# PearCoding/PearRay

Hardware: AMD Instinct MI355X
Metric: Msamples/s (higher is better)
Workload: dtype f32; 1 GPU; C4: Cornell box + 999968-triangle soup (1000000 triangles), 1920x1080, `direct` integrator (NEE+MIS+RR, depth 64), sobol 1024-spp schedule, hero wavelengths (spd CMIS), 307 iterations timed; parallelism=tiles1, collective=none (one rank)

## Files before the change

pearray_amd/csrc/device/pr_device.h:

```cpp
#pragma once

#include <hip/hip_runtime.h>
#include <stdint.h>

#include "../../../include/prgpu.h"

#ifndef PR_INLINE_CLOSURES
#define PR_INLINE_CLOSURES 0
#endif

#if PR_INLINE_CLOSURES
#define PR_CLOSURE __forceinline__
#else
#define PR_CLOSURE __noinline__
#endif

namespace prd {

constexpr float PR_EPS		= 1.1920928955078125e-7f;
constexpr float PR_INV_PI_F = 0.31830988618379067154f;
constexpr float PR_PI_F	  = 3.14159265358979323846f;
constexpr uint32_t INVALID	= PRGPU_INVALID_ID;
constexpr float SHADOW_RAY_MIN = 0.0001f;
constexpr float BOUNCE_RAY_MIN = 0.0001f;
// ... 5 lines not shown
constexpr float CIE_END		   = 830.0f;
constexpr float CIE_Y_NORM_SUM = 113.042314572337f;
constexpr float CIE_RANGE	   = CIE_END - CIE_START;
constexpr float CIE_DELTA	   = CIE_RANGE / (CIE_SAMPLES - 1);
constexpr float CIE_Y_NORM	   = CIE_Y_NORM_SUM * CIE_DELTA;

struct __attribute__((aligned(64))) Rec64 {
	float4 q[4];
};
static_assert(sizeof(Rec64) == 64, "Rec64 must be 64 bytes");
constexpr uint32_t REC_LEAF_BIT = 1u;
constexpr uint32_t REC_SINGLE_BIT = 2u;
constexpr uint32_t REC_EMPTY	= 0xFFFFFFFFu;
constexpr uint32_t REC_UNIT_SHIFT = 2u;
constexpr uint32_t LEAF_UNIT_SINGLE = 0x80000000u;
__host__ __device__ __forceinline__ const float4* rec_ptr(const Rec64* recs, uint32_t ref)
{
	return reinterpret_cast<const float4*>(reinterpret_cast<const char*>(recs) + (size_t(ref & ~3u) << 4));
}
constexpr float SLAB_REL		= 1.0000028610229492f;
constexpr float INV_D_MAX		= 1.2089258196146292e24f;
constexpr float SCENE_COORD_MAX = 268435456.0f;

struct DevEntity {
	float m[12];
	float nm[9];
	uint32_t first_tri, n_tris, emission, has_normals;
	float vol_scale, world_area;
	uint32_t light_id, kind;
	float sphere_r;
	uint32_t has_uvs;
};

constexpr uint32_t FEAT_DELTA_MATERIALS = 1u, FEAT_INFINITE_LIGHTS = 2u, FEAT_PLANES = 4u, FEAT_SPHERES = 8u, FEAT_AOVS = 16u, FEAT_SHAPE_LIGHTS = 32u, FEAT_TEXTURES = 64u,
				   FEAT_ROUGH_MATERIALS = 128u, FEAT_LPE = 256u, FEAT_QUADRICS = 512u, FEAT_DISKS = 1024u, FEAT_IMAGES = 2048u,
				   FEAT_MIX_MATERIALS = 4096u ,
				   FEAT_EXPR = 8192u , FEAT_ALL = 16383u;

struct DevQuadric {
	float p[10];
	float lo[3], hi[3];
	float wlo[3], whi[3];
	float inv[12];
	uint32_t tri;
	uint32_t entity;
};

struct DevShapeLight {
	float S[3], Ex[3], Ey[3], Ez[3], nrm[3];
	float width, height;
	float inv[12];
	float pdf_cache;
	float radius;
	float pad[2];
};
struct __attribute__((aligned(128))) DevLight {
	float m[12];
	float nm[9];
	uint32_t entity, kind, n_tris, tri_offset;
	uint32_t has_normals, radiance;
	float vol_scale;
	prgpu_spectrum node, lhs, rhs;
	uint32_t pad[3];
};
static_assert(sizeof(DevLight) == 256, "DevLight must be two 128-byte lines");
struct __attribute__((aligned(128))) DevMaterial {
	prgpu_material m;
	prgpu_spectrum albedo;
};
static_assert(sizeof(DevMaterial) == 128, "DevMaterial must be one 128-byte line");
constexpr uint32_t LIGHT_TRI_FLOATS = 20;
constexpr uint32_t PRIM_SPHERE_BIT = 0x40000000u;
constexpr uint32_t PRIM_DISK_BIT   = 0x20000000u;
constexpr uint32_t PRIM_INDEX_MASK = ~(PRIM_SPHERE_BIT | PRIM_DISK_BIT);

struct DevInfLight {
	uint32_t kind, radiance, background, flags;
	float nm[9], inv_nm[9];
	float outgoing[3];
	float dx[3], dy[3];
	float cos_theta, cone_pdf;
	uint32_t table_offset, az_count, el_count;
	uint32_t dist_offset, dist_w, dist_h;
	float ground_brightness;
};
constexpr int SKY_BANDS			 = PRGPU_SKY_BANDS;
constexpr float SKY_BAND_START	 = 320.0f;
constexpr float SKY_BAND_DELTA	 = 40.0f;
constexpr float ELEVATION_RANGE = PR_PI_F * 0.5f;
constexpr float AZIMUTH_RANGE	 = PR_PI_F * 2;

struct DevCamera {
	float o[3], right[3], up[3], focal[3], xap[3], yap[3];
	float near_t, far_t;
	uint32_t dof, ortho;
	uint32_t kind;
	float angles[4];
	float fov, xaspect, yaspect;
	uint32_t clip;
};

struct DevScene {
	const Rec64* recs;
	uint32_t n_tris, n_inner, n_leaf;
	uint32_t bvh_wide;
	const float* positions;
	const float* normals;
	const float* uvs;
	const uint32_t* indices;
	const uint32_t* tri_material;
	const uint32_t* tri_entity;
	const uint32_t* tri_slot;
	const uint8_t* tri_class;
	const DevEntity* entities;
	const DevMaterial* materials;
	const prgpu_emission* emissions;
	const prgpu_spectrum* spectra;
	const float* tables;
	const uint32_t* light_entity;
	const DevLight* lights;
	const float* light_tris;
	const float* light_cdf;
	uint32_t n_lights;
	const DevInfLight* inf_lights;
	const DevShapeLight* shape_lights;
	uint32_t n_inf_lights;
	const float* sky_cdf;
	float scene_radius;
	uint32_t features;
	const float* wl_cdf;
	uint32_t wl_cdf_size;
	float wl_u_offset, wl_u_scale;
	float agh_c, agh_n;
	const float* sobol2d;
	const float* rr_prob;
	uint32_t rr_size;
	const float* filter;
	const float* cie;
	DevCamera cam;
	prgpu_settings cfg;
	uint32_t spp, mj_x, mj_y, mj_seed;
	uint32_t halton_bx, halton_by, halton_burnin;
	uint32_t single_tap;
	float centre_weight;
	float eps_t;
	const DevQuadric* quadrics;
	uint32_t n_quadrics;
	const float4* shade_rec;
};

struct __attribute__((aligned(128))) SlotState {
	float4 ray_o, ray_d;
	float4 hit;
	uint32_t flags, pad[3];
	float4 sh_o, sh_d;
	float4 wl, wl_pdf;
	float4 cie_x, cie_y, cie_z;
	float4 throughput, path_pdf, prev_pdf;
	float4 last_pos;
	float4 sh_xyz;
};
static_assert(sizeof(SlotState) == 256, "SlotState must be two 128-byte lines");
struct PathState {
	uint64_t* rng;
	uint32_t* pixel;
	struct SlotState* st;
	uint32_t* iter;
	float4* sh_o;
	float4* sh_d;
	float4* sh_xyz;
	uint32_t* sh_slot;
	float* iter_xyz;
	uint32_t plane_stride;
	uint32_t iter_base;
	float* out_xyz;
	uint32_t* samples;
	uint32_t* feedback;
	uint32_t* prim_entity;
	uint32_t* prim_prim;
	float* online_mean;
	float* online_variance;
	const struct DevLpe* lpe;
	uint32_t* cost;
	float* aov[PRGPU_AOV_COUNT];
	uint32_t aov_mask;
};

constexpr uint32_t FLAG_MONO		  = 1u << 8;
constexpr uint32_t FLAG_LAST_DELTA	  = 1u << 9;
constexpr uint32_t FLAG_LAST_EMISSIVE = 1u << 10;
constexpr uint32_t FLAG_NO_RAY		  = 1u << 12;
constexpr uint32_t FLAG_GROUP_MONO	  = 1u << 11;

struct V3 {
	float x, y, z;
};
__device__ __forceinline__ V3 v3(float x, float y, float z) { return V3{ x, y, z }; }
__device__ __forceinline__ V3 operator+(V3 a, V3 b) { return v3(a.x + b.x, a.y + b.y, a.z + b.z); }
__device__ __forceinline__ V3 operator-(V3 a, V3 b) { return v3(a.x - b.x, a.y - b.y, a.z - b.z); }
__device__ __forceinline__ V3 operator-(V3 a) { return v3(-a.x, -a.y, -a.z); }
__device__ __forceinline__ V3 operator*(V3 a, float s) { return v3(a.x * s, a.y * s, a.z * s); }
__device__ __forceinline__ float dot(V3 a, V3 b) { return (a.x * b.x + a.y * b.y) + a.z * b.z; }
__device__ __forceinline__ V3 cross(V3 a, V3 b) { return v3(a.y * b.z - a.z * b.y, a.z * b.x - a.x * b.z, a.x * b.y - a.y * b.x); }
__device__ __forceinline__ V3 normalized(V3 a)
{
	const float n = sqrtf(dot(a, a));
	return v3(a.x / n, a.y / n, a.z / n);
}
__device__ __forceinline__ float comp(V3 a, int i) { return i == 0 ? a.x : (i == 1 ? a.y : a.z); }

struct Blob {
	float v[4];
};
__device__ __forceinline__ Blob blob(float a) { return Blob{ { a, a, a, a } }; }
__device__ __forceinline__ Blob blob4(float a, float b, float c, float d) { return Blob{ { a, b, c, d } }; }
__device__ __forceinline__ Blob from4(float4 a) { return blob4(a.x, a.y, a.z, a.w); }
__device__ __forceinline__ float4 to4(Blob a) { return make_float4(a.v[0], a.v[1], a.v[2], a.v[3]); }
__device__ __forceinline__ Blob operator*(Blob a, Blob b) { return blob4(a.v[0] * b.v[0], a.v[1] * b.v[1], a.v[2] * b.v[2], a.v[3] * b.v[3]); }
__device__ __forceinline__ Blob operator*(Blob a, float s) { return blob4(a.v[0] * s, a.v[1] * s, a.v[2] * s, a.v[3] * s); }
__device__ __forceinline__ Blob operator/(Blob a, Blob b) { return blob4(a.v[0] / b.v[0], a.v[1] / b.v[1], a.v[2] / b.v[2], a.v[3] / b.v[3]); }
__device__ __forceinline__ Blob operator/(Blob a, float s) { return blob4(a.v[0] / s, a.v[1] / s, a.v[2] / s, a.v[3] / s); }
__device__ __forceinline__ Blob operator-(Blob a, Blob b) { return blob4(a.v[0] - b.v[0], a.v[1] - b.v[1], a.v[2] - b.v[2], a.v[3] - b.v[3]); }
__device__ __forceinline__ float bsum(Blob a) { return ((a.v[0] + a.v[1]) + a.v[2]) + a.v[3]; }
__device__ __forceinline__ bool all_le(Blob a, float e) { return a.v[0] <= e && a.v[1] <= e && a.v[2] <= e && a.v[3] <= e; }
__device__ __forceinline__ bool is_zero(Blob a, float e)
{
	return fabsf(a.v[0]) <= e && fabsf(a.v[1]) <= e && fabsf(a.v[2]) <= e && fabsf(a.v[3]) <= e;
}
__device__ __forceinline__ Blob hero_only() { return blob4(1, 0, 0, 0); }

constexpr uint64_t PCG_MULT = 6364136223846793005ULL;
__device__ __forceinline__ uint32_t rng_u32(uint64_t& s)
{
	const uint64_t old	  = s;
	s					  = old * PCG_MULT;
	const uint32_t rshift = uint32_t(old >> 61) & 7u;
	const uint64_t x	  = old ^ (old >> 22);
	return uint32_t(x >> (22u + rshift));
}
__device__ __forceinline__ float rng_float(uint64_t& s)
{
	return __uint_as_float((rng_u32(s) >> 9) | 0x3F800000u) - 1.0f;
}

__device__ __forceinline__ void pr_sincos_2pi(float u, float& s, float& c)
{
	const float k  = floorf(u * 4.0f + 0.5f);
	const float r  = u - 0.25f * k;
	const float x  = 6.28318530717958647692f * r;
	const float x2 = x * x;
	float ps	   = -1.9515295891e-4f;
	ps			   = ps * x2 + 8.3321608736e-3f;
	ps			   = ps * x2 + -1.6666654611e-1f;
	const float sn = (ps * x2) * x + x;
	float pc	   = 2.443315711809948e-5f;
	pc			   = pc * x2 + -1.388731625493765e-3f;
	pc			   = pc * x2 + 4.166664568298827e-2f;
	const float cs = (pc * x2) * x2 + (1.0f - 0.5f * x2);
	switch (int(k) & 3) {
	case 0: s = sn; c = cs; break;
	case 1: s = cs; c = -sn; break;
	case 2: s = -sn; c = -cs; break;
	default: s = -cs; c = sn; break;
	}
}
__device__ __forceinline__ void pr_sincos_rad(float x, float& s, float& c) { pr_sincos_2pi(x * 0.15915494309189533577f, s, c); }
__device__ __forceinline__ float asin_poly(float x)
{
	const float z = x * x;
	float p		  = 4.2163199048e-2f;
	p			  = p * z + 2.4181311049e-2f;
	p			  = p * z + 4.5470025998e-2f;
	p			  = p * z + 7.4953002686e-2f;
	p			  = p * z + 1.6666752422e-1f;
	return (p * z) * x + x;
}
__device__ __forceinline__ float safe_acos(float a)
{
	const float x = fmaxf(-1.0f, fminf(1.0f, a));
	if (x < -0.5f)
		return 3.14159265358979323846f - 2.0f * asin_poly(sqrtf((1.0f + x) * 0.5f));
	if (x > 0.5f)
		return 2.0f * asin_poly(sqrtf((1.0f - x) * 0.5f));
	return 1.57079632679489661923f - asin_poly(x);
}
__device__ __forceinline__ float diff_prod(float a, float b, float c, float d)
{
	const float cd	= c * d;
	const float err = __fmaf_rn(-c, d, cd);
	const float dop = __fmaf_rn(a, b, -cd);
	return dop + err;
}
__device__ __forceinline__ float sum_prod(float a, float b, float c, float d) { return __fmaf_rn(a, b, c * d); }
__device__ __forceinline__ float atan_poly(float xx)
{
	float x = fabsf(xx), y = 0.0f;
	if (x > 2.414213562373095f) {
		y = 1.57079632679489661923f;
		x = -(1.0f / x);
	} else if (x > 0.4142135623730950f) {
		y = 0.78539816339744830962f;
		x = (x - 1.0f) / (x + 1.0f);
	}
	const float z = x * x;
	float p		  = 8.05374449538e-2f;
	p			  = p * z - 1.38776856032e-1f;
	p			  = p * z + 1.99777106478e-1f;
	p			  = p * z - 3.33329491539e-1f;
	y			  = y + ((p * z) * x + x);
	return xx < 0.0f ? -y : y;
}
__device__ __forceinline__ float pr_atan2(float y, float x)
{
	if (x == 0.0f) {
		if (y == 0.0f)
			return 0.0f;
		return y > 0.0f ? 1.57079632679489661923f : -1.57079632679489661923f;
	}
	const float a = atan_poly(y / x);
	if (x > 0.0f)
// ... 997 lines not shown
```

pearray_amd/csrc/device/render.h:

```cpp
#pragma once
#include "pr_device.h"

namespace prd {
constexpr int N_DEVICE_COUNTERS = PRGPU_STAT_COUNT + 32;

struct TraceWorkspace {
	uint32_t* queue_head = nullptr;
	uint2* spill		 = nullptr;
	uint32_t max_blocks	 = 0;
	int refill_below	 = 44;
	uint32_t* bl_list	 = nullptr;
	uint32_t* bl_word	 = nullptr;
	uint32_t* slot_unit	 = nullptr;
	size_t bl_entries	 = 0;
};
size_t trace_workspace_spill_entries(uint32_t max_blocks);
uint32_t trace_stack_capacity();

void launch_raygen(const DevScene& sc, const PathState& ps, uint32_t slot_base, uint32_t n_slots, uint32_t iter, unsigned long long* gstats, hipStream_t st);
void launch_trace_closest(const DevScene& sc, const PathState& ps, const uint32_t* active, uint32_t slot_base, uint32_t n_active, bool count,
						  const TraceWorkspace& ws, uint32_t* shade_counters, unsigned long long* gstats, hipStream_t st);
void launch_shade(const DevScene& sc, const PathState& ps, const uint32_t* active, uint32_t slot_base, uint32_t n_active, uint32_t* next_active,
				  uint32_t* counters, uint32_t* dead_list, uint32_t* queue_head_closest, uint32_t* queue_head_shadow, unsigned long long* gstats,
				  hipStream_t st);
void launch_regen(const DevScene& sc, const PathState& ps, const uint32_t* dead, uint32_t n_dead, uint32_t iter_end, uint32_t* next_active,
				  uint32_t* counters, unsigned long long* gstats, hipStream_t st);
void launch_trace_shadow(const DevScene& sc, const PathState& ps, uint32_t n_items, bool count, const TraceWorkspace& ws, unsigned long long* gstats,
						 hipStream_t st);
struct PersistentGeometry {
	uint32_t n_blocks, slots_per_block;
};
PersistentGeometry persistent_geometry(uint32_t n_owned, uint32_t max_blocks, uint32_t max_slots_per_block);
uint32_t persistent_slot_padding();
uint32_t slot_array_padding();
uint32_t persistent_block_threads();
int shade_ticks_counter();
struct PersistentTuning {
	uint32_t slots	  = 384;
	int shade_min	  = 64;
	int shade_partial = 16;
	int fin_batch	  = 16;
	int occupancy	  = 3;
	int shader_wave	  = -1;
	bool resident	  = true;
};
void launch_path_persistent(const DevScene& sc, const PathState& ps, const uint32_t* owned, uint32_t n_owned, uint32_t iter_begin, uint32_t iter_end,
							bool count, const TraceWorkspace& ws, const PersistentTuning& tune, int shader_waves , uint32_t* next_pixel, uint32_t* error,
							unsigned long long* gstats, hipStream_t st);
struct PathVariant {
	int id;
	uint32_t features;
};
constexpr uint32_t FEAT_NO_LPE = FEAT_ALL & ~(FEAT_LPE | FEAT_QUADRICS | FEAT_DISKS | FEAT_IMAGES | FEAT_MIX_MATERIALS | FEAT_EXPR), FEAT_NO_ROUGH = FEAT_NO_LPE & ~FEAT_ROUGH_MATERIALS;
constexpr PathVariant PATH_VARIANTS[] = { { 1, 0u }, { 2, FEAT_DELTA_MATERIALS }, { 3, FEAT_NO_ROUGH }, { 4, FEAT_NO_LPE }, { 5, FEAT_ALL } };
constexpr int N_PATH_VARIANTS		  = int(sizeof(PATH_VARIANTS) / sizeof(PATH_VARIANTS[0]));
constexpr int path_variant(uint32_t features)
{
	for (int i = 0; i < N_PATH_VARIANTS - 1; ++i)
		if ((features & ~PATH_VARIANTS[i].features) == 0u)
			return i;
	return N_PATH_VARIANTS - 1;
}
constexpr int path_variant_row(int id)
{
	int i = 0;
	while (i < N_PATH_VARIANTS && PATH_VARIANTS[i].id != id)
		++i;
	return i;
}
constexpr bool path_variants_nested()
{
	for (int i = 0; i + 1 < N_PATH_VARIANTS; ++i)
		if ((PATH_VARIANTS[i].features & ~PATH_VARIANTS[i + 1].features) != 0u)
			return false;
	return true;
}
static_assert(PATH_VARIANTS[N_PATH_VARIANTS - 1].features == FEAT_ALL, "the last variant must cover every scene");
constexpr bool expr_rides_with_images()
{
	for (int i = 0; i < N_PATH_VARIANTS; ++i)
		if (((PATH_VARIANTS[i].features & FEAT_IMAGES) != 0u) != ((PATH_VARIANTS[i].features & FEAT_EXPR) != 0u))
			return false;
	return true;
}
static_assert(expr_rides_with_images(), "FEAT_EXPR and FEAT_IMAGES must sit in the same rows: the closures' _uv forms serve both");
static_assert(path_variants_nested(), "each variant's mask must be contained in the next one's: then the first covering row is the smallest covering one");
struct PathSub {
	int occupancy;
	bool wide, count;
};
constexpr PathSub PATH_SUBS[] = { { 3, false, false }, { 3, false, true }, { 2, false, false }, { 2, false, true }, { 3, true, false }, { 3, true, true } };
constexpr int N_PATH_SUBS	  = int(sizeof(PATH_SUBS) / sizeof(PATH_SUBS[0]));
constexpr int path_sub(int occupancy, bool wide, bool count)
{
	const int occ = occupancy >= 3 ? 3 : 2;
	int i		  = 0;
	while (i < N_PATH_SUBS && !(PATH_SUBS[i].occupancy == occ && PATH_SUBS[i].count == count && (occ == 2 || PATH_SUBS[i].wide == wide)))
		++i;
	return i;
}
constexpr bool path_subs_complete()
{
	for (int k = 0; k < 8; ++k)
		if (path_sub(2 + (k >> 2), (k & 2) != 0, (k & 1) != 0) >= N_PATH_SUBS)
			return false;
	for (int i = 0; i < N_PATH_SUBS; ++i)
		if (path_sub(PATH_SUBS[i].occupancy, PATH_SUBS[i].wide, PATH_SUBS[i].count) != i)
			return false;
	return true;
}
static_assert(path_subs_complete(), "PATH_SUBS and path_sub disagree");
struct LatencyGeometry {
	uint32_t n_blocks, slots_per_wave, total_slots;
};
struct LatencyTuning {
	uint32_t slots_per_wave = 256;
	int shade_min			= 48;
	int refill_below		= 40;
};
LatencyGeometry latency_geometry(uint32_t n_owned, uint32_t max_blocks_throughput, uint32_t max_slots_per_wave);
bool latency_variant_built(uint32_t features);
void launch_path_latency(const DevScene& sc, const PathState& ps, const uint32_t* owned, uint32_t n_owned, uint32_t iter_begin, uint32_t iter_end, bool count,
						 const TraceWorkspace& ws, const LatencyTuning& tune, uint32_t* error, unsigned long long* gstats, hipStream_t st);
void launch_resolve(const DevScene& sc, const PathState& ps, uint32_t iter, hipStream_t st);
size_t sort_active_temp_bytes(uint32_t n_max);
void launch_sort_active(const DevScene& sc, const PathState& ps, const uint32_t* active, uint32_t n, uint32_t* keys_in, uint32_t* keys_out, uint32_t* active_out,
						void* temp, size_t temp_bytes, hipStream_t st);
void launch_service_closest(const DevScene& sc, uint32_t n, const float* org, const float* dir, const float* tmin, const float* tmax,
							uint32_t* entity, uint32_t* prim, float* u, float* v, float* t, const TraceWorkspace& ws, unsigned long long* gstats,
							hipStream_t st);
void launch_tri_slot(const DevScene& sc, const uint32_t* leaf_units , uint32_t* tri_slot, hipStream_t st);
void launch_service_closest_split(const DevScene& sc, uint32_t n, const float* org, const float* dir, const float* tmin, const float* tmax,
								  uint32_t* entity, uint32_t* prim, float* u, float* v, float* t, const TraceWorkspace& ws, uint32_t* tri_slot,
								  unsigned long long* gstats, bool leaf_single , hipStream_t st);
void launch_service_any(const DevScene& sc, uint32_t n, const float* org, const float* dir, const float* tmin, const float* distance,
						uint8_t* occluded, const TraceWorkspace& ws, unsigned long long* gstats, hipStream_t st);
struct AoState {
	float4* rec;
	uint32_t* occluded;
	const uint64_t* jump;
	uint32_t* counts;
	uint64_t jump_all;
	uint32_t sample_count;
	uint64_t* dbg_state;
	float* dbg_org;
	float* dbg_dir;
	uint8_t* dbg_occluded;
};

void launch_ao_hits(const DevScene& sc, const PathState& ps, const AoState& ao, uint32_t n_slots, bool instrumented, uint32_t* n_hits, uint32_t* queue_head_closest,
					uint32_t* queue_head_ao, unsigned long long* gstats, hipStream_t st);
void launch_ao_occlusion(const DevScene& sc, const PathState& ps, const AoState& ao, uint32_t n_slots, bool instrumented, const uint32_t* n_hits, const TraceWorkspace& ws,
						 unsigned long long* gstats, hipStream_t st);
void launch_ao_splat(const DevScene& sc, const PathState& ps, const AoState& ao, uint32_t n_slots, const uint32_t* n_hits, hipStream_t st);
bool ao_counts_folded();

constexpr uint32_t VF_RANDOM_COLOURS = 23, VF_GREEN = 23, VF_RED = 24, VF_BLUE = 25, VF_COLOURS = 26;
struct VfState {
	const float4* colours;
	uint32_t mode;
	uint32_t weighting;
};
void launch_vf_shade(const DevScene& sc, const PathState& ps, const VfState& vf, uint32_t n_slots, uint32_t* queue_head_closest, unsigned long long* gstats, hipStream_t st);
}
```

pearray_amd/csrc/device/render.hip:

```cpp
#define PR_WAVEFRONT 1
#define PR_THROUGHPUT 2
#define PR_LATENCY 3
#if !defined(PR_UNIT) || (PR_UNIT != PR_WAVEFRONT && PR_UNIT != PR_THROUGHPUT && PR_UNIT != PR_LATENCY)
#error "compile with -DPR_UNIT=PR_WAVEFRONT, PR_THROUGHPUT or PR_LATENCY (see the Makefile)"
#endif
#include "render.h"

#include <algorithm>
#include <array>
#include <utility>
#if PR_UNIT == PR_WAVEFRONT
#include <hipcub/hipcub.hpp>
#endif

namespace prd {

__device__ __forceinline__ unsigned long long lane_ballot(bool p) { return __builtin_amdgcn_ballot_w64(p); }
__device__ __forceinline__ bool lane_in(unsigned long long m) { return __builtin_amdgcn_inverse_ballot_w64(m); }
__device__ __forceinline__ int wave_popc(unsigned long long m)
{
	int n = __builtin_popcountll(m);
	asm volatile("" : "+s"(n));
	return n;
}
// ... 641 lines not shown
	if ((FEATS & FEAT_QUADRICS) && E.kind == PRGPU_ENTITY_QUADRIC) {
		const DevQuadric& Q = sc.quadrics[E.has_uvs];
		const V3 L = v3(((Q.inv[0] * P.x + Q.inv[1] * P.y) + Q.inv[2] * P.z) + Q.inv[3], ((Q.inv[4] * P.x + Q.inv[5] * P.y) + Q.inv[6] * P.z) + Q.inv[7],
						((Q.inv[8] * P.x + Q.inv[9] * P.y) + Q.inv[10] * P.z) + Q.inv[11]);
		g.N = mat3_mul(E.nm, normalized(quadric_gradient(Q.p, L)));
		frame_duff(g.N, g.Nx, g.Ny);
		g.Nx	   = normalized(g.Nx);
		g.Ny	   = normalized(g.Ny);
		g.entity   = e;
		g.prim	   = 0;
		g.material = sc.tri_material[tri];
		g.emission = E.emission;
		g.uv[0] = g.uv[1] = 0.0f;
		return;
	}
	if ((FEATS & FEAT_PLANES) && E.kind == PRGPU_ENTITY_PLANE) {
		const uint32_t t0 = E.first_tri;
		const V3 v0 = load3(sc.positions, sc.indices[3 * t0]), v1 = load3(sc.positions, sc.indices[3 * t0 + 1]), v3p = load3(sc.positions, sc.indices[3 * t0 + 2]);
		const V3 x = v3p - v0, y = v1 - v0;
		g.N		   = normalized(mat3_mul(E.nm, normalized(cross(x, y))));
		g.Nx	   = normalized(linear_mul(E.m, x));
		g.Ny	   = normalized(linear_mul(E.m, y));
		g.entity   = e;
		g.prim	   = 0;
		g.material = sc.tri_material[tri];
		g.emission = E.emission;
		g.uv[0] = tri == E.first_tri ? u : 1 - u;
		g.uv[1] = tri == E.first_tri ? v : 1 - v;
		return;
	}
	const bool has_uv = (FEATS & FEAT_TEXTURES) && E.has_uvs != 0u;
	const V3 n0 = v3(r0.x, r0.y, r0.z), n1 = v3(r0.w, r1.x, r1.y), n2 = v3(r1.z, r1.w, r2.x);
	const V3 p0 = v3(r2.y, r2.z, r2.w), p1 = v3(r3.x, r3.y, r3.z), p2 = v3(r3.w, r4.x, r4.y);
	const float uv0[2] = { r4.z, r4.w }, uv1[2] = { r5.x, r5.y }, uv2[2] = { r5.z, r5.w };
	if (FEATS & (FEAT_TEXTURES | FEAT_AOVS)) {
		if (has_uv) {
			for (int c = 0; c < 2; ++c)
				g.uv[c] = (uv1[c] * u + uv2[c] * v) + uv0[c] * (1 - u - v);
		} else {
			g.uv[0] = u;
			g.uv[1] = v;
		}
	}
	if (E.has_normals) {
		N = tri_interp(n0, n1, n2, u, v);
		if (has_uv) {
			const V3 dp1 = p1 - p0, dp2 = p2 - p0;
			const float du1 = uv1[0] - uv0[0], dv1 = uv1[1] - uv0[1];
			const float du2 = uv2[0] - uv0[0], dv2 = uv2[1] - uv0[1];
			const float det = diff_prod(dv2, du1, dv1, du2);
			if (det <= PR_EPS) {
				frame_duff(N, Nx, Ny);
				Nx = normalized_or_zero(Nx);
				Ny = normalized_or_zero(Ny);
			} else {
				const V3 t = dp1 * dv2 - dp2 * dv1;
				Nx		   = v3(t.x / det, t.y / det, t.z / det);
				Nx		   = Nx - N * dot(N, Nx);
				Nx		   = normalized_or_zero(Nx);
				Ny		   = cross(N, Nx);
			}
		} else {
			frame_duff(N, Nx, Ny);
		}
	} else {
		Nx = p1 - p0;
		Ny = p2 - p0;
		N  = cross(Nx, Ny);
	}
	g.N		   = normalized(mat3_mul(E.nm, N));
	g.Nx	   = normalized(mat3_mul(E.nm, Nx));
	g.Ny	   = normalized(mat3_mul(E.nm, Ny));
	g.entity   = e;
	g.prim	   = tri - E.first_tri;
	g.material = __float_as_uint(r6.y);
	g.emission = E.emission;
}

struct PathCie {
	float x[4], y[4], z[4];
};
__device__ __forceinline__ uint32_t fragment_value(const DevScene& sc, const Blob& mis, const Blob& importance, const Blob& grp_importance,
												  const Blob& radiance, bool mono, const PathCie& cie, float blend, float xyz[3])
{
	const Blob imp		  = grp_importance * importance;
	const Blob heroFactor = mono ? hero_only() : blob(1);
	const Blob contrib	  = heroFactor * ((mis * imp) * radiance);
	uint32_t fb = 0;
	for (int k = 0; k < 4; ++k) {
		if (isnan(contrib.v[k]))
			fb |= 0x1;
		if (isinf(contrib.v[k]))
			fb |= 0x2;
		if (contrib.v[k] < -PR_EPS)
			fb |= 0x4;
	}
	xyz[0] = xyz[1] = xyz[2] = 0.0f;
	if (fb)
		return fb;
	float triplet[3] = { 0, 0, 0 };
	if (sc.cfg.spectral_mono) {
		triplet[0] = triplet[1] = triplet[2] = contrib.v[0];
	} else {
		for (int k = 0; k < 4; ++k) {
			triplet[0] += contrib.v[k] * cie.x[k];
			triplet[1] += contrib.v[k] * cie.y[k];
			triplet[2] += contrib.v[k] * cie.z[k];
		}
	}
	const float w = sc.single_tap ? sc.centre_weight * blend : blend;
	xyz[0] = w * triplet[0];
	xyz[1] = w * triplet[1];
	xyz[2] = w * triplet[2];
	return 0;
}
__device__ __forceinline__ uint32_t fragment_feedback_zero(const Blob& mis, const Blob& importance, const Blob& grp_importance, bool mono)
{
	const Blob imp		  = grp_importance * importance;
	const Blob heroFactor = mono ? hero_only() : blob(1);
	const Blob contrib	  = heroFactor * ((mis * imp) * blob(0));
	uint32_t fb = 0;
	for (int k = 0; k < 4; ++k) {
		if (isnan(contrib.v[k]))
			fb |= 0x1;
		if (isinf(contrib.v[k]))
			fb |= 0x2;
		if (contrib.v[k] < -PR_EPS)
			fb |= 0x4;
	}
	return fb;
}
__device__ __forceinline__ size_t iter_entry(const PathState& ps, uint32_t slot, uint32_t pixel)
{
	return (ps.plane_stride ? size_t(ps.iter[slot] - ps.iter_base) * ps.plane_stride : size_t(0)) + size_t(3) * pixel;
}
__device__ __forceinline__ void apply_fragment(const PathState& ps, uint32_t pixel, size_t entry, uint32_t fb, const float xyz[3], uint32_t lpe_mask = 0u)
{
	if (fb) {
		ps.feedback[pixel] |= fb;
	} else {
		ps.iter_xyz[entry + 0] += xyz[0];
		ps.iter_xyz[entry + 1] += xyz[1];
		ps.iter_xyz[entry + 2] += xyz[2];
		for (uint32_t k = 0; lpe_mask != 0u && k < PRGPU_LPE_MAX; ++k)
			if (lpe_mask & (1u << k)) {
				float* plane = ps.lpe->iter[k];
				plane[entry + 0] += xyz[0];
				plane[entry + 1] += xyz[1];
				plane[entry + 2] += xyz[2];
			}
	}
}

__device__ __forceinline__ void fold_iteration(const PathState& ps, uint32_t pixel, uint32_t iter, const float value[3], bool with_lpe = false)
{
	const float it = (float)(iter + 1), itm1 = (float)iter;
	for (int c = 0; c < 3; ++c) {
		if (ps.online_mean) {
			float mean		  = ps.online_mean[3 * pixel + c];
			const float var	  = ps.online_variance[3 * pixel + c];
			const float delta = value[c] - mean;
			mean += delta / it;
			const float delta2				  = value[c] - mean;
			ps.online_mean[3 * pixel + c]	  = mean;
			ps.online_variance[3 * pixel + c] = (var * itm1 + delta * delta2) / it;
		}
		ps.out_xyz[3 * pixel + c] = (ps.out_xyz[3 * pixel + c] * itm1 + value[c]) / it;
	}
	if (with_lpe && ps.lpe)
		for (uint32_t k = 0; k < ps.lpe->n; ++k) {
			float* out		  = ps.lpe->out[k];
			const float* iter_ = ps.lpe->iter[k];
			for (int c = 0; c < 3; ++c)
				out[3 * pixel + c] = (out[3 * pixel + c] * itm1 + iter_[3 * pixel + c]) / it;
		}
}
__device__ __forceinline__ float rr_probability(const DevScene& sc, uint32_t L)
{
	return sc.rr_prob[L < sc.rr_size ? L : sc.rr_size - 1];
}
__device__ __forceinline__ bool is_normal(float f)
{
	const uint32_t e = (__float_as_uint(f) >> 23) & 0xFFu;
	return e != 0 && e != 0xFF;
}

struct BlockStats {
	unsigned int v[PRGPU_STAT_COUNT + 4];
};
__device__ __forceinline__ void stats_init(BlockStats& s)
{
	if (threadIdx.x < PRGPU_STAT_COUNT + 4)
		s.v[threadIdx.x] = 0;
	__syncthreads();
}
__device__ __forceinline__ void stats_flush(BlockStats& s, unsigned long long* g)
{
	__syncthreads();
	if (threadIdx.x < PRGPU_STAT_COUNT + 4 && s.v[threadIdx.x])
		atomicAdd(&g[threadIdx.x], (unsigned long long)s.v[threadIdx.x]);
}

__device__ __forceinline__ uint32_t wave_append(bool pred, uint32_t* counter)
{
	const unsigned long long mask = __ballot(pred);
	const uint32_t lane			  = threadIdx.x & 63u;
	const uint32_t prefix		  = __popcll(mask & ((1ull << lane) - 1ull));
	uint32_t base				  = 0;
	if (mask != 0ull) {
		const int leader = __ffsll((long long)mask) - 1;
		if ((int)lane == leader)
			base = atomicAdd(counter, (uint32_t)__popcll(mask));
		base = __shfl(base, leader, 64);
	}
	return base + prefix;
}

__device__ __forceinline__ float halton(uint32_t index, uint32_t base)
{
	float result = 0;
	float f		 = 1;
	for (uint32_t i = index; i > 0;) {
		f = f / base;
		result += f * (i % base);
		i = (uint32_t)floorf(i / (float)base);
	}
	return result;
}
struct WlTable {
	const float* cdf	  = nullptr;
	const uint16_t* guide = nullptr;
};
__device__ __forceinline__ bool camera_path(const DevScene& sc, const PathState& ps, uint32_t slot, uint32_t iter, BlockStats& bs, bool with_lpe = false, WlTable wlt = WlTable())
{
	const prgpu_settings& cfg = sc.cfg;
	const uint32_t pixel	  = ps.pixel[slot];
	const uint32_t gx = pixel % cfg.width, gy = pixel / cfg.width;
	uint64_t rnd = ps.rng[pixel];
	float ax, ay;
	if (cfg.aa_sampler == PRGPU_SAMPLER_MJITT) {
		const uint32_t n  = max(1u, sc.spp);
		const uint32_t id = mjitt_permute(iter, n, sc.mj_seed * 0x51633e2d);
		const uint32_t sx = mjitt_permute(id % sc.mj_x, sc.mj_x, sc.mj_seed * 0x68bc21eb);
		const uint32_t sy = mjitt_permute(id / sc.mj_x, sc.mj_y, sc.mj_seed * 0x02e5be93);
		const float jx	  = rng_float(rnd);
		const float jy	  = rng_float(rnd);
		ax				  = (sx + (sy + jx) / sc.mj_y) / sc.mj_x;
		ay				  = (id + jy) / n;
	} else if (cfg.aa_sampler == PRGPU_SAMPLER_UNIFORM) {
		ax = ay = 0.5f;
	} else if (cfg.aa_sampler == PRGPU_SAMPLER_STRATIFIED) {
		const float range = (1.0f - 0.0f) / (int)sc.mj_x;
		const float ux = rng_float(rnd), uy = rng_float(rnd);
		ax = 0.0f + ux * range + (int)(iter % sc.mj_x) * range;
		ay = 0.0f + uy * range + (int)(iter / sc.mj_x) * range;
	} else if (cfg.aa_sampler >= PRGPU_SAMPLER_SOBOL && cfg.aa_sampler <= PRGPU_SAMPLER_HAMMERSLEY && iter < sc.spp) {
		ax = sc.sobol2d[2 * iter];
		ay = sc.sobol2d[2 * iter + 1];
	} else if (cfg.aa_sampler == PRGPU_SAMPLER_HALTON || cfg.aa_sampler == PRGPU_SAMPLER_HAMMERSLEY) {
		ax = halton(iter + sc.halton_burnin, sc.halton_bx);
		ay = halton(iter + sc.halton_burnin, sc.halton_by);
	} else {
		ax = rng_float(rnd);
		ay = rng_float(rnd);
	}
	const float px = (float)gx + ax - 0.5f, py = (float)gy + ay - 0.5f;
	const float l1 = rng_float(rnd), l2 = rng_float(rnd);
	(void)rng_float(rnd);
	Blob wl, wl_pdf;
	if (cfg.spectral_mono) {
		wl	   = blob(cfg.spectral_start);
		wl_pdf = blob(1.0f);
	} else if (cfg.mapper == PRGPU_MAPPER_SPD_CMIS) {
		const float span = cfg.spectral_end - cfg.spectral_start;
		for (int k = 0; k < 4; ++k) {
			float pdf;
			const float u = rng_float(rnd);
			const float v = wlt.guide ? distribution_sample_continuous_guided(wlt.cdf, sc.wl_cdf_size, wlt.guide, u, pdf) : distribution_sample_continuous(sc.wl_cdf, sc.wl_cdf_size, u, pdf);
			wl.v[k]		  = v * span + cfg.spectral_start;
			wl_pdf.v[k]	  = pdf;
		}
	} else if (cfg.mapper == PRGPU_MAPPER_SPD_HERO) {
		const float span = cfg.spectral_end - cfg.spectral_start;
		float pdf;
		const float v	  = distribution_sample_continuous(sc.wl_cdf, sc.wl_cdf_size, rng_float(rnd), pdf);
		const float hero  = v * span + cfg.spectral_start;
		const float delta = span / 4;
		wl.v[0]			  = hero;
		for (int k = 1; k < 4; ++k)
			wl.v[k] = cfg.spectral_start + fmodf(hero - cfg.spectral_start + k * delta, span);
		wl_pdf = blob(pdf);
	} else if (cfg.mapper == PRGPU_MAPPER_AGH_CMIS) {
		for (int k = 0; k < 4; ++k) {
			wl.v[k]		= agh_sample(rng_float(rnd), sc.agh_n, sc.agh_c);
			wl_pdf.v[k] = agh_pdf(wl.v[k], sc.agh_n);
		}
	} else if (cfg.mapper == PRGPU_MAPPER_AGH_HERO) {
		const float span  = cfg.spectral_end - cfg.spectral_start;
		const float hero  = agh_sample(rng_float(rnd), sc.agh_n, sc.agh_c);
		const float delta = span / 4;
		wl.v[0]			  = hero;
		for (int k = 1; k < 4; ++k)
			wl.v[k] = cfg.spectral_start + fmodf(hero - cfg.spectral_start + k * delta, span);
		wl_pdf = blob(agh_pdf(hero, sc.agh_n));
	} else if (cfg.mapper == PRGPU_MAPPER_CIE || cfg.mapper == PRGPU_MAPPER_CIE_Y) {
		const float span = cfg.spectral_end - cfg.spectral_start;
		for (int k = 0; k < 4; ++k) {
			float pdf;
			const float v = distribution_sample_continuous(sc.wl_cdf, sc.wl_cdf_size, sc.wl_u_offset + rng_float(rnd) * sc.wl_u_scale, pdf);
			wl.v[k]		  = v * span + cfg.spectral_start;
			wl_pdf.v[k]	  = pdf / sc.wl_u_scale;
		}
	} else {
		const float u	  = rng_float(rnd);
		const float span  = cfg.spectral_end - cfg.spectral_start;
		const float delta = span / 4;
		const float start = u * span;
		wl.v[0]			  = start + cfg.spectral_start;
		for (int k = 1; k < 4; ++k)
			wl.v[k] = cfg.spectral_start + fmodf(start + k * delta, span);
		wl_pdf = blob(1.0f);
	}
	const float nx = 2 * (px / (float)cfg.width - 0.5f);
	const float ny = -(2 * (py / (float)cfg.height - 0.5f));
	const DevCamera& cam = sc.cam;
	V3 o = v3(cam.o[0], cam.o[1], cam.o[2]);
	V3 d = (v3(cam.right[0], cam.right[1], cam.right[2]) * nx + v3(cam.up[0], cam.up[1], cam.up[2]) * ny) + v3(cam.focal[0], cam.focal[1], cam.focal[2]);
	bool has_ray = true;
	if (cam.kind == PRGPU_CAMERA_SPHERICAL) {
		const float sx = px / (float)cfg.width, sy = 1 - py / (float)cfg.height;
		const float theta = cam.angles[0] + sy * (cam.angles[1] - cam.angles[0]);
		const float phi	  = cam.angles[2] + sx * (cam.angles[3] - cam.angles[2]);
		float sT, cT, sP, cP;
		pr_sincos_rad(theta, sT, cT);
		pr_sincos_rad(phi, sP, cP);
		d = normalized(from_tangent_space(v3(cam.up[0], cam.up[1], cam.up[2]), v3(cam.right[0], cam.right[1], cam.right[2]), v3(cam.focal[0], cam.focal[1], cam.focal[2]),
										  v3(sP * cT, cP * cT, sT)));
	} else if (cam.kind == PRGPU_CAMERA_FISHEYE) {
		const float fx = 2 * (px / (float)cfg.width - 0.5f) / cam.xaspect;
		const float fy = -(2 * (py / (float)cfg.height - 0.5f) / cam.yaspect);
		has_ray		   = !(cam.clip && fx * fx + fy * fy > 1);
		const float r	  = sqrtf(fx * fx + fy * fy);
		const float theta = r * cam.fov / 2;
		float sT, cT;
		pr_sincos_rad(theta, sT, cT);
		const float sP = r < PR_EPS ? 0 : fy / r;
		const float cP = r < PR_EPS ? 0 : fx / r;
		d = normalized(from_tangent_space(v3(cam.focal[0], cam.focal[1], cam.focal[2]), v3(cam.right[0], cam.right[1], cam.right[2]), v3(cam.up[0], cam.up[1], cam.up[2]),
										  v3(cP * sT, sP * sT, cT)));
	} else if (cam.ortho) {
		o = (o + v3(cam.right[0], cam.right[1], cam.right[2]) * nx) + v3(cam.up[0], cam.up[1], cam.up[2]) * ny;
		d = v3(cam.focal[0], cam.focal[1], cam.focal[2]);
	} else {
		if (cam.dof) {
			float sn, cs;
			pr_sincos_2pi(l1, sn, cs);
			const V3 e = v3(cam.xap[0], cam.xap[1], cam.xap[2]) * (l2 * sn) + v3(cam.yap[0], cam.yap[1], cam.yap[2]) * (l2 * cs);
			o		   = o + e;
			d		   = d - e;
		}
		d = normalized(d);
	}
	const bool mono	   = cfg.spectral_mono || !cfg.spectral_hero;
	ps.rng[pixel]	   = rnd;
	if (has_ray) {
		ps.st[slot].ray_o = make_float4(o.x, o.y, o.z, cam.near_t);
		ps.st[slot].ray_d = make_float4(d.x, d.y, d.z, cam.far_t);
	} else {
		ps.st[slot].ray_o = make_float4(o.x, o.y, o.z, 1.0f);
		ps.st[slot].ray_d = make_float4(0.0f, 0.0f, 1.0f, 0.0f);
	}
	ps.st[slot].wl		   = to4(wl);
	ps.st[slot].wl_pdf	   = to4(wl_pdf);
	{
		float c0[3], c1[3], c2[3], c3[3];
		cie_eval(sc.cie, wl.v[0], c0);
		cie_eval(sc.cie, wl.v[1], c1);
		cie_eval(sc.cie, wl.v[2], c2);
		cie_eval(sc.cie, wl.v[3], c3);
		ps.st[slot].cie_x = make_float4(c0[0], c1[0], c2[0], c3[0]);
		ps.st[slot].cie_y = make_float4(c0[1], c1[1], c2[1], c3[1]);
		ps.st[slot].cie_z = make_float4(c0[2], c1[2], c2[2], c3[2]);
	}
	ps.st[slot].throughput = make_float4(1, 1, 1, 1);
	ps.st[slot].path_pdf  = make_float4(1, 1, 1, 1);
	ps.st[slot].prev_pdf  = make_float4(1, 1, 1, 1);
	if (sc.features & FEAT_SHAPE_LIGHTS)
		ps.st[slot].last_pos = make_float4(0, 0, 0, 0);
	ps.st[slot].flags	   = 0u | (mono ? (FLAG_MONO | FLAG_GROUP_MONO) : 0u) | FLAG_LAST_DELTA | (has_ray ? 0u : FLAG_NO_RAY);
	if (with_lpe && ps.lpe) {
		const DevLpe& L	   = *ps.lpe;
		L.state[slot]	   = lpe_step(ps.lpe, 0u, LPE_SYM_CAMERA);
		const size_t lentry = (ps.plane_stride ? size_t(iter - ps.iter_base) * ps.plane_stride : size_t(0)) + size_t(3) * pixel;
		for (uint32_t k = 0; k < L.n; ++k) {
			float* plane	  = L.iter[k];
			plane[lentry + 0] = 0.0f;
			plane[lentry + 1] = 0.0f;
			plane[lentry + 2] = 0.0f;
		}
	}
	{
		const size_t entry = (ps.plane_stride ? size_t(iter - ps.iter_base) * ps.plane_stride : size_t(0)) + size_t(3) * pixel;
		ps.iter_xyz[entry + 0] = 0.0f;
		ps.iter_xyz[entry + 1] = 0.0f;
		ps.iter_xyz[entry + 2] = 0.0f;
	}
	atomicAdd(&bs.v[PRGPU_STAT_PIXEL_SAMPLES], 1u);
	if (has_ray) {
		atomicAdd(&bs.v[PRGPU_STAT_CAMERA_RAYS], 1u);
		atomicAdd(&bs.v[PRGPU_STAT_PRIMARY_RAYS], 1u);
	}
	return has_ray;
}

#if PR_UNIT == PR_WAVEFRONT
__global__ void __launch_bounds__(256) k_raygen(DevScene sc, PathState ps, uint32_t slot_base, uint32_t n_slots, uint32_t iter, unsigned long long* gstats)
{
	__shared__ BlockStats bs;
	stats_init(bs);
	const uint32_t local = blockIdx.x * blockDim.x + threadIdx.x;
	if (local < n_slots) {
		ps.iter[slot_base + local] = iter;
		camera_path(sc, ps, slot_base + local, iter, bs, ps.lpe != nullptr);
	}
	stats_flush(bs, gstats);
}

__global__ void __launch_bounds__(256) k_regen(DevScene sc, PathState ps, const uint32_t* __restrict__ dead, uint32_t n_dead, uint32_t iter_end,
											  uint32_t* __restrict__ next_active, uint32_t* __restrict__ counters, unsigned long long* gstats)
{
	__shared__ BlockStats bs;
	stats_init(bs);
	const uint32_t i = blockIdx.x * blockDim.x + threadIdx.x;
	bool alive	  = false;
	uint32_t slot = 0;
	if (i < n_dead) {
		slot				 = dead[i];
		const uint32_t pixel = ps.pixel[slot];
		const uint32_t iter	 = ps.iter[slot];
		const float v[3] = { ps.iter_xyz[3 * pixel], ps.iter_xyz[3 * pixel + 1], ps.iter_xyz[3 * pixel + 2] };
		fold_iteration(ps, pixel, iter, v, ps.lpe != nullptr);
		if (iter + 1 < iter_end) {
			ps.iter[slot] = iter + 1;
			camera_path(sc, ps, slot, iter + 1, bs, ps.lpe != nullptr);
			alive = true;
		}
	}
	const uint32_t pos = wave_append(alive, &counters[0]);
	if (alive)
		next_active[pos] = slot;
	stats_flush(bs, gstats);
}

template <bool COUNT>
__global__ void __launch_bounds__(TRAV_BLOCK) k_trace_closest(DevScene sc, PathState ps, const uint32_t* __restrict__ active, uint32_t slot_base,
															 uint32_t n_active, uint32_t* queue_head, uint2* spill, int refill_below, uint32_t* shade_counters,
															 unsigned long long* gstats)
{
	if (blockIdx.x == 0 && threadIdx.x == 0) {
		shade_counters[0] = 0;
		shade_counters[1] = 0;
		shade_counters[2] = 0;
	}
	auto load = [&](uint32_t i, V3& o, V3& d, float& tmin, float& tmax) {
		const uint32_t slot = active ? active[i] : slot_base + i;
		const float4 ro = ps.st[slot].ray_o, rd = ps.st[slot].ray_d;
		o	 = v3(ro.x, ro.y, ro.z);
		d	 = v3(rd.x, rd.y, rd.z);
		tmin = ro.w;
		tmax = rd.w;
	};
	auto store = [&](uint32_t i, const Hit& h) {
		const uint32_t slot = active ? active[i] : slot_base + i;
		ps.st[slot].hit		= make_float4(h.t, h.u, h.v, __uint_as_float(h.tri));
	};
	trace_persistent<false, COUNT>(sc, n_active, queue_head, spill, refill_below, load, store, gstats);
}

#endif
__device__ __forceinline__ RoughDistribution rough_distribution(const prgpu_material& m)
{
	const bool aniso = (m.flags & PRGPU_MATF_ANISOTROPIC) != 0;
	return RoughDistribution{ m.roughness_x, aniso ? m.roughness_y : m.roughness_x, aniso, (m.flags & PRGPU_MATF_NO_VNDF) == 0 };
}
__device__ __forceinline__ Blob rough_dielectric_eval(const RoughDistribution& d, V3 V, V3 L, const Blob& spec, const Blob& trans, const Blob& ior)
{
	Blob w;
	if (sv_same_hemisphere(V, L)) {
		for (int i = 0; i < 4; ++i)
			w.v[i] = mf_reflection_eval(d, V, L, false, DIELECTRIC_AIR, ior.v[i]);
		return w * spec;
	}
	for (int i = 0; i < 4; ++i)
		w.v[i] = mf_transmission_eval(d, V, L, DIELECTRIC_AIR, ior.v[i]);
	return w * trans;
}
__device__ __forceinline__ Blob rough_dielectric_pdf(const RoughDistribution& d, V3 V, V3 L, const Blob& ior)
{
	Blob F, p;
	for (int i = 0; i < 4; ++i)
		F.v[i] = fresnel_dielectric(V.z, DIELECTRIC_AIR, ior.v[i]);
	if (sv_same_hemisphere(V, L)) {
		for (int i = 0; i < 4; ++i)
			p.v[i] = mf_reflection_pdf(d, L, V);
		return F * p;
	}
	for (int i = 0; i < 4; ++i)
		p.v[i] = mf_transmission_pdf(d, V, L, DIELECTRIC_AIR, ior.v[i]);
	return (blob(1) - F) * p;
}
struct Principled {
	Blob base, ior, cie_y;
	float diff_trans, roughness, anisotropic, spec_trans, spec_tint, flatness, metallic, sheen, sheen_tint, clearcoat, clearcoat_gloss;
	bool thin, has_trans, vndf;

	__device__ __forceinline__ static float mix(float v0, float v1, float t) { return (1 - t) * v0 + t * v1; }
	__device__ __forceinline__ static float schlick_r0(float eta)
	{
		const float factor = (eta - 1.0f) / (eta + 1.0f);
		return factor * factor;
	}
	__device__ __forceinline__ float thin_transmission_roughness() const { return fmaxf(0.0f, fminf(1.0f, (0.65f * (bsum(ior) / 4) - 0.35f) * roughness)); }
	__device__ __forceinline__ RoughDistribution roughness_closure(float r) const
	{
		const float aspect = sqrtf(1 - anisotropic * 0.9f);
		const float ax	   = fmaxf(0.001f, r * r / aspect);
		const float ay	   = fmaxf(0.001f, r * r * aspect);
		return RoughDistribution{ ax, ay, true, vndf };
	}
	__device__ __forceinline__ bool is_delta() const { return roughness_closure(roughness).is_delta(); }
	struct Lobes {
		float diff_refl, diff_trans, spec_refl, spec_trans;
	};
	__device__ __forceinline__ Lobes lobe_distribution(V3 V) const
	{
		Lobes d;
		d.diff_refl = roughness * roughness * (1.0f - metallic) * (1.0f - spec_trans);
		d.spec_refl = 1;
		if (has_trans) {
			const float F = fresnel_dielectric(V.z, DIELECTRIC_AIR, ior.v[0]);
			d.diff_trans  = diff_trans * d.diff_refl;
			d.spec_trans  = (1.0f - F) * (1.0f - metallic) * spec_trans;
			d.spec_refl *= F;
		} else {
			d.diff_trans = 0;
			d.spec_trans = 0;
		}
		const float norm = d.diff_refl + d.spec_refl + d.diff_trans + d.spec_trans;
		if (norm <= PR_EPS)
			return Lobes{ 1.0f, 0.0f, 0.0f, 0.0f };
		d.diff_refl /= norm;
		d.spec_refl /= norm;
		d.diff_trans /= norm;
		d.spec_trans /= norm;
// ... 334 lines not shown
	v = theta * PR_INV_PI_F;
}
__device__ __forceinline__ float env_jacobian(float v)
{
	float s, c;
	pr_sincos_rad(v * PR_PI_F, s, c);
	const float denom = 2 * PR_PI_F * PR_PI_F * s;
	return denom <= PR_EPS ? 0.0f : 1.0f / denom;
}
template <bool EXPR = false>
__device__ __forceinline__ void inf_light_eval(const DevScene& sc, const DevInfLight& il, V3 dir, const Blob& wl, bool camera_ray, Blob& radiance, float& dir_pdf)
{
	if (il.kind == PRGPU_LIGHT_ENVIRONMENT && (il.flags & PRGPU_ENVF_TEXTURED)) {
		const V3 ld = mat3_mul(il.inv_nm, dir);
		float u, v;
		uv_from_direction(ld, u, v);
		radiance = (camera_ray && il.background != INVALID) ? spectrum_eval<false, EXPR>(sc, il.background, wl) : env_image_eval<EXPR>(sc, il, wl, u, v);
		if (il.dist_w)
			dir_pdf = distribution2d_pdf(sc.sky_cdf + il.dist_offset, il.dist_w, il.dist_h, u, v) * env_jacobian(v);
		else
			dir_pdf = fabsf(ld.z) * PR_INV_PI_F;
		return;
	}
	if (il.kind == PRGPU_LIGHT_SKY) {
		const ElAz ea	  = ea_from_direction(mat3_mul(il.inv_nm, dir));
		const bool extend = (il.flags & PRGPU_SKYF_EXTEND) != 0;
		if (!extend && ea.el < 0.0f) {
			radiance = blob(0);
			dir_pdf	 = 0.0f;
			return;
		}
		radiance = sky_radiance(sc.tables + il.table_offset, il.az_count, il.el_count, wl, ea);
		dir_pdf	 = distribution2d_pdf(sc.sky_cdf + il.dist_offset, il.dist_w, il.dist_h, ea.az / AZIMUTH_RANGE,
									  extend ? ea.el / (2 * ELEVATION_RANGE) + 0.5f : ea.el / ELEVATION_RANGE);
		dir_pdf *= sky_jacobian(ea.el);
		return;
	}
	if (il.kind == PRGPU_LIGHT_SUN) {
		const float cosine = fmaxf(0.0f, dot(dir, v3(il.outgoing[0], il.outgoing[1], il.outgoing[2])));
		if (cosine < il.cos_theta) {
			radiance = blob(0);
			dir_pdf	 = 0.0f;
		} else {
			radiance = spectrum_eval<false, EXPR>(sc, il.radiance, wl);
			dir_pdf	 = il.cone_pdf;
		}
		return;
	}
	if (il.kind == PRGPU_LIGHT_CIE_SKY) {
		radiance = cie_sky_radiance<EXPR>(sc, il, wl, dir);
		dir_pdf	 = fabsf(mat3_mul(il.inv_nm, dir).z) * PR_INV_PI_F;
		return;
	}
	radiance	= spectrum_eval<false, EXPR>(sc, (camera_ray && il.background != INVALID) ? il.background : il.radiance, wl);
	const V3 ld = mat3_mul(il.inv_nm, dir);
	dir_pdf		= fabsf(ld.z) * PR_INV_PI_F;
}
template <bool EXPR = false>
__device__ __forceinline__ void inf_light_sample(const DevScene& sc, const DevInfLight& il, float d0, float d1, const Blob& wl, V3& L, float& dir_pdf, Blob& radiance)
{
	if (il.kind == PRGPU_LIGHT_DISTANT) {
		L		 = v3(il.outgoing[0], il.outgoing[1], il.outgoing[2]);
		dir_pdf	 = 1.0f;
		radiance = spectrum_eval<false, EXPR>(sc, il.radiance, wl);
	} else if (il.kind == PRGPU_LIGHT_ENVIRONMENT && (il.flags & PRGPU_ENVF_TEXTURED)) {
		float u, v;
		V3 lo;
		if (il.dist_w) {
			distribution2d_sample(sc.sky_cdf + il.dist_offset, il.dist_w, il.dist_h, d0, d1, u, v, dir_pdf);
			float st, ct, sp, cp;
			pr_sincos_rad(v * PR_PI_F, st, ct);
			pr_sincos_rad(u * 2 * PR_PI_F, sp, cp);
			lo = v3(st * cp, st * sp, ct);
			dir_pdf *= env_jacobian(v);
		} else {
			u		= d0;
			v		= d1;
			lo		= cos_hemi(d0, d1);
			dir_pdf = lo.z * PR_INV_PI_F;
		}
		L		 = mat3_mul(il.nm, lo);
		radiance = env_image_eval<EXPR>(sc, il, wl, u, v);
	} else if (il.kind == PRGPU_LIGHT_SKY) {
		float u, v;
		distribution2d_sample(sc.sky_cdf + il.dist_offset, il.dist_w, il.dist_h, d0, d1, u, v, dir_pdf);
		const ElAz ea = (il.flags & PRGPU_SKYF_EXTEND) ? ElAz{ 2 * ELEVATION_RANGE * (v - 0.5f), AZIMUTH_RANGE * u } : ElAz{ ELEVATION_RANGE * v, AZIMUTH_RANGE * u };
		L			  = mat3_mul(il.nm, ea_to_direction(ea));
		dir_pdf *= sky_jacobian(ea.el);
		radiance = sky_radiance(sc.tables + il.table_offset, il.az_count, il.el_count, wl, ea);
	} else if (il.kind == PRGPU_LIGHT_SUN) {
		const V3 dir = uniform_cone(d0, d1, il.cos_theta);
		L			 = from_tangent_space(v3(il.outgoing[0], il.outgoing[1], il.outgoing[2]), v3(il.dx[0], il.dx[1], il.dx[2]), v3(il.dy[0], il.dy[1], il.dy[2]), dir);
		dir_pdf		 = il.cone_pdf;
		radiance	 = spectrum_eval<false, EXPR>(sc, il.radiance, wl);
	} else {
		const V3 lo = cos_hemi(d0, d1);
		dir_pdf		= lo.z * PR_INV_PI_F;
		L			= mat3_mul(il.nm, lo);
		radiance	= il.kind == PRGPU_LIGHT_CIE_SKY ? cie_sky_radiance<EXPR>(sc, il, wl, L) : spectrum_eval<false, EXPR>(sc, il.radiance, wl);
	}
}

__device__ __forceinline__ uint32_t scatter_symbol(uint32_t kind, float roughness_x, V3 Vt, V3 Lt)
{
	const bool same = sv_same_hemisphere(Vt, Lt);
	switch (kind) {
	case PRGPU_MAT_LAMBERT:
	case PRGPU_MAT_OREN_NAYAR: return LPE_SYM_DIFFUSE_REFLECTION;
	case PRGPU_MAT_NULL: return LPE_SYM_SPECULAR_TRANSMISSION;
	case PRGPU_MAT_DIELECTRIC:
	case PRGPU_MAT_ROUGH_DIELECTRIC: return same ? LPE_SYM_SPECULAR_REFLECTION : LPE_SYM_SPECULAR_TRANSMISSION;
	case PRGPU_MAT_PRINCIPLED:
		return roughness_x < 0.5f ? (same ? LPE_SYM_SPECULAR_REFLECTION : LPE_SYM_SPECULAR_TRANSMISSION) : (same ? LPE_SYM_DIFFUSE_REFLECTION : LPE_SYM_DIFFUSE_TRANSMISSION);
	default: return LPE_SYM_SPECULAR_REFLECTION;
	}
}
__device__ __forceinline__ uint32_t scatter_symbol(const prgpu_material& m, V3 Vt, V3 Lt) { return scatter_symbol(m.kind, m.roughness_x, Vt, Lt); }

template <bool AOVS>
__device__ __forceinline__ void commit_shading_point(const PathState& ps, uint32_t pixel, V3 P, const GeomPoint& gp, V3 ray_d, float depth2)
{
	ps.samples[pixel] += 1;
	if (AOVS && ps.aov_mask) {
		auto add3 = [&](int k, V3 v) {
			if (ps.aov[k]) {
				ps.aov[k][3 * pixel] += v.x;
				ps.aov[k][3 * pixel + 1] += v.y;
				ps.aov[k][3 * pixel + 2] += v.z;
			}
		};
		auto add1 = [&](int k, float v) {
			if (ps.aov[k])
				ps.aov[k][pixel] += v;
		};
		add3(PRGPU_AOV_POSITION, P);
		add3(PRGPU_AOV_NORMAL, gp.N);
		add3(PRGPU_AOV_NORMAL_G, gp.N);
		add3(PRGPU_AOV_TANGENT, gp.Nx);
		add3(PRGPU_AOV_BITANGENT, gp.Ny);
		add3(PRGPU_AOV_VIEW, ray_d);
		add1(PRGPU_AOV_ENTITY_ID, (float)gp.entity);
		add1(PRGPU_AOV_MATERIAL_ID, (float)gp.material);
		add1(PRGPU_AOV_EMISSION_ID, (float)gp.emission);
		add1(PRGPU_AOV_DEPTH, sqrtf(depth2));
	}
}

template <uint32_t FEATS>
__device__ __forceinline__ void shade_vertex(const DevScene& sc, const PathState& ps, uint32_t slot, BlockStats& bs, bool& alive, bool& want_shadow,
											 float4& sh_o, float4& sh_d, float4& sh_xyz, const float4* hit_src = nullptr )
{
	constexpr bool EXPR		  = (FEATS & FEAT_EXPR) != 0u;
	const prgpu_settings& cfg = sc.cfg;
	const uint32_t pixel = ps.pixel[slot];
	const size_t entry	 = iter_entry(ps, slot, pixel);
	const float4 ro = ps.st[slot].ray_o, rd = ps.st[slot].ray_d;
	const V3 ray_o = v3(ro.x, ro.y, ro.z), ray_d = v3(rd.x, rd.y, rd.z);
	const float4 hit4  = hit_src ? *hit_src : ps.st[slot].hit;
	const uint32_t tri = __float_as_uint(hit4.w);
	uint32_t flags	   = ps.st[slot].flags;
	if (flags & FLAG_NO_RAY)
		return;
	const uint32_t depth = flags & 0xFFu;
	const bool mono		 = (flags & FLAG_MONO) != 0;
	const Blob wl		 = from4(ps.st[slot].wl);
	const Blob wvl_pdf	 = from4(ps.st[slot].wl_pdf);
	PathCie cie;
	{
		const float4 cx = ps.st[slot].cie_x, cy = ps.st[slot].cie_y, cz = ps.st[slot].cie_z;
		cie.x[0] = cx.x; cie.x[1] = cx.y; cie.x[2] = cx.z; cie.x[3] = cx.w;
		cie.y[0] = cy.x; cie.y[1] = cy.y; cie.y[2] = cy.z; cie.y[3] = cy.w;
		cie.z[0] = cz.x; cie.z[1] = cz.y; cie.z[2] = cz.z; cie.z[3] = cz.w;
	}
	Blob throughput		 = from4(ps.st[slot].throughput);
	Blob path_pdf		 = from4(ps.st[slot].path_pdf);
	Blob prev_pdf		 = from4(ps.st[slot].prev_pdf);
	const Blob grp_imp	 = (flags & FLAG_GROUP_MONO) ? hero_only() : blob(1.0f);
	const float blend	 = 1.0f;
	const bool power_mis = cfg.mis == PRGPU_MIS_POWER;
	const Blob hf		 = mono ? hero_only() : blob(1.0f);
	const bool with_lpe	 = (FEATS & FEAT_LPE) && ps.lpe != nullptr;
	uint32_t lpe		 = with_lpe ? ps.lpe->state[slot] : 0u;

	if (depth == 0 && tri == INVALID) {
		ps.prim_entity[pixel] = INVALID;
		ps.prim_prim[pixel]	  = INVALID;
	}
	if (tri == INVALID) {
		atomicAdd(&bs.v[PRGPU_STAT_BACKGROUND_HITS], 1u);
		float xyz[3];
		uint32_t fb;
		const uint32_t m_bg = with_lpe ? lpe_accepting(ps.lpe, lpe_step(ps.lpe, lpe, LPE_SYM_BACKGROUND)) : 0u;
		if (depth == 0) {
			atomicAdd(&bs.v[PRGPU_STAT_CAMERA_DEPTH], 1u);
			bool illuminated = false;
			for (uint32_t k = 0; (FEATS & FEAT_INFINITE_LIGHTS) && k < sc.n_inf_lights; ++k) {
				const DevInfLight& il = sc.inf_lights[k];
				if (il.kind == PRGPU_LIGHT_DISTANT)
					continue;
				illuminated = true;
				Blob radiance;
				float dir_pdf;
				inf_light_eval<EXPR>(sc, il, ray_d, wl, true, radiance, dir_pdf);
				fb = fragment_value(sc, blob(1), blob(1), grp_imp, radiance, mono, cie, blend, xyz);
				apply_fragment(ps, pixel, entry, fb, xyz, m_bg);
			}
			if (!illuminated) {
				fb = fragment_value(sc, blob(1), blob(1), grp_imp, blob(0), mono, cie, blend, xyz);
				apply_fragment(ps, pixel, entry, fb, xyz, m_bg);
			}
		} else if ((FEATS & FEAT_INFINITE_LIGHTS) && sc.n_inf_lights && cfg.direct) {
			float denom_mis = 0;
			Blob radiance	= blob(0);
			for (uint32_t k = 0; k < sc.n_inf_lights; ++k) {
				const DevInfLight& il = sc.inf_lights[k];
				if (il.kind == PRGPU_LIGHT_DISTANT)
					continue;
				Blob er;
				float dir_pdf;
				inf_light_eval<EXPR>(sc, il, ray_d, wl, false, er, dir_pdf);
				const float selProb = sc.light_cdf[sc.n_lights + k + 1] - sc.light_cdf[sc.n_lights + k];
				const float pdf_S	= dir_pdf * selProb;
				for (int c = 0; c < 4; ++c)
					radiance.v[c] += er.v[c];
				const Blob a = prev_pdf * pdf_S;
				denom_mis += bsum(power_mis ? a * a : a);
			}
			if (!cfg.nee || (flags & FLAG_LAST_DELTA)) {
				fb = fragment_value(sc, hf / (wvl_pdf * bsum(hf)), throughput, grp_imp, radiance, mono, cie, blend, xyz);
			} else {
				const float denom = bsum(power_mis ? path_pdf * path_pdf : path_pdf) + denom_mis;
				const float p0	  = power_mis ? path_pdf.v[0] * path_pdf.v[0] : path_pdf.v[0];
				const Blob mis	  = (hf * p0) / ((power_mis ? wvl_pdf * wvl_pdf : wvl_pdf) * denom);
				fb				  = fragment_value(sc, mis, throughput, grp_imp, radiance, mono, cie, blend, xyz);
			}
			apply_fragment(ps, pixel, entry, fb, xyz, m_bg);
		} else {
			fb = fragment_value(sc, hf / (wvl_pdf * bsum(hf)), throughput, grp_imp, blob(0), mono, cie, blend, xyz);
			apply_fragment(ps, pixel, entry, fb, xyz, m_bg);
		}
	} else {
		const V3 P = ray_o + ray_d * hit4.x;
		GeomPoint gp;
		geometry_point<FEATS>(sc, tri, hit4.y, hit4.z, P, gp);
		if (depth == 0) {
			ps.prim_entity[pixel] = gp.entity;
			ps.prim_prim[pixel]	  = gp.prim;
		}
		const V3 N		   = gp.N;
		const float NdotV  = dot(ray_d, N);
		const V3 dP		   = ray_o - P;
		const float depth2 = dot(dP, dP);
		const uint32_t pathLength = depth + 1;
		atomicAdd(&bs.v[PRGPU_STAT_ENTITY_HITS], 1u);
		atomicAdd(&bs.v[PRGPU_STAT_CAMERA_DEPTH], 1u);
		if (pathLength == 1)
			commit_shading_point<(FEATS & FEAT_AOVS) != 0>(ps, pixel, P, gp, ray_d, depth2);
		const bool hasEmission = gp.emission != INVALID;
		bool go_on			   = true;
		if (cfg.direct && hasEmission) {
			const float cosC = -NdotV;
			if (!(fabsf(cosC) <= PR_EPS)) {
				const bool behind	= cosC < 0.0f;
				const Blob radiance = behind ? blob(0) : spectrum_eval<false, EXPR>(sc, sc.emissions[gp.emission].radiance, wl);
				float xyz[3];
				uint32_t fb;
				if (!cfg.nee || behind || (flags & FLAG_LAST_DELTA)) {
					fb = fragment_value(sc, hf / (wvl_pdf * bsum(hf)), throughput, grp_imp, radiance, mono, cie, blend, xyz);
				} else {
					const uint32_t lid	 = sc.entities[gp.entity].light_id;
					const float selProb	 = sc.light_cdf[lid + 1] - sc.light_cdf[lid];
					float posPDF		 = 1.0f / sc.entities[gp.entity].world_area;
					if ((FEATS & FEAT_SHAPE_LIGHTS) && sc.entities[gp.entity].kind == PRGPU_ENTITY_PLANE) {
						const float4 lpos = ps.st[slot].last_pos;
						posPDF			  = plane_light_pdf(sc.shape_lights[gp.entity], P, v3(lpos.x, lpos.y, lpos.z));
					} else if ((FEATS & FEAT_SHAPE_LIGHTS) && sc.entities[gp.entity].kind == PRGPU_ENTITY_SPHERE) {
						posPDF = 2 * sc.shape_lights[gp.entity].pdf_cache;
					}
					posPDF				 = posPDF * depth2 / fabsf(cosC);
					const float posPDF_S = posPDF * selProb;
					const Blob a		 = prev_pdf * posPDF_S;
					const float denom	 = bsum(power_mis ? a * a : a) + bsum(power_mis ? path_pdf * path_pdf : path_pdf);
					const float p0		 = power_mis ? path_pdf.v[0] * path_pdf.v[0] : path_pdf.v[0];
					const Blob mis		 = (hf * p0) / ((power_mis ? wvl_pdf * wvl_pdf : wvl_pdf) * denom);
					fb					 = fragment_value(sc, mis, throughput, grp_imp, radiance, mono, cie, blend, xyz);
				}
				apply_fragment(ps, pixel, entry, fb, xyz, with_lpe ? lpe_accepting(ps.lpe, lpe_step(ps.lpe, lpe, LPE_SYM_EMISSIVE)) : 0u);
			}
			if (!cfg.emissive_scatter)
				go_on = false;
		}
		if (gp.material == INVALID)
			go_on = false;
		if (go_on) {
			const DevMaterial& dmat = sc.materials[gp.material];
			prgpu_material mat		= dmat.m;
			constexpr bool MIX		= (FEATS & FEAT_MIX_MATERIALS) != 0u;
			const bool comb			= MIX && (mat.kind == PRGPU_MAT_BLEND || mat.kind == PRGPU_MAT_ADD);
			if ((FEATS & FEAT_TEXTURES) && (sc.features & FEAT_TEXTURES) && !comb) {
				mat.albedo		 = resolve_texture(sc, mat.albedo, gp.uv);
				mat.ior			 = resolve_texture(sc, mat.ior, gp.uv);
				mat.k			 = resolve_texture(sc, mat.k, gp.uv);
				mat.transmission = resolve_texture(sc, mat.transmission, gp.uv);
			}
			const V3 Vt				 = to_tangent_space(N, gp.Nx, gp.Ny, -ray_d);
			uint64_t rnd			 = ps.rng[pixel];
			const bool deltaMat		 = (FEATS & FEAT_DELTA_MATERIALS) && (mat.kind == PRGPU_MAT_DIELECTRIC || mat.kind == PRGPU_MAT_CONDUCTOR || mat.kind == PRGPU_MAT_MIRROR);
			const bool roughMat		 = (FEATS & FEAT_ROUGH_MATERIALS) && (mat.kind == PRGPU_MAT_ROUGH_CONDUCTOR || mat.kind == PRGPU_MAT_ROUGH_DIELECTRIC || mat.kind == PRGPU_MAT_PRINCIPLED);
			const bool delta1 = comb && mix_delta_only(sc.materials[mat.two_sided].m.kind), delta2 = comb && mix_delta_only(sc.materials[mat.thin].m.kind);
			const bool deltaOnly = comb ? (delta1 && delta2) : (deltaMat || (MIX && mat.kind == PRGPU_MAT_NULL));
			const Blob cie_y_blob	 = blob4(cie.y[0], cie.y[1], cie.y[2], cie.y[3]);
			constexpr bool IMG	= (FEATS & FEAT_IMAGES) != 0u;
			Blob albedo_v		= roughMat ? blob(0) : albedo_eval<IMG, EXPR>(sc, mat, dmat.albedo, dmat.m.albedo, wl, gp.uv);
			if (cfg.nee && !deltaOnly && !hasEmission && (sc.n_lights + ((FEATS & FEAT_INFINITE_LIGHTS) ? sc.n_inf_lights : 0u))) {
				do {
					float selPdf;
					const uint32_t n_sel = sc.n_lights + ((FEATS & FEAT_INFINITE_LIGHTS) ? sc.n_inf_lights : 0u);
					const float u_sel	 = rng_float(rnd);
					uint32_t lid		 = 0;
					if (n_sel == 1)
						selPdf = 1.0f;
					else
						lid = distribution_sample_discrete(sc.light_cdf, n_sel + 1, u_sel, selPdf, nullptr);
					if ((FEATS & FEAT_INFINITE_LIGHTS) && lid >= sc.n_lights) {
						const DevInfLight& il = sc.inf_lights[lid - sc.n_lights];
						const float d0 = rng_float(rnd), d1 = rng_float(rnd);
						(void)rng_float(rnd);
						(void)rng_float(rnd);
						V3 L;
						float dirPdf;
						const bool delta = il.kind == PRGPU_LIGHT_DISTANT;
						Blob radiance;
						inf_light_sample<EXPR>(sc, il, d0, d1, wl, L, dirPdf, radiance);
						const V3 lpos	 = P + L * sc.scene_radius;
						const V3 dLP	 = lpos - P;
						const float sqrD = dot(dLP, dLP);
						const float cosC = fabsf(dot(L, N));
						const float cosL = 1.0f;
						if (!(cosC * cosL > GEOMETRY_EPS && sqrD > DISTANCE_EPS))
							break;
						const V3 Lt = to_tangent_space(N, gp.Nx, gp.Ny, L);
						Blob weight, bsdf_pdf;
						bool evalDelta;
						uint32_t sym_kind	= 0u;
						float sym_roughness = 0.0f;
						if constexpr (MIX)
							vertex_eval<FEATS>(sc, mat, albedo_v, comb, delta1, delta2, wl, cie_y_blob, Vt, Lt, weight, bsdf_pdf, evalDelta, sym_kind, sym_roughness, gp.uv);
						else
							material_eval<FEATS>(sc, mat, albedo_v, wl, cie_y_blob, Vt, Lt, weight, bsdf_pdf, evalDelta, gp.uv);
						if (evalDelta)
							break;
						const Blob bsdfWvlPdfS = bsdf_pdf * hf;
						if (all_le(bsdfWvlPdfS, PDF_EPS))
							break;
						const Blob connectionW = radiance * weight;
						const bool worth	   = !is_zero(connectionW, PR_EPS);
						float lightPdfS;
						if (delta) {
							lightPdfS = 1;
						} else {
							lightPdfS = dirPdf;
							lightPdfS *= selPdf;
							if (!is_normal(lightPdfS) || lightPdfS <= PDF_EPS)
								break;
						}
						const Blob lightPdfS2 = (blob(1) * lightPdfS) * hf;
						if (all_le(lightPdfS2, PDF_EPS))
							break;
						Blob mis;
						if (cfg.direct && !(flags & FLAG_LAST_EMISSIVE)) {
							const float rr		= rr_probability(sc, pathLength);
							const Blob bsdfPdfS = bsdfWvlPdfS * rr;
							const Blob a = path_pdf * lightPdfS2, b = path_pdf * bsdfPdfS;
							const float denom = bsum(power_mis ? a * a : a) + bsum(power_mis ? b * b : b);
							const float num	  = path_pdf.v[0] * lightPdfS2.v[0];
							mis = delta ? hf / bsum(hf) : blob(power_mis ? num * num : num) / ((hf * denom) * (power_mis ? wvl_pdf * wvl_pdf : wvl_pdf));
						} else {
							mis = hf / (wvl_pdf * bsum(hf));
						}
						const V3 oN = dot(L, N) < 0 ? -N : N;
						float sh_far = INFINITY;
						const V3 so	 = sane_ray(safe_position(P, L, oN), sh_far);
						float xyz_vis[3];
						const float xyz_occ[3] = { 0.0f, 0.0f, 0.0f };
						const uint32_t fb_vis = fragment_value(sc, mis, throughput, grp_imp, connectionW / lightPdfS2.v[0], mono, cie, blend, xyz_vis);
						const uint32_t fb_occ = fragment_feedback_zero(mis, throughput, grp_imp, mono);
						atomicAdd(&bs.v[PRGPU_STAT_BACKGROUND_HITS], 1u);
						if (worth) {
							atomicAdd(&bs.v[PRGPU_STAT_SHADOW_RAYS], 1u);
							want_shadow = true;
							sh_o		= make_float4(so.x, so.y, so.z, SHADOW_RAY_MIN);
							sh_d		= make_float4(L.x, L.y, L.z, sh_far);
							const uint32_t m_nee = with_lpe ? lpe_accepting(ps.lpe, lpe_step(ps.lpe, lpe_step(ps.lpe, lpe, scatter_symbol(MIX ? sym_kind : mat.kind, MIX ? sym_roughness : mat.roughness_x, Vt, Lt)), LPE_SYM_BACKGROUND)) : 0u;
							sh_xyz		= make_float4(xyz_vis[0], xyz_vis[1], xyz_vis[2], __uint_as_float(fb_vis | (fb_occ << 8) | (m_nee << 16)));
						} else {
							apply_fragment(ps, pixel, entry, fb_occ, xyz_occ);
						}
						break;
					}
					const DevLight& LE = sc.lights[lid];
					const uint32_t le  = LE.entity;
					const float u0 = rng_float(rnd), u1 = rng_float(rnd);
					V3 lp;
					float pdf_a;
					GeomPoint lgp;
					if ((FEATS & FEAT_SHAPE_LIGHTS) && LE.kind == PRGPU_ENTITY_PLANE) {
						const DevShapeLight& SL = sc.shape_lights[le];
						plane_light_sample(SL, P, u0, u1, lp, pdf_a);
						lgp.N = v3(SL.Ez[0], SL.Ez[1], SL.Ez[2]);
					} else if ((FEATS & FEAT_SHAPE_LIGHTS) && LE.kind == PRGPU_ENTITY_SPHERE) {
						sphere_light_sample(sc.shape_lights[le], LE.m, P, u0, u1, lp, pdf_a);
						lgp.N = normalized_or_zero(lp - v3(LE.m[3], LE.m[7], LE.m[11]));
					} else if ((FEATS & FEAT_DISKS) && LE.kind == PRGPU_ENTITY_DISK) {
						disk_light_sample(sc.shape_lights[le], LE.m, u0, u1, lp, pdf_a);
						lgp.N = normalized(mat3_mul(LE.nm, v3(0.0f, 0.0f, 1.0f)));
					} else {
						float k0, k1;
						const float f0		= modff(u0 * LE.n_tris, &k0);
						const float f1		= modff(u1 * LE.n_tris, &k1);
						const uint32_t face = min((uint32_t)k0, LE.n_tris - 1);
						const float* lt = sc.light_tris + size_t(LE.tri_offset + face) * LIGHT_TRI_FLOATS;
						const V3 p0 = v3(lt[0], lt[1], lt[2]), p1 = v3(lt[3], lt[4], lt[5]), p2 = v3(lt[6], lt[7], lt[8]);
						const V3 ee		 = cross(p1 - p0, p2 - p0);
						const float area = 0.5f * sqrtf(dot(ee, ee));
						pdf_a			 = 1.0f / (LE.n_tris * area * LE.vol_scale);
						float bu, bv;
						if (f1 > f0) {
							const float x = f0 / 2;
							bu = x;
							bv = f1 - x;
						} else {
							const float y = f1 / 2;
							bu = f0 - y;
							bv = y;
						}
						lp = affine_mul(LE.m, tri_interp(p0, p1, p2, bu, bv));
						V3 Nl;
						if (LE.has_normals)
							Nl = tri_interp(v3(lt[9], lt[10], lt[11]), v3(lt[12], lt[13], lt[14]), v3(lt[15], lt[16], lt[17]), bu, bv);
						else
							Nl = cross(p1 - p0, p2 - p0);
						lgp.N = normalized(mat3_mul(LE.nm, Nl));
					}
					const V3 L			 = normalized(lp - P);
					const float cosLight = fminf(1.0f, fmaxf(-1.0f, -dot(L, lgp.N)));
					const Blob radiance	 = spectrum_eval_copy<EXPR>(sc, LE.node, LE.lhs, LE.rhs, wl);
					const V3 dLP		 = lp - P;
					const float sqrD	 = dot(dLP, dLP);
					const float cosC	 = fabsf(dot(L, N));
					const float cosL	 = fabsf(cosLight);
					if (!(cosC * cosL > GEOMETRY_EPS && sqrD > DISTANCE_EPS))
						break;
					const V3 Lt = to_tangent_space(N, gp.Nx, gp.Ny, L);
					Blob weight, bsdf_pdf;
					bool evalDelta;
					uint32_t sym_kind	= 0u;
					float sym_roughness = 0.0f;
					if constexpr (MIX)
						vertex_eval<FEATS>(sc, mat, albedo_v, comb, delta1, delta2, wl, cie_y_blob, Vt, Lt, weight, bsdf_pdf, evalDelta, sym_kind, sym_roughness, gp.uv);
					else
						material_eval<FEATS>(sc, mat, albedo_v, wl, cie_y_blob, Vt, Lt, weight, bsdf_pdf, evalDelta, gp.uv);
					if (evalDelta)
						break;
					const Blob bsdfWvlPdfS = bsdf_pdf * hf;
					if (all_le(bsdfWvlPdfS, PDF_EPS))
						break;
					const Blob connectionW = radiance * weight;
					const bool worth	   = !is_zero(connectionW, PR_EPS);
					float lightPdfS		   = pdf_a * sqrD / cosL;
					lightPdfS *= selPdf;
					if (!is_normal(lightPdfS) || lightPdfS <= PDF_EPS)
						break;
					const Blob lightPdfS2 = (blob(1) * lightPdfS) * hf;
					if (all_le(lightPdfS2, PDF_EPS))
						break;
					Blob mis;
					if (cfg.direct && !(flags & FLAG_LAST_EMISSIVE)) {
						const float rr		= rr_probability(sc, pathLength);
						const Blob bsdfPdfS = bsdfWvlPdfS * rr;
						const Blob a = path_pdf * lightPdfS2, b = path_pdf * bsdfPdfS;
						const float denom = bsum(power_mis ? a * a : a) + bsum(power_mis ? b * b : b);
						const float num	  = path_pdf.v[0] * lightPdfS2.v[0];
						mis				  = blob(power_mis ? num * num : num) / ((hf * denom) * (power_mis ? wvl_pdf * wvl_pdf : wvl_pdf));
					} else {
						mis = hf / (wvl_pdf * bsum(hf));
					}
					float distance = sqrtf(sqrD);
					const V3 oN	   = dot(L, N) < 0 ? -N : N;
					const V3 so	   = sane_ray(safe_position(P, L, oN), distance);
					float xyz_vis[3];
					const float xyz_occ[3] = { 0.0f, 0.0f, 0.0f };
					const uint32_t fb_vis = fragment_value(sc, mis, throughput, grp_imp, connectionW / lightPdfS2.v[0], mono, cie, blend, xyz_vis);
					const uint32_t fb_occ = fragment_feedback_zero(mis, throughput, grp_imp, mono);
					atomicAdd(&bs.v[PRGPU_STAT_ENTITY_HITS], 1u);
					if (worth) {
						atomicAdd(&bs.v[PRGPU_STAT_SHADOW_RAYS], 1u);
						want_shadow = true;
						sh_o		= make_float4(so.x, so.y, so.z, SHADOW_RAY_MIN);
						sh_d		= make_float4(L.x, L.y, L.z, distance);
						const uint32_t m_nee = with_lpe ? lpe_accepting(ps.lpe, lpe_step(ps.lpe, lpe_step(ps.lpe, lpe, scatter_symbol(MIX ? sym_kind : mat.kind, MIX ? sym_roughness : mat.roughness_x, Vt, Lt)), LPE_SYM_EMISSIVE)) : 0u;
						sh_xyz		= make_float4(xyz_vis[0], xyz_vis[1], xyz_vis[2], __uint_as_float(fb_vis | (fb_occ << 8) | (m_nee << 16)));
					} else {
						apply_fragment(ps, pixel, entry, fb_occ, xyz_occ);
					}
				} while (false);
			}
			flags = hasEmission ? (flags | FLAG_LAST_EMISSIVE) : (flags & ~FLAG_LAST_EMISSIVE);

			const float scatProb = deltaOnly ? 1.0f : rr_probability(sc, pathLength);
			bool cont			 = !(scatProb <= PR_EPS);
			if (cont && scatProb < 1.0f) {
				const float rp = rng_float(rnd);
				if (rp > scatProb)
					cont = false;
			}
			if (cont) {
				V3 Lt;
				Blob integral_weight, pdf_s;
				bool heroCollapsing = false;
				float mix_weight = 1.0f, mix_pdf = 1.0f;
				bool child_rough = false;
				if (comb) {
					const bool add	  = mat.kind == PRGPU_MAT_ADD;
					const float f	  = fminf(1.0f, fmaxf(0.0f, mat.roughness_x));
					const bool second = !(rng_float(rnd) < (add ? 0.5f : 1 - f));
					mix_pdf			  = add ? 0.5f : (second ? f : 1 - f);
					mix_weight		  = add ? 1.0f : mix_pdf;
					const uint32_t id = second ? mat.thin : mat.two_sided;
					mix_child<FEATS>(sc, id, wl, gp.uv, mat, albedo_v, child_rough);
				}
				const bool sampleDeltaMat = comb ? mix_delta_only(mat.kind) : deltaOnly, sampleRoughMat = comb ? child_rough : roughMat;
				bool sampleDelta	= sampleDeltaMat;
				if (sampleRoughMat && IMG) {
					rough_sample_uv(sc, mat, wl, cie_y_blob, Vt, rnd, Lt, integral_weight, pdf_s, sampleDelta, heroCollapsing, gp.uv);
				} else if (sampleRoughMat) {
					rough_sample(sc, mat, wl, cie_y_blob, Vt, rnd, Lt, integral_weight, pdf_s, sampleDelta, heroCollapsing);
				} else if ((FEATS & FEAT_DELTA_MATERIALS) && mat.kind == PRGPU_MAT_MIRROR) {
					pdf_s			= blob(1);
					integral_weight = albedo_v;
					Lt				= v3(-Vt.x, -Vt.y, Vt.z);
				} else if (MIX && mat.kind == PRGPU_MAT_NULL) {
					pdf_s			= blob(1);
					integral_weight = blob(1);
					Lt				= -Vt;
				} else if ((FEATS & FEAT_DELTA_MATERIALS) && mat.kind == PRGPU_MAT_CONDUCTOR) {
					pdf_s		   = blob(1);
					const Blob eta = spectrum_eval<IMG, EXPR>(sc, mat.ior, wl, gp.uv), kk = spectrum_eval<IMG, EXPR>(sc, mat.k, wl, gp.uv);
					Blob fresnel;
					for (int i = 0; i < 4; ++i)
						fresnel.v[i] = fresnel_conductor(fabsf(Vt.z), 1.0f, eta.v[i], kk.v[i]);
					integral_weight = fresnel * albedo_v;
					Lt				= v3(-Vt.x, -Vt.y, Vt.z);
					heroCollapsing	= spectrum_varying<EXPR>(sc.spectra[mat.ior]) || spectrum_varying<EXPR>(sc.spectra[mat.k]);
				} else if (sampleDeltaMat) {
					pdf_s		  = blob(1);
					const Blob n2 = spectrum_eval<IMG, EXPR>(sc, mat.ior, wl, gp.uv);
					float F		  = fresnel_dielectric(Vt.z, DIELECTRIC_AIR, n2.v[0]);
					if (mat.thin && F < 1.0f)
						F += (1 - F) * F / (F + 1);
					const Blob rWeight = albedo_v;
					if (rng_float(rnd) <= F) {
						Lt				= v3(-Vt.x, -Vt.y, Vt.z);
						integral_weight = rWeight;
					} else {
						const Blob tWeight = mat.transmission != INVALID ? spectrum_eval<IMG, EXPR>(sc, mat.transmission, wl, gp.uv) : rWeight;
						if (mat.thin) {
							Lt				= -Vt;
							integral_weight = tWeight;
						} else {
							Lt				= refract_shading(DIELECTRIC_AIR / n2.v[0], Vt);
							integral_weight = (signbit(Lt.z) == signbit(Vt.z)) ? rWeight : tWeight;
						}
					}
					heroCollapsing = spectrum_varying<EXPR>(sc.spectra[mat.ior]);
				} else if (MIX && mat.kind == PRGPU_MAT_OREN_NAYAR) {
					const float s1 = rng_float(rnd), s2 = rng_float(rnd);
					Lt				= cos_hemi(s1, s2);
					integral_weight = oren_nayar_calc(albedo_v, mat.roughness_x, Vt, Lt, fmaxf(0.0f, Lt.z));
					pdf_s			= blob(Lt.z * PR_INV_PI_F);
				} else if (!mat.two_sided && Vt.z < 0.0f) {
					Lt				= v3(0, 0, 0);
					integral_weight = blob(0);
					pdf_s			= blob(0);
				} else {
					const float s1 = rng_float(rnd), s2 = rng_float(rnd);
					Lt				= cos_hemi(s1, s2);
					integral_weight = albedo_v;
					pdf_s			= blob(Lt.z * PR_INV_PI_F);
					if (signbit(Vt.z) != signbit(Lt.z))
						Lt = -Lt;
				}
				if (comb) {
					integral_weight = integral_weight * mix_weight;
					pdf_s			= pdf_s * mix_pdf;
				}
				const V3 L = normalized(from_tangent_space(N, gp.Nx, gp.Ny, Lt));
				if (with_lpe)
					lpe = lpe_step(ps.lpe, lpe, scatter_symbol(mat, Vt, Lt));
				flags	 = sampleDelta ? (flags | FLAG_LAST_DELTA) : (flags & ~FLAG_LAST_DELTA);
				prev_pdf = path_pdf;
				path_pdf = path_pdf * (pdf_s * scatProb);
				if (all_le(path_pdf, PDF_EPS))
					cont = false;
				if (cont) {
					throughput = throughput * integral_weight;
					if (heroCollapsing) {
						throughput = throughput * hero_only();
						path_pdf   = path_pdf * hero_only();
					}
					if (is_zero(throughput, PR_EPS))
						cont = false;
					if (heroCollapsing)
						flags |= FLAG_MONO;
				}
				if (cont) {
					const V3 oN		 = dot(L, N) < 0 ? -N : N;
					float far_t		 = INFINITY;
					const V3 no		 = sane_ray(safe_position(P, L, oN), far_t);
					const uint32_t nd = depth + 1;
					if (nd < cfg.max_ray_depth) {
						alive				= true;
						ps.st[slot].ray_o		= make_float4(no.x, no.y, no.z, BOUNCE_RAY_MIN);
						ps.st[slot].ray_d		= make_float4(L.x, L.y, L.z, far_t);
						ps.st[slot].throughput = to4(throughput);
						ps.st[slot].path_pdf	= to4(path_pdf);
						ps.st[slot].prev_pdf	= to4(prev_pdf);
						if ((FEATS & FEAT_SHAPE_LIGHTS) && (sc.features & FEAT_SHAPE_LIGHTS))
							ps.st[slot].last_pos = make_float4(P.x, P.y, P.z, 0.0f);
						ps.st[slot].flags		= (flags & ~0xFFu) | nd;
						if (with_lpe)
							ps.lpe->state[slot] = lpe;
						atomicAdd(&bs.v[PRGPU_STAT_CAMERA_RAYS], 1u);
						atomicAdd(&bs.v[PRGPU_STAT_BOUNCE_RAYS], 1u);
						if (flags & FLAG_MONO)
							atomicAdd(&bs.v[PRGPU_STAT_MONOCHROME_RAYS], 1u);
					}
				}
			}
			ps.rng[pixel] = rnd;
		}
	}
}

#if PR_UNIT == PR_WAVEFRONT
__global__ void __launch_bounds__(256) k_shade(DevScene sc, PathState ps, const uint32_t* __restrict__ active, uint32_t slot_base, uint32_t n_active,
											  uint32_t* __restrict__ next_active, uint32_t* __restrict__ counters ,
											  uint32_t* __restrict__ dead_list, uint32_t* queue_head_closest, uint32_t* queue_head_shadow,
											  unsigned long long* gstats)
{
	__shared__ BlockStats bs;
	stats_init(bs);
	if (blockIdx.x == 0 && threadIdx.x == 0) {
		*queue_head_closest = 0;
		*queue_head_shadow	= 0;
	}
	const uint32_t i = blockIdx.x * blockDim.x + threadIdx.x;
	bool alive = false, want_shadow = false;
	uint32_t slot = 0;
	float4 sh_o = make_float4(0, 0, 0, 0), sh_d = sh_o, sh_xyz = sh_o;
	if (i < n_active) {
		slot = active ? active[i] : slot_base + i;
		if (ps.lpe)
			shade_vertex<FEAT_ALL>(sc, ps, slot, bs, alive, want_shadow, sh_o, sh_d, sh_xyz);
		else if (sc.features)
			shade_vertex<(FEAT_ALL & ~FEAT_LPE)>(sc, ps, slot, bs, alive, want_shadow, sh_o, sh_d, sh_xyz);
		else
			shade_vertex<0u>(sc, ps, slot, bs, alive, want_shadow, sh_o, sh_d, sh_xyz);
	}
	const uint32_t pos_next = wave_append(alive, &counters[0]);
	if (alive)
		next_active[pos_next] = slot;
	if (dead_list) {
		const bool died			= i < n_active && !alive;
		const uint32_t pos_dead = wave_append(died, &counters[2]);
		if (died)
			dead_list[pos_dead] = slot;
	}
	const uint32_t pos_sh = wave_append(want_shadow, &counters[1]);
	if (want_shadow) {
		ps.sh_o[pos_sh]	   = sh_o;
		ps.sh_d[pos_sh]	   = sh_d;
		ps.sh_xyz[pos_sh]  = sh_xyz;
		ps.sh_slot[pos_sh] = slot;
	}
	stats_flush(bs, gstats);
}

template <bool COUNT>
__global__ void __launch_bounds__(TRAV_BLOCK) k_trace_shadow(DevScene sc, PathState ps, uint32_t n, uint32_t* queue_head, uint2* spill,
															int refill_below, unsigned long long* gstats)
{
	auto load = [&](uint32_t i, V3& o, V3& d, float& tmin, float& tmax) {
		const float4 so = ps.sh_o[i], sd = ps.sh_d[i];
		o	 = v3(so.x, so.y, so.z);
		d	 = v3(sd.x, sd.y, sd.z);
		tmin = so.w;
		tmax = sd.w - 0.001f;
	};
	auto store = [&](uint32_t i, const Hit& h) {
		const float4 x		 = ps.sh_xyz[i];
		const uint32_t fbs	 = __float_as_uint(x.w);
		const uint32_t pixel = ps.pixel[ps.sh_slot[i]];
		const size_t entry	 = iter_entry(ps, ps.sh_slot[i], pixel);
		if (h.tri != INVALID) {
			const uint32_t fb = (fbs >> 8) & 0xFFu;
			if (fb)
				ps.feedback[pixel] |= fb;
		} else {
			const float xyz[3] = { x.x, x.y, x.z };
			apply_fragment(ps, pixel, entry, fbs & 0xFFu, xyz, (fbs >> 16) & 0xFu);
		}
	};
	trace_persistent<true, COUNT>(sc, n, queue_head, spill, refill_below, load, store, gstats);
}

__global__ void __launch_bounds__(256) k_resolve(DevScene sc, PathState ps, uint32_t iter)
{
	const uint32_t W = sc.cfg.width, H = sc.cfg.height;
	const uint32_t p = blockIdx.x * blockDim.x + threadIdx.x;
	if (p >= W * H)
		return;
	float acc[3];
	if (sc.single_tap) {
		acc[0] = ps.iter_xyz[3 * p];
		acc[1] = ps.iter_xyz[3 * p + 1];
		acc[2] = ps.iter_xyz[3 * p + 2];
	} else {
		const int r = (int)sc.cfg.filter_radius, dd = 2 * r + 1;
		const int x = (int)(p % W), y = (int)(p / W);
		acc[0] = acc[1] = acc[2] = 0.0f;
		for (int sy = y - r; sy <= y + r; ++sy) {
			if (sy < 0 || sy >= (int)H)
				continue;
			for (int sx = x - r; sx <= x + r; ++sx) {
				if (sx < 0 || sx >= (int)W)
					continue;
				const float fw = sc.filter[(y - sy + r) * dd + (x - sx + r)];
				if (fw > PR_EPS) {
					const uint32_t q = (uint32_t)sy * W + (uint32_t)sx;
					acc[0] += fw * ps.iter_xyz[3 * q];
					acc[1] += fw * ps.iter_xyz[3 * q + 1];
					acc[2] += fw * ps.iter_xyz[3 * q + 2];
				}
			}
		}
	}
	fold_iteration(ps, p, iter, acc);
}


#endif
#ifndef PR_PP_SLOTS_MAX
#define PR_PP_SLOTS_MAX (PP_BLOCK == 768 ? 1536 : 512)
#endif
#ifndef PR_FIN_PRIO
#define PR_FIN_PRIO 2
#endif
#ifndef PR_REFILL_PRIO
#define PR_REFILL_PRIO 2
#endif
#ifndef PR_SHADE_PRIO
#define PR_SHADE_PRIO 3
#endif
constexpr int PP_SLOTS_MAX		= PR_PP_SLOTS_MAX;
constexpr uint32_t WL_LDS		= 448;
constexpr uint32_t PP_EMPTY		= 0xFFFFFFFFu;
constexpr uint32_t PP_ANY		= 0x80000000u;
constexpr uint32_t PP_DEAD		= 0x100u;
constexpr uint32_t PP_VISIBLE	= 0x200u;
constexpr uint32_t PP_CLS_SHIFT	= 12u;
constexpr uint32_t PP_SHADOW	= 0x400u;
constexpr unsigned long long PP_IDLE_LIMIT_TICKS = 30ull * 100000000ull;

template <int NQ>
struct PPShared {
	uint2 stack[STACK_LDS * TRAV_BLOCK];
	uint32_t q_ray[2 * PP_SLOTS_MAX];
	uint32_t q_shade[NQ + 1][PP_SLOTS_MAX];
	uint32_t pending[PP_SLOTS_MAX];
	uint32_t ray_head, ray_tail, shade_head[NQ + 1], shade_tail[NQ + 1];
	float wl_cdf[WL_LDS];
	uint16_t wl_guide[CDF_GUIDE_BUCKETS + 2];
	uint32_t n_list, unit_next, exhausted, n_frozen;
	uint32_t live;
	uint32_t error;
	BlockStats bs;
};

__device__ __forceinline__ uint32_t lds_load(const uint32_t* p) { return __hip_atomic_load(p, __ATOMIC_RELAXED, __HIP_MEMORY_SCOPE_WORKGROUP); }
__device__ __forceinline__ uint32_t wave_bcast0(uint32_t v) { return (uint32_t)__builtin_amdgcn_readfirstlane((int)v); }

__device__ __forceinline__ void ring_push(uint32_t* q, uint32_t cap_mask, uint32_t* tail, bool pred, uint32_t value)
{
	const unsigned long long mask = __ballot(pred);
	if (mask == 0ull)
		return;
	const uint32_t lane = threadIdx.x & 63u;
	uint32_t base		= 0;
	const int leader	= __ffsll((long long)mask) - 1;
	if ((int)lane == leader)
		base = __hip_atomic_fetch_add(tail, (uint32_t)__popcll(mask), __ATOMIC_RELAXED, __HIP_MEMORY_SCOPE_WORKGROUP);
	base = __shfl(base, leader, 64);
	if (pred)
		__hip_atomic_store(&q[(base + __popcll(mask & ((1ull << lane) - 1ull))) & cap_mask], value, __ATOMIC_RELEASE, __HIP_MEMORY_SCOPE_WORKGROUP);
}
__device__ __forceinline__ uint32_t ring_claim(uint32_t* head, const uint32_t* tail, uint32_t want, uint32_t& first)
{
	uint32_t n = 0, h = 0;
	if ((threadIdx.x & 63u) == 0) {
		h				 = lds_load(head);
		const uint32_t t = lds_load(tail);
		n				 = min(want, t - h);
		if (n) {
			uint32_t expect = h;
			if (!__hip_atomic_compare_exchange_strong(head, &expect, h + n, __ATOMIC_RELAXED, __ATOMIC_RELAXED, __HIP_MEMORY_SCOPE_WORKGROUP))
				n = 0;
		}
	}
	first = wave_bcast0(h);
	return wave_bcast0(n);
}
__device__ __forceinline__ uint32_t ring_take(uint32_t* q, uint32_t cap_mask, uint32_t pos)
{
	uint32_t* e = &q[pos & cap_mask];
	uint32_t v;
	while ((v = __hip_atomic_load(e, __ATOMIC_ACQUIRE, __HIP_MEMORY_SCOPE_WORKGROUP)) == PP_EMPTY)
		__builtin_amdgcn_s_sleep(1);
	__hip_atomic_store(e, PP_EMPTY, __ATOMIC_RELAXED, __HIP_MEMORY_SCOPE_WORKGROUP);
	return v;
}


template <uint32_t FEATS>
__device__ __forceinline__ void apply_deferred_nee(const PathState& ps, uint32_t slot, uint32_t pw)
{
	if (pw & PP_SHADOW) {
		const float4 x		 = ps.st[slot].sh_xyz;
		const uint32_t fbs	 = __float_as_uint(x.w);
		const uint32_t pixel = ps.pixel[slot];
		if (pw & PP_VISIBLE) {
			const float xyz[3] = { x.x, x.y, x.z };
			apply_fragment(ps, pixel, iter_entry(ps, slot, pixel), fbs & 0xFFu, xyz, (FEATS & FEAT_LPE) ? (fbs >> 16) & 0xFu : 0u);
		} else if ((fbs >> 8) & 0xFFu) {
			ps.feedback[pixel] |= (fbs >> 8) & 0xFFu;
		}
	}
}

template <uint32_t FEATS>
__device__ __forceinline__ void fold_ended_sample(const PathState& ps, uint32_t slot, uint32_t pixel, uint32_t iter)
{
	if (ps.cost)
		ps.cost[pixel] += (ps.st[slot].flags & 0xFFu) + 1u;
	if (!ps.plane_stride) {
		const float v[3] = { ps.iter_xyz[3 * pixel], ps.iter_xyz[3 * pixel + 1], ps.iter_xyz[3 * pixel + 2] };
		fold_iteration(ps, pixel, iter, v, (FEATS & FEAT_LPE) != 0u);
	}
}


struct PersistentArgs {
	const uint32_t* owned;
	uint32_t n_owned;
	uint32_t* next_pixel;
	uint32_t* error;
	uint32_t slots_per_block;
	uint32_t iter_begin, iter_end;
	uint2* spill;
	int refill_below;
	uint32_t shade_min;
	uint32_t shade_partial;
	uint32_t shader_wave;
	int fin_batch;
	uint32_t direct_map;
	uint32_t resident;
	uint32_t bl_cap;
	uint32_t* bl_list;
	uint32_t* bl_word;
	uint32_t* slot_unit;
	unsigned long long* gstats;
};
constexpr uint32_t PP_SHADE_HELP = 128u;
constexpr uint32_t BL_UNWRITTEN = 0xFFFFFFFEu, BL_HOLE = 0xFFFFFFFFu;

template <bool COUNT, uint32_t FEATS, int WIDE>
__device__ __forceinline__ void path_persistent(const DevScene& sc, const PathState& ps, const PersistentArgs& a)
{
	constexpr int NQ = (FEATS & FEAT_ROUGH_MATERIALS) ? 2 : 1;
	constexpr int QR = NQ;
	constexpr uint32_t FEATS_PLAIN = FEATS & ~FEAT_ROUGH_MATERIALS;
	__shared__ PPShared<NQ> sh;
	constexpr uint32_t RAY_MASK = 2 * PP_SLOTS_MAX - 1, SHADE_MASK = PP_SLOTS_MAX - 1;
	const uint32_t lane	 = threadIdx.x & 63u;
	const uint32_t block_slots = a.slots_per_block;
	const uint32_t slot0	   = blockIdx.x * block_slots;
	for (uint32_t i = threadIdx.x; i < 2 * PP_SLOTS_MAX; i += TRAV_BLOCK)
		sh.q_ray[i] = PP_EMPTY;
	for (uint32_t i = threadIdx.x; i < PP_SLOTS_MAX; i += TRAV_BLOCK) {
		sh.q_shade[QR][i] = i < block_slots ? i : PP_EMPTY;
		for (int q = 0; q < NQ; ++q)
			sh.q_shade[q][i] = PP_EMPTY;
		sh.pending[i] = 0;
		if (i < block_slots)
			ps.pixel[slot0 + i] = INVALID;
	}
	if (threadIdx.x == 0) {
		sh.ray_head = sh.ray_tail = 0;
		for (int q = 0; q < NQ; ++q)
			sh.shade_head[q] = sh.shade_tail[q] = 0;
		sh.shade_head[QR] = 0;
		sh.shade_tail[QR] = block_slots;
		sh.live					  = block_slots;
		sh.error				  = 0;
		sh.n_list = sh.unit_next = sh.exhausted = sh.n_frozen = 0;
	}
	uint32_t* const bl_list = a.bl_list + size_t(blockIdx.x) * a.bl_cap;
	uint32_t* const bl_word = a.bl_word + size_t(blockIdx.x) * a.bl_cap;
	if (a.resident)
		for (uint32_t i = threadIdx.x; i < a.bl_cap; i += TRAV_BLOCK) {
			bl_list[i] = BL_UNWRITTEN;
			bl_word[i] = 0u;
		}
	const bool wl_in_lds = sc.wl_cdf_size >= 2u && sc.wl_cdf_size <= WL_LDS && sc.cfg.mapper == PRGPU_MAPPER_SPD_CMIS;
	if (wl_in_lds)
		for (uint32_t i = threadIdx.x; i < sc.wl_cdf_size; i += TRAV_BLOCK)
			sh.wl_cdf[i] = sc.wl_cdf[i];
	stats_init(sh.bs);
	__syncthreads();
	if (wl_in_lds) {
		for (uint32_t b = threadIdx.x; b <= CDF_GUIDE_BUCKETS; b += TRAV_BLOCK) {
			const float x = (float)b / (float)CDF_GUIDE_BUCKETS;
			int first = 0, len = (int)sc.wl_cdf_size;
			while (len > 0) {
				const int half = len / 2, middle = first + half;
				if (sh.wl_cdf[middle] <= x) {
					first = middle + 1;
					len -= half + 1;
				} else {
					len = half;
				}
			}
			sh.wl_guide[b] = (uint16_t)first;
		}
		__syncthreads();
	}
	WlTable wlt;
	if (wl_in_lds) {
		wlt.cdf	  = sh.wl_cdf;
		wlt.guide = sh.wl_guide;
	}

	Stack st;
	Trav s;
	trav_attach(s, st, sh.stack, a.spill);
	s.any			  = false;
	bool has_ray	  = false;
	uint32_t my_entry = 0;

	uint32_t spins	  = 0;
	unsigned long long t_idle_since = 0;
	uint32_t cn_c = 0, cl_c = 0, cn_a = 0, cl_a = 0, cs_c = 0, cs_a = 0, witers = 0, wleaf = 0, sbatches = 0, slanes = 0;
	unsigned long long t_shade = 0, t_idle = 0, t_leaf = 0, t_inner = 0, t_refill = 0, t_fin = 0, t_cam = 0, t_vert = 0;
	unsigned long long t_cls[4] = { 0, 0, 0, 0 };
	uint32_t b_cls[4] = { 0, 0, 0, 0 }, l_cls[4] = { 0, 0, 0, 0 };
	const unsigned long long t_start = COUNT ? wall_clock64() : 0ull;
	const unsigned long long c_start = COUNT ? (unsigned long long)clock64() : 0ull;

	const uint32_t shader_idx = 3u;
	const bool shader		  = a.shader_wave != 0u && ((threadIdx.x >> 6) & 3u) + a.shader_wave > shader_idx;
	const uint32_t shade_full = a.shader_wave != 0u ? PP_SHADE_HELP : a.shade_min;
	for (;;) {
		const int n_act	  = __popcll(__ballot(has_ray));
		uint32_t n_shade = wave_bcast0(lds_load(&sh.shade_tail[0]) - lds_load(&sh.shade_head[0]));
		int cls			 = 0;
		for (int q = 1; q < NQ + 1; ++q) {
			const uint32_t nq = wave_bcast0(lds_load(&sh.shade_tail[q]) - lds_load(&sh.shade_head[q]));
			if (nq > n_shade) {
				n_shade = nq;
				cls		= q;
			}
		}
		uint32_t n_queued = wave_bcast0(lds_load(&sh.ray_tail) - lds_load(&sh.ray_head));

		bool shade_now;
		if (shader)
			shade_now = n_shade > 0u;
		else if (a.shader_wave != 0u)
			shade_now = n_shade >= shade_full || (n_queued == 0u && n_shade > 0u && n_act == 0);
		else
			shade_now = n_shade >= a.shade_min || (n_queued == 0u && ((n_shade >= a.shade_partial && n_act < a.refill_below) || (n_shade > 0u && n_act == 0)));
		if (shade_now) {
			uint32_t first;
			const uint32_t n = ring_claim(&sh.shade_head[cls], &sh.shade_tail[cls], 64u, first);
			if (n) {
				spins			  = 0;
#if PR_SHADE_PRIO
				__builtin_amdgcn_s_setprio(PR_SHADE_PRIO);
#endif
				const unsigned long long t0 = COUNT ? wall_clock64() : 0ull;
				if (COUNT && lane == 0) {
					++sbatches;
					slanes += n;
				}
				const bool mine	  = lane < n;
				uint32_t slot_l	  = 0;
				const bool regen_pass = cls == QR;
				const bool regen	  = regen_pass;
				if (mine)
					slot_l = ring_take(sh.q_shade[cls], SHADE_MASK, first + lane);
				const uint32_t slot = slot0 + slot_l;
				if (mine)
					apply_deferred_nee<FEATS>(ps, slot, lds_load(&sh.pending[slot_l]));
				bool alive = false, want_shadow = false;
				float4 sh_o = make_float4(0, 0, 0, 0), sh_d = sh_o, sh_xyz = sh_o;
				const unsigned long long t0v = COUNT ? wall_clock64() : 0ull;
				if (regen_pass) {
				} else if (NQ > 1 && cls == 1) {
					if (mine)
						shade_vertex<FEATS>(sc, ps, slot, sh.bs, alive, want_shadow, sh_o, sh_d, sh_xyz);
				} else {
					if (mine)
						shade_vertex<FEATS_PLAIN>(sc, ps, slot, sh.bs, alive, want_shadow, sh_o, sh_d, sh_xyz);
				}
				if (COUNT)
					t_vert += wall_clock64() - t0v;
				const bool to_regen = !regen_pass && mine && !alive && !want_shadow;
				const bool ended	= mine && regen;
				bool need_pixel	 = false;
				uint32_t iter	 = 0;
				if (ended) {
					const uint32_t pixel = ps.pixel[slot];
					need_pixel			 = true;
					if (pixel != INVALID) {
						iter = ps.iter[slot];
						fold_ended_sample<FEATS>(ps, slot, pixel, iter);
						if (iter + 1 < a.iter_end) {
							if (!a.resident) {
								need_pixel = false;
								iter	   = iter + 1;
							} else {
								const uint32_t old = __hip_atomic_fetch_add(&bl_word[a.slot_unit[slot]], 1u, __ATOMIC_ACQ_REL, __HIP_MEMORY_SCOPE_WORKGROUP);
								if ((old >> 16) >= (old & 0xFFFFu) + 1u) {
									need_pixel = false;
									iter	   = iter + 1;
								}
							}
						}
					}
				}
				bool retired = false;
				if (a.resident) {
					if (wave_bcast0(lds_load(&sh.exhausted)) == 0u) {
						const unsigned long long m = __ballot(need_pixel);
						if (m != 0ull) {
							const uint32_t n	= (uint32_t)__popcll(m);
							const uint32_t rank = (uint32_t)__popcll(m & ((1ull << lane) - 1ull));
							const int leader	= __ffsll((long long)m) - 1;
							uint32_t pos		= 0;
							if ((int)lane == leader)
								pos = __hip_atomic_fetch_add(&sh.n_list, n, __ATOMIC_RELAXED, __HIP_MEMORY_SCOPE_WORKGROUP);
							pos = __shfl(pos, leader, 64);
							const uint32_t n_fit = pos >= a.bl_cap ? 0u : min(n, a.bl_cap - pos);
							uint32_t idx		 = a.n_owned;
							if (n_fit != 0u) {
								__builtin_amdgcn_fence(__ATOMIC_SEQ_CST, "workgroup");
								if ((int)lane == leader)
									idx = atomicAdd(a.next_pixel, n_fit);
								idx = __shfl(idx, leader, 64);
							}
							if ((n_fit < n || idx + n_fit >= a.n_owned) && (int)lane == leader)
								__hip_atomic_store(&sh.exhausted, 1u, __ATOMIC_RELEASE, __HIP_MEMORY_SCOPE_WORKGROUP);
							if (need_pixel && rank < n_fit) {
								const uint32_t i = idx + rank;
								uint32_t entry	 = BL_HOLE;
								if (i < a.n_owned) {
									entry				= a.owned[i];
									ps.pixel[slot]		= entry;
									a.slot_unit[slot]	= pos + rank;
									iter				= a.iter_begin;
									need_pixel			= false;
								}
								__hip_atomic_store(&bl_list[pos + rank], entry, __ATOMIC_RELEASE, __HIP_MEMORY_SCOPE_WORKGROUP);
							}
						}
					}
					const uint32_t rounds = a.iter_end - a.iter_begin - 1u;
					while (__any(need_pixel)) {
						uint32_t nf = lds_load(&sh.n_frozen);
						if (nf == 0u) {
							if (lane == 0) {
								uint32_t expect = 0u;
								(void)__hip_atomic_compare_exchange_strong(&sh.n_frozen, &expect, min(lds_load(&sh.n_list), a.bl_cap) + 1u, __ATOMIC_RELAXED, __ATOMIC_RELAXED,
																		   __HIP_MEMORY_SCOPE_WORKGROUP);
							}
							nf = lds_load(&sh.n_frozen);
						}
						const uint32_t N		   = wave_bcast0(nf) - 1u;
						const unsigned long long total = (unsigned long long)N * rounds;
						const unsigned long long m = __ballot(need_pixel);
						const uint32_t rank		   = (uint32_t)__popcll(m & ((1ull << lane) - 1ull));
						const int leader		   = __ffsll((long long)m) - 1;
						uint32_t u0				   = 0;
						if ((int)lane == leader)
							u0 = __hip_atomic_fetch_add(&sh.unit_next, (uint32_t)__popcll(m), __ATOMIC_RELAXED, __HIP_MEMORY_SCOPE_WORKGROUP);
						u0 = __shfl(u0, leader, 64);
						if (need_pixel) {
							const uint32_t u = u0 + rank;
							if (u >= total) {
								retired	   = true;
								need_pixel = false;
							} else {
								const uint32_t k = u % N;
								uint32_t p;
								while ((p = __hip_atomic_load(&bl_list[k], __ATOMIC_ACQUIRE, __HIP_MEMORY_SCOPE_WORKGROUP)) == BL_UNWRITTEN)
									__builtin_amdgcn_s_sleep(1);
								if (p != BL_HOLE) {
									const uint32_t old = __hip_atomic_fetch_add(&bl_word[k], 1u << 16, __ATOMIC_ACQ_REL, __HIP_MEMORY_SCOPE_WORKGROUP);
									const uint32_t r   = (old >> 16) + 1u;
									if ((old & 0xFFFFu) >= r) {
										ps.pixel[slot]	  = p;
										a.slot_unit[slot] = k;
										iter			  = a.iter_begin + r;
										need_pixel		  = false;
									}
								}
							}
						}
					}
				} else {
					uint32_t idx;
					if (a.direct_map)
						idx = need_pixel && ps.pixel[slot] == INVALID ? slot : a.n_owned;
					else
						idx = wave_append(need_pixel, a.next_pixel);
					if (need_pixel) {
						if (idx < a.n_owned) {
							ps.pixel[slot] = a.owned[idx];
							iter		   = a.iter_begin;
						} else {
							retired = true;
						}
					}
				}
				const unsigned long long t0c = COUNT ? wall_clock64() : 0ull;
				if (ended && !retired) {
					ps.iter[slot] = iter;
					camera_path(sc, ps, slot, iter, sh.bs, (FEATS & FEAT_LPE) != 0u, wlt);
					alive = true;
				}
				if (COUNT)
					t_cam += wall_clock64() - t0c;
				const int n_retired = __popcll(__ballot(retired));
				if (n_retired && lane == 0)
					__hip_atomic_fetch_sub(&sh.live, (uint32_t)n_retired, __ATOMIC_RELAXED, __HIP_MEMORY_SCOPE_WORKGROUP);
				if (mine && !retired) {
					if (want_shadow) {
						ps.st[slot].sh_o	= sh_o;
						ps.st[slot].sh_d	= sh_d;
						ps.st[slot].sh_xyz = sh_xyz;
					}
					__hip_atomic_store(&sh.pending[slot_l], (alive ? 1u : 0u) + (want_shadow ? 1u + PP_SHADOW : 0u) + (alive ? 0u : PP_DEAD), __ATOMIC_RELAXED,
									   __HIP_MEMORY_SCOPE_WORKGROUP);
				}
				ring_push(sh.q_shade[QR], SHADE_MASK, &sh.shade_tail[QR], to_regen, slot_l);
				ring_push(sh.q_ray, RAY_MASK, &sh.ray_tail, want_shadow, slot_l | PP_ANY);
				ring_push(sh.q_ray, RAY_MASK, &sh.ray_tail, alive, slot_l);
				{
					const uint32_t pslot = slot0 + (has_ray ? (my_entry & ~PP_ANY) : 0u);
					const bool pany		 = has_ray && (my_entry & PP_ANY) != 0;
					const float4 ro = pany ? ps.st[pslot].sh_o : ps.st[pslot].ray_o, rd = pany ? ps.st[pslot].sh_d : ps.st[pslot].ray_d;
					s.r	   = ray_prepare(v3(ro.x, ro.y, ro.z), v3(rd.x, rd.y, rd.z), sc.eps_t);
					s.tmin = ro.w + 0.0f;
					s.any  = pany;
				}
#if PR_SHADE_PRIO
				__builtin_amdgcn_s_setprio(0);
#endif
				if (COUNT)
					t_shade += wall_clock64() - t0;
				if (COUNT && lane == 0)
					for (int q = 0; q < NQ + 1; ++q)
						if (q == cls) {
							t_cls[q] += wall_clock64() - t0;
							b_cls[q] += 1u;
							l_cls[q] += n;
						}
			}
			continue;
		}

		const unsigned long long idle = __ballot(!has_ray);
		if (!shader && idle != 0ull && n_queued > 0u) {
#if PR_REFILL_PRIO
			__builtin_amdgcn_s_setprio(PR_REFILL_PRIO);
#endif
			const unsigned long long t0r = COUNT ? wall_clock64() : 0ull;
			uint32_t first;
			const uint32_t n = ring_claim(&sh.ray_head, &sh.ray_tail, (uint32_t)__popcll(idle), first);
			const uint32_t r = __popcll(idle & ((1ull << lane) - 1ull));
			if (!has_ray && r < n) {
				my_entry			= ring_take(sh.q_ray, RAY_MASK, first + r);
				const uint32_t slot = slot0 + (my_entry & ~PP_ANY);
				const bool any		= (my_entry & PP_ANY) != 0;
				const float4 ro = any ? ps.st[slot].sh_o : ps.st[slot].ray_o, rd = any ? ps.st[slot].sh_d : ps.st[slot].ray_d;
				trav_begin(s, st, v3(ro.x, ro.y, ro.z), v3(rd.x, rd.y, rd.z), ro.w, any ? rd.w - 0.001f : rd.w, sc.eps_t);
				s.any	= any;
				has_ray = true;
				if (FEATS & FEAT_QUADRICS)
					trav_quadrics<(NQ > 1)>(sc, s, any);
			}
#if PR_REFILL_PRIO
			__builtin_amdgcn_s_setprio(0);
#endif
			if (COUNT)
				t_refill += wall_clock64() - t0r;
		}
		if (!__any(has_ray)) {
			if (lds_load(&sh.live) == 0u || lds_load(&sh.error) != 0u)
				break;
			const unsigned long long t0 = COUNT ? wall_clock64() : 0ull;
			__builtin_amdgcn_s_sleep(8);
			if (COUNT)
				t_idle += wall_clock64() - t0;
			if (n_shade == 0u && n_queued == 0u) {
				if (spins++ == 0u)
					t_idle_since = wall_clock64();
				else if ((spins & 1023u) == 0u && wall_clock64() - t_idle_since > PP_IDLE_LIMIT_TICKS) {
					if (lane == 0) {
						__hip_atomic_store(&sh.error, 1u, __ATOMIC_RELAXED, __HIP_MEMORY_SCOPE_WORKGROUP);
						atomicExch(a.error, 1u);
					}
					break;
				}
			}
			continue;
		}
		spins = 0;
		unsigned long long m_has  = lane_ballot(has_ray);
		unsigned long long m_wait = m_has & lane_ballot(s.cur == REC_EMPTY);
		for (;;) {
			const unsigned long long m_lb	 = lane_ballot((s.cur & REC_LEAF_BIT) != 0u);
			const unsigned long long m_leaf	 = m_has & m_lb & ~m_wait;
			const unsigned long long m_inner = m_has & ~m_lb;
			const int n_leaf = wave_popc(m_leaf), n_inner = wave_popc(m_inner);
			if (COUNT && lane == 0)
				++witers;
			const bool do_inner = n_inner >= n_leaf;
			const unsigned long long t0s = COUNT ? wall_clock64() : 0ull;
			if (lane_in(do_inner ? m_inner : m_leaf)) {
				const float4* __restrict__ rec = rec_ptr(sc.recs, s.cur);
				const float4 q0 = rec[0], q1 = rec[1], q2 = rec[2];
				const bool wide = WIDE == 2 ? sc.bvh_wide != 0u : WIDE == 1;
				float4 qw		= make_float4(0.0f, 0.0f, 0.0f, 0.0f);
				if (wide && do_inner)
					qw = rec[3];
				const uint2 top_e	   = PR_PEEK ? st.peek() : make_uint2(0u, 0u);
				const uint2* const top = PR_PEEK ? &top_e : nullptr;
				if (do_inner) {
					if (COUNT) {
						cn_c += s.any ? 0 : 1;
						cn_a += s.any ? 1 : 0;
					}
					trav_inner_rec<MODE_MIXED>(s, st, q0, q1, q2, qw, wide, top);
				} else {
					float4 q3 = make_float4(0.0f, 0.0f, 0.0f, 0.0f), q4 = q3, q5 = q3, q6 = q3, q7 = q3;
					if (!(s.cur & REC_SINGLE_BIT)) {
						q3 = rec[3];
						q4 = rec[4];
						q5 = rec[5];
						q6 = rec[6];
						q7 = rec[7];
					}
					if (COUNT) {
						cl_c += s.any ? 0 : 1;
						cl_a += s.any ? 1 : 0;
						if (s.cur & REC_SINGLE_BIT) {
							cs_c += s.any ? 0 : 1;
							cs_a += s.any ? 1 : 0;
						}
					}
					trav_leaf_rec<MODE_MIXED, (FEATS & ANA_ALL), (NQ > 1)>(s, st, q0, q1, q2, q3, q4, q5, q6, q7, top);
				}
			}
			if (COUNT) {
				if (do_inner)
					t_inner += wall_clock64() - t0s;
				else
					t_leaf += wall_clock64() - t0s;
			}
			const unsigned long long m_done = m_has & lane_ballot(s.cur == REC_EMPTY);
			unsigned long long m_fin		= m_done;
			if (a.fin_batch > 1) {
				const int n_done = wave_popc(m_done);
				const int n_run	 = wave_popc(m_has & ~m_done);
				if (n_done < a.fin_batch && n_run >= a.refill_below)
					m_fin = 0ull;
			}
			const unsigned long long t0f = COUNT ? wall_clock64() : 0ull;
			if (m_fin != 0ull) {
// ... 527 lines not shown
	hipLaunchKernelGGL(k_service_closest, trav_grid(ws, n), dim3(TRAV_BLOCK), 0, st, sc, n, org, dir, tmin, tmax, entity, prim, u, v, t, ws.queue_head,
					   ws.spill, ws.refill_below, gstats);
}
void launch_tri_slot(const DevScene& sc, const uint32_t* leaf_units, uint32_t* tri_slot, hipStream_t st)
{
	if (sc.n_leaf)
		hipLaunchKernelGGL(k_tri_slot, grid_for(sc.n_leaf), dim3(256), 0, st, sc, leaf_units, tri_slot);
}
void launch_service_closest_split(const DevScene& sc, uint32_t n, const float* org, const float* dir, const float* tmin, const float* tmax,
								  uint32_t* entity, uint32_t* prim, float* u, float* v, float* t, const TraceWorkspace& ws, uint32_t* tri_slot,
								  unsigned long long* gstats, bool leaf_single, hipStream_t st)
{
	(void)hipMemsetAsync(ws.queue_head, 0, sizeof(uint32_t), st);
	if (sc.bvh_wide)
		hipLaunchKernelGGL(k_service_closest_split<true>, trav_grid(ws, n), dim3(TRAV_BLOCK), 0, st, sc, n, org, dir, tmin, tmax, entity, prim, u, v, t, ws.queue_head,
						   ws.spill, tri_slot, ws.refill_below, gstats, leaf_single);
	else
		hipLaunchKernelGGL(k_service_closest_split<false>, trav_grid(ws, n), dim3(TRAV_BLOCK), 0, st, sc, n, org, dir, tmin, tmax, entity, prim, u, v, t, ws.queue_head,
						   ws.spill, tri_slot, ws.refill_below, gstats, leaf_single);
}
void launch_service_any(const DevScene& sc, uint32_t n, const float* org, const float* dir, const float* tmin, const float* distance,
						uint8_t* occluded, const TraceWorkspace& ws, unsigned long long* gstats, hipStream_t st)
{
	(void)hipMemsetAsync(ws.queue_head, 0, sizeof(uint32_t), st);
	hipLaunchKernelGGL(k_service_any, trav_grid(ws, n), dim3(TRAV_BLOCK), 0, st, sc, n, org, dir, tmin, distance, occluded, ws.queue_head, ws.spill,
					   ws.refill_below, gstats);
}
void launch_ao_hits(const DevScene& sc, const PathState& ps, const AoState& ao, uint32_t n_slots, bool instrumented, uint32_t* n_hits, uint32_t* queue_head_closest,
					uint32_t* queue_head_ao, unsigned long long* gstats, hipStream_t st)
{
	if (instrumented)
		hipLaunchKernelGGL(k_ao_hits<true>, grid_for(n_slots), dim3(256), 0, st, sc, ps, ao, n_slots, n_hits, queue_head_closest, queue_head_ao, gstats);
	else
		hipLaunchKernelGGL(k_ao_hits<false>, grid_for(n_slots), dim3(256), 0, st, sc, ps, ao, n_slots, n_hits, queue_head_closest, queue_head_ao, gstats);
}
void launch_ao_occlusion(const DevScene& sc, const PathState& ps, const AoState& ao, uint32_t n_slots, bool instrumented, const uint32_t* n_hits, const TraceWorkspace& ws,
						 unsigned long long* gstats, hipStream_t st)
{
	const dim3 g = trav_grid(ws, n_slots * ao.sample_count);
	if (instrumented)
		hipLaunchKernelGGL(k_ao_occlusion<true>, g, dim3(TRAV_BLOCK), 0, st, sc, ps, ao, n_hits, ws.queue_head, ws.spill, ws.refill_below, gstats);
	else
		hipLaunchKernelGGL(k_ao_occlusion<false>, g, dim3(TRAV_BLOCK), 0, st, sc, ps, ao, n_hits, ws.queue_head, ws.spill, ws.refill_below, gstats);
}
void launch_ao_splat(const DevScene& sc, const PathState& ps, const AoState& ao, uint32_t n_slots, const uint32_t* n_hits, hipStream_t st)
{
	hipLaunchKernelGGL(k_ao_splat, grid_for(n_slots), dim3(256), 0, st, sc, ps, ao, n_hits);
}
bool ao_counts_folded() { return PR_AO_FOLD != 0; }
void launch_vf_shade(const DevScene& sc, const PathState& ps, const VfState& vf, uint32_t n_slots, uint32_t* queue_head_closest, unsigned long long* gstats, hipStream_t st)
{
	hipLaunchKernelGGL(k_vf_shade, grid_for(n_slots), dim3(256), 0, st, sc, ps, vf, n_slots, queue_head_closest, gstats);
}

#endif

template <int VARIANT, int SUB>
void launch_pp(const DevScene& sc, const PathState& ps, const PersistentArgs& a, dim3 grid, hipStream_t st);
template <int VARIANT, int SUB>
void launch_pl(const DevScene& sc, const PathState& ps, const WaveArgs& a, dim3 grid, hipStream_t st);
#if PR_UNIT != PR_WAVEFRONT
#if !defined(PR_VARIANT) || !defined(PR_SUB)
#error "compile the persistent-kernel units with -DPR_VARIANT=<id of a row of PATH_VARIANTS> -DPR_SUB=<index>"
#endif
static_assert(path_variant_row(PR_VARIANT) < N_PATH_VARIANTS, "PR_VARIANT is not the id of a row of PATH_VARIANTS");
#if PR_UNIT == PR_LATENCY
template <int VARIANT, int SUB>
void launch_pl(const DevScene& sc, const PathState& ps, const WaveArgs& a, dim3 grid, hipStream_t st)
{
	static_assert(SUB == 0 || SUB == 1, "latency units: PR_SUB=0 (plain) or 1 (instrumented)");
	hipLaunchKernelGGL((k_path_latency<SUB != 0, PATH_VARIANTS[path_variant_row(VARIANT)].features>), grid, dim3(TRAV_BLOCK), 0, st, sc, ps, a);
}
template void launch_pl<PR_VARIANT, PR_SUB>(const DevScene&, const PathState&, const WaveArgs&, dim3, hipStream_t);
#else
template <int VARIANT, int SUB>
void launch_pp(const DevScene& sc, const PathState& ps, const PersistentArgs& a, dim3 grid, hipStream_t st)
{
	constexpr PathSub u		 = PATH_SUBS[SUB];
	constexpr uint32_t FEATS = PATH_VARIANTS[path_variant_row(VARIANT)].features;
	const dim3 block(TRAV_BLOCK);
	if constexpr (u.occupancy == 3)
		hipLaunchKernelGGL((k_path_persistent_occ3<u.count, FEATS, u.wide>), grid, block, 0, st, sc, ps, a);
	else
		hipLaunchKernelGGL((k_path_persistent<u.count, FEATS>), grid, block, 0, st, sc, ps, a);
}
template void launch_pp<PR_VARIANT, PR_SUB>(const DevScene&, const PathState&, const PersistentArgs&, dim3, hipStream_t);
#endif
#endif

#if PR_UNIT == PR_WAVEFRONT
PersistentGeometry persistent_geometry(uint32_t n_owned, uint32_t max_blocks, uint32_t max_slots_per_block)
{
	PersistentGeometry g;
	const uint32_t per_block = (n_owned + max_blocks - 1) / std::max(1u, max_blocks);
	const uint32_t cap		 = std::min((uint32_t)PP_SLOTS_MAX, std::max(256u, max_slots_per_block / 64u * 64u));
	g.slots_per_block		 = std::min(cap, std::max(64u, per_block));
	g.n_blocks				 = std::max(1u, std::min(max_blocks, (n_owned + g.slots_per_block - 1) / g.slots_per_block));
	return g;
}
uint32_t persistent_slot_padding() { return PP_SLOTS_MAX; }
uint32_t slot_array_padding() { return std::max<uint32_t>(PP_SLOTS_MAX, (TRAV_BLOCK / 64u) * PW_SLOTS_MAX); }
uint32_t persistent_block_threads() { return PP_BLOCK; }
int shade_ticks_counter() { return CNT_SHADE_TICKS; }

typedef void (*PpLaunchFn)(const DevScene&, const PathState&, const PersistentArgs&, dim3, hipStream_t);
typedef void (*PlLaunchFn)(const DevScene&, const PathState&, const WaveArgs&, dim3, hipStream_t);
template <int... I>
constexpr std::array<PpLaunchFn, sizeof...(I)> pp_launch_table(std::integer_sequence<int, I...>)
{
	return { { launch_pp<PATH_VARIANTS[I / N_PATH_SUBS].id, I % N_PATH_SUBS>... } };
}
constexpr bool pl_variant_built(int row) { return ((PR_PL_VARIANTS >> (PATH_VARIANTS[row].id - 1)) & 1u) != 0u; }
template <int ROW, int SUB>
constexpr PlLaunchFn pl_launcher()
{
	if constexpr (pl_variant_built(ROW))
		return launch_pl<PATH_VARIANTS[ROW].id, SUB>;
	else
		return nullptr;
}
template <int... I>
constexpr std::array<PlLaunchFn, sizeof...(I)> pl_launch_table(std::integer_sequence<int, I...>)
{
	return { { pl_launcher<I / 2, I % 2>()... } };
}

void launch_path_persistent(const DevScene& sc, const PathState& ps, const uint32_t* owned, uint32_t n_owned, uint32_t iter_begin, uint32_t iter_end,
							bool count, const TraceWorkspace& ws, const PersistentTuning& tune, int shader_waves, uint32_t* next_pixel, uint32_t* error,
							unsigned long long* gstats, hipStream_t st)
{
	const uint32_t max_slots_per_block = tune.slots;
	const PersistentGeometry g = persistent_geometry(n_owned, ws.max_blocks, max_slots_per_block);
	const bool all_in_flight   = uint64_t(g.n_blocks) * g.slots_per_block >= n_owned;
	PersistentArgs a;
	a.owned			  = owned;
	a.n_owned		  = n_owned;
	a.next_pixel	  = next_pixel;
	a.error			  = error;
	a.slots_per_block = g.slots_per_block;
	a.iter_begin	  = iter_begin;
	a.iter_end		  = iter_end;
	a.spill			  = ws.spill;
	a.refill_below	  = ws.refill_below;
	a.shade_min		  = (uint32_t)std::min(64, std::max(1, tune.shade_min));
	a.shade_partial	  = (uint32_t)std::min(64, std::max(1, tune.shade_partial));
	a.shader_wave	  = PP_BLOCK == 256 ? (uint32_t)std::min(2, std::max(0, shader_waves)) : (shader_waves ? 1u : 0u);
	a.gstats		  = gstats;
	a.direct_map	  = all_in_flight ? 1u : 0u;
	a.fin_batch		  = std::min(64, std::max(1, tune.fin_batch));
	const bool resident_ok = tune.resident;
	a.bl_cap		  = (uint32_t)std::min<uint64_t>(n_owned, 2ull * ((n_owned + g.n_blocks - 1) / g.n_blocks) + 1024ull);
	a.bl_list		  = ws.bl_list;
	a.bl_word		  = ws.bl_word;
	a.slot_unit		  = ws.slot_unit;
	a.resident		  = resident_ok && !all_in_flight && iter_end - iter_begin >= 2u && iter_end - iter_begin < 65536u && ws.bl_list != nullptr
						&& uint64_t(a.bl_cap) * g.n_blocks <= ws.bl_entries && uint64_t(a.bl_cap) * (iter_end - iter_begin) < (1ull << 31)
					  ? 1u
					  : 0u;
	if (!a.resident)
		a.bl_cap = 0;
	(void)hipMemsetAsync(next_pixel, 0, sizeof(uint32_t), st);
	const dim3 grid(g.n_blocks);
	static constexpr auto table = pp_launch_table(std::make_integer_sequence<int, N_PATH_VARIANTS * N_PATH_SUBS>{});
	table[path_variant(sc.features) * N_PATH_SUBS + path_sub(tune.occupancy, sc.bvh_wide != 0u, count)](sc, ps, a, grid, st);
}

LatencyGeometry latency_geometry(uint32_t n_owned, uint32_t max_blocks_throughput, uint32_t max_slots_per_wave)
{
	LatencyGeometry g;
	const uint32_t waves_per_block = TRAV_BLOCK / 64u;
	const uint32_t max_blocks	   = std::max(1u, max_blocks_throughput * 2u / 3u);
	const uint32_t max_waves	   = max_blocks * waves_per_block;
	const uint32_t cap			   = std::min((uint32_t)PW_SLOTS_MAX, std::max(64u, max_slots_per_wave / 64u * 64u));
	uint32_t spw = ((n_owned + max_waves - 1u) / max_waves + 63u) / 64u * 64u;
	spw			 = std::min(cap, std::max(64u, spw));
	g.slots_per_wave = spw;
	const uint32_t waves = std::max(1u, std::min(max_waves, (n_owned + spw - 1u) / spw));
	g.n_blocks			 = (waves + waves_per_block - 1u) / waves_per_block;
	g.total_slots		 = g.n_blocks * waves_per_block * spw;
	return g;
}
bool latency_variant_built(uint32_t features)
{
	return pl_variant_built(path_variant(features));
}
void launch_path_latency(const DevScene& sc, const PathState& ps, const uint32_t* owned, uint32_t n_owned, uint32_t iter_begin, uint32_t iter_end, bool count,
						 const TraceWorkspace& ws, const LatencyTuning& tune, uint32_t* error, unsigned long long* gstats, hipStream_t st)
{
	const LatencyGeometry g = latency_geometry(n_owned, ws.max_blocks, tune.slots_per_wave);
	WaveArgs a;
	a.owned			 = owned;
	a.n_owned		 = n_owned;
	a.error			 = error;
	a.slots_per_wave = g.slots_per_wave;
	a.total_slots	 = g.total_slots;
	a.iter_begin	 = iter_begin;
	a.iter_end		 = iter_end;
	a.spill			 = ws.spill;
	a.slot_index	 = ws.slot_unit;
	a.refill_below	 = std::min(64, std::max(1, tune.refill_below));
	a.shade_min		 = (uint32_t)std::min(64, std::max(1, tune.shade_min));
	a.gstats		 = gstats;
	static constexpr auto table = pl_launch_table(std::make_integer_sequence<int, N_PATH_VARIANTS * 2>{});
	if (PlLaunchFn fn = table[path_variant(sc.features) * 2 + (count ? 1 : 0)])
		fn(sc, ps, a, dim3(g.n_blocks), st);
}

uint32_t trace_stack_capacity() { return (uint32_t)(STACK_LDS + STACK_SPILL); }
size_t trace_workspace_spill_entries(uint32_t max_blocks) { return size_t(max_blocks) * std::max(TRAV_BLOCK, PP_BLOCK) * STACK_SPILL; }
#endif

}
```

pearray_amd/csrc/prgpu_api.hip:

```cpp
#include <hip/hip_runtime.h>
#include <dlfcn.h>

#include <algorithm>
#include <climits>
#include <cmath>
#include <cstdlib>
#include <cstring>
#include <map>
#include <string>
#include <vector>

#include "../../include/prgpu.h"
#include "device/bvh.h"
#include "device/render.h"
#include "host/setup.h"
#include "tables/pr_vf_colors.inl"
static_assert(sizeof(PR_VF_COLOR_RGB) / sizeof(PR_VF_COLOR_RGB[0]) == prd::VF_COLOURS, "one row per colour index of device/render.h");

namespace {

thread_local std::string g_error;

int fail(int code, const std::string& msg)
{
// ... 7 lines not shown
		if (_e != hipSuccess)                                                                               \
			return fail(PRGPU_EDEVICE, std::string(#expr) + " failed: " + hipGetErrorString(_e));           \
	} while (0)

}
namespace prgpu_host {
int set_last_error(int code, const std::string& msg) { return fail(code, msg); }
}
namespace {

constexpr int KNOB_INVALID = INT_MIN;
struct Knobs {
	int mode = -1;
	prd::PersistentTuning pp;
	bool pp_slots_set		   = false;
	int pp_kernel			   = 0;
	prd::LatencyTuning pl;
	int pp_refill			   = 48;
	int pp_blocks_per_cu	   = 0;
	int pp_max_blocks		   = 0;
	int pp_planes			   = 8;
	uint64_t pp_launch_samples = 128ull << 20;
	int pp_launch_min_iters	   = 8;
	bool pp_tune_order		   = true;
	int groups				   = 1;
	bool sort_rays			   = false;
	bool trace_split		   = true;
	bool comm_force_rccl	   = false;
	uint32_t force_features	   = 0;
	bool debug_counters		   = false;
	const char* dump_block_life = nullptr;
	int bvh_width			   = 0;
	int bvh_top				   = -1;
	int bvh_leaf			   = 0;
	int bvh_parity			   = -1;
};
Knobs read_knobs()
{
	auto num = [](const char* name, long long def, long long lo, long long hi) -> long long {
		const char* env = getenv(name);
		return env ? std::min(hi, std::max(lo, atoll(env))) : def;
	};
	auto choice = [](const char* name, std::initializer_list<std::pair<const char*, int>> choices, int def) -> int {
		const char* env = getenv(name);
		if (!env)
			return def;
		for (const auto& c : choices)
			if (std::strcmp(env, c.first) == 0)
				return c.second;
		return KNOB_INVALID;
	};
	Knobs k;
	k.mode		 = choice("PRGPU_MODE", { { "lockstep", 0 }, { "streaming", 1 }, { "persistent", 2 } }, k.mode);
	k.pp_kernel	 = choice("PRGPU_PP_KERNEL", { { "auto", 0 }, { "throughput", 1 }, { "latency", 2 } }, k.pp_kernel);
	k.bvh_width	 = choice("PRGPU_BVH_WIDTH", { { "auto", 0 }, { "4", 4 }, { "6", 6 } }, k.bvh_width);
	k.bvh_top	 = choice("PRGPU_BVH_TOP", { { "auto", -1 }, { "file", 0 }, { "area", 1 }, { "morton", 2 } }, k.bvh_top);
	k.bvh_leaf	 = choice("PRGPU_BVH_LEAF", { { "auto", 0 }, { "3", 3 }, { "1", 1 } }, k.bvh_leaf);
	k.bvh_parity = choice("PRGPU_BVH_PARITY", { { "auto", -1 }, { "even", 0 }, { "odd", 1 } }, k.bvh_parity);
	k.pl.slots_per_wave	  = (uint32_t)num("PRGPU_PL_SLOTS", k.pl.slots_per_wave, 64, 256);
	k.pl.shade_min		  = (int)num("PRGPU_PL_SHADE_MIN", k.pl.shade_min, 1, 64);
	k.pl.refill_below	  = (int)num("PRGPU_PL_REFILL", k.pl.refill_below, 1, 64);
	k.pp_slots_set		  = getenv("PRGPU_PP_SLOTS") != nullptr;
	k.pp.slots			  = (uint32_t)num("PRGPU_PP_SLOTS", k.pp.slots, 256, prd::persistent_slot_padding());
	k.pp.shade_min		  = (int)num("PRGPU_PP_SHADE_MIN", k.pp.shade_min, 1, 64);
	k.pp.shade_partial	  = (int)num("PRGPU_PP_SHADE_PARTIAL", k.pp.shade_partial, 1, 64);
	k.pp.fin_batch		  = (int)num("PRGPU_PP_FIN_BATCH", k.pp.fin_batch, 1, 64);
	k.pp.occupancy		  = (int)num("PRGPU_PP_OCCUPANCY", k.pp.occupancy, 2, 3);
	k.pp.shader_wave	  = (int)num("PRGPU_PP_SHADER", k.pp.shader_wave, -1, 2);
	k.pp.resident		  = num("PRGPU_PP_RESIDENT", 1, 0, 1) != 0;
	k.pp_refill			  = (int)num("PRGPU_PP_REFILL", k.pp_refill, 1, 64);
	k.pp_blocks_per_cu	  = (int)num("PRGPU_PP_BLOCKS_PER_CU", 0, 0, 8);
	k.pp_max_blocks		  = (int)num("PRGPU_PP_MAX_BLOCKS", 0, 0, 1 << 20);
	k.pp_planes			  = (int)num("PRGPU_PP_PLANES", k.pp_planes, 1, 64);
	k.pp_launch_samples	  = (uint64_t)num("PRGPU_PP_LAUNCH_SAMPLES", (long long)k.pp_launch_samples, 1, 1ll << 40);
	k.pp_launch_min_iters = (int)num("PRGPU_PP_LAUNCH_MIN_ITERS", k.pp_launch_min_iters, 1, 1 << 15);
	k.pp_tune_order		  = num("PRGPU_PP_TUNE_ORDER", 1, 0, 1) != 0;
	k.groups			  = (int)num("PRGPU_GROUPS", k.groups, 1, 16);
	k.sort_rays			  = num("PRGPU_SORT_RAYS", 0, 0, 1) != 0;
	k.trace_split		  = num("PRGPU_TRACE_SPLIT", 1, 0, 1) != 0;
	k.comm_force_rccl	  = num("PRGPU_COMM_FORCE_RCCL", 0, 0, 1) != 0;
	if (const char* env = getenv("PRGPU_FORCE_FEATURES"))
		k.force_features = (uint32_t)strtoul(env, nullptr, 0);
	k.debug_counters  = getenv("PRGPU_DEBUG_COUNTERS") != nullptr;
	k.dump_block_life = getenv("PRGPU_DUMP_BLOCK_LIFE");
	return k;
}

struct TraceRange {
	typedef int (*PushFn)(const char*);
	typedef int (*PopFn)();
	static PushFn& push_fn() { static PushFn f = nullptr; return f; }
	static PopFn& pop_fn() { static PopFn f = nullptr; return f; }
	static bool bind()
	{
		static const bool bound = [] {
			for (const char* name : { "librocprofiler-sdk-roctx.so.1", "librocprofiler-sdk-roctx.so", "libroctx64.so.4", "libroctx64.so" }) {
				void* lib = dlopen(name, RTLD_NOW | RTLD_LOCAL | RTLD_NOLOAD);
				if (!lib)
					continue;
				push_fn() = reinterpret_cast<PushFn>(dlsym(lib, "roctxRangePushA"));
				pop_fn()  = reinterpret_cast<PopFn>(dlsym(lib, "roctxRangePop"));
				if (push_fn() && pop_fn())
					return true;
				push_fn() = nullptr;
				pop_fn()  = nullptr;
				dlclose(lib);
			}
			return false;
		}();
		return bound;
	}
	bool active;
	explicit TraceRange(const char* name) : active(bind()) { if (active) (void)push_fn()(name); }
	~TraceRange() { if (active) (void)pop_fn()(); }
	TraceRange(const TraceRange&) = delete;
	TraceRange& operator=(const TraceRange&) = delete;
};

struct TimedLaunch {
	hipEvent_t start, stop;
	int family;
};
enum Family { FAM_RAYGEN, FAM_TRACE_CLOSEST, FAM_SHADE, FAM_TRACE_ANY, FAM_RESOLVE, FAM_SORT, FAM_PATH, FAM_REDUCE, FAM_AO, FAM_VF, N_FAMILIES };
const char* const FAMILY_NAMES[] = { "raygen", "trace_closest", "shade", "trace_any", "resolve", "sort", "path", "reduce", "ao", "vf" };
static_assert(sizeof(FAMILY_NAMES) / sizeof(FAMILY_NAMES[0]) == N_FAMILIES, "one name per timing family");

}

struct prgpu_scene {
	int device = 0;
	hipStream_t own_stream = nullptr, stream = nullptr;
	prd::DevScene sc{};
	prd::PathState ps{};
	prgpu_settings cfg{};
	uint32_t n_pixels = 0, n_slots = 0;
	std::vector<void*> allocations;
	uint32_t bvh_units = 0;
	uint32_t bvh_stack_bound = 0, bvh_top = 0;
	int bvh_leaf = 3;
	float bvh_cost4 = 0.0f, bvh_cost6 = 0.0f;
	int pp_shader_waves = -1;
	double pp_shading_share = 0.0;
	uint64_t pp_launches = 0;
	int pp_calibration_tries = 0;
	unsigned long long *gstats_before = nullptr, *gstats_after = nullptr;
	uint32_t pp_last_blocks = 0, pp_last_slots = 0, pp_last_kernel = 0;
	float* own_xyz = nullptr;
	uint32_t *own_samples = nullptr, *own_feedback = nullptr;
	uint32_t *active_a = nullptr, *active_b = nullptr, *dead_a = nullptr, *dead_b = nullptr;
	enum Mode { LOCKSTEP, STREAMING, PERSISTENT };
	Mode mode = LOCKSTEP;
	Knobs knobs;
	uint32_t pp_planes = 1;
	uint32_t *pp_pixel = nullptr, *pp_next = nullptr, *pp_error = nullptr;
	unsigned long long* gstats = nullptr;
	prd::TraceWorkspace ws;
	prd::TraceWorkspace ws_pp;
	struct Group {
		hipStream_t s_main = nullptr, s_shadow = nullptr;
		hipEvent_t ev_shade = nullptr, ev_shadow = nullptr;
		uint32_t slot_begin = 0, n_slots = 0;
		uint32_t *active_a = nullptr, *active_b = nullptr, *counters = nullptr, *h_counters = nullptr;
		uint32_t *dead_a = nullptr, *dead_b = nullptr;
		uint32_t *dead_cur = nullptr, *dead_prev = nullptr;
		uint32_t *sort_keys_a = nullptr, *sort_keys_b = nullptr, *sort_active = nullptr;
		void* sort_temp = nullptr;
		size_t sort_temp_bytes = 0;
		uint32_t n_dead_prev = 0;
		prd::TraceWorkspace ws_closest, ws_shadow;
		prd::PathState ps;
		const uint32_t* active = nullptr;
		uint32_t* next = nullptr;
		uint32_t n_active = 0, depth = 0;
		bool done = true, shadow_pending = false;
	};
	std::vector<Group> groups;
	hipEvent_t ev_resolve = nullptr;
	bool resolve_recorded = false;
	bool instrument = false, timing = false;
	std::vector<TimedLaunch> pending;
	double family_ms[N_FAMILIES] = { 0 };
	uint64_t family_launches[N_FAMILIES] = { 0 };
	uint64_t rays_closest = 0, rays_any = 0;
	uint32_t next_iteration = 0;
	bool ao_enabled = false;
	prd::AoState ao{};
	bool vf_enabled = false;
	prd::VfState vf{};
	prd::TraceWorkspace ws_ao;
	std::vector<prgpu_tile> tiles;
	prd::DevLpe lpe_host{};
	uint32_t order_tuned_at = 0;
	bool poisoned = false;
	uint32_t reduced_at = 0xFFFFFFFFu;
	struct Reduced {
		float* xyz = nullptr;
		uint32_t *samples = nullptr, *feedback = nullptr;
		float *online_mean = nullptr, *online_variance = nullptr;
		float* aov[PRGPU_AOV_COUNT] = {};
		std::vector<float*> lpe;
		bool valid = false;
	} reduced;

	template <typename T>
	int alloc(T*& ptr, size_t count, bool zero = false)
	{
		void* p = nullptr;
		HIP_TRY(hipMalloc(&p, std::max<size_t>(count, 1) * sizeof(T)));
		allocations.push_back(p);
		ptr = static_cast<T*>(p);
		if (zero)
			HIP_TRY(hipMemsetAsync(p, 0, std::max<size_t>(count, 1) * sizeof(T), stream));
		return PRGPU_OK;
	}
	template <typename T>
	int upload(const T*& ptr, const T* src, size_t count)
	{
		T* p = nullptr;
		const int rc = alloc(p, count);
		if (rc != PRGPU_OK)
			return rc;
		if (count)
			HIP_TRY(hipMemcpyAsync(p, src, count * sizeof(T), hipMemcpyHostToDevice, stream));
		ptr = p;
		return PRGPU_OK;
	}
	template <typename T>
	int upload(const T*& ptr, const std::vector<T>& v)
	{
		return upload(ptr, v.data(), v.size());
	}

	void time_begin(Family family, hipStream_t st)
	{
		if (!timing)
			return;
		TimedLaunch t;
		t.family = family;
		(void)hipEventCreate(&t.start);
		(void)hipEventCreate(&t.stop);
		(void)hipEventRecord(t.start, st);
		pending.push_back(t);
	}
	void time_end(hipStream_t st)
	{
		if (!timing)
			return;
		(void)hipEventRecord(pending.back().stop, st);
	}
	void collect_timing()
	{
		for (TimedLaunch& t : pending) {
			float ms = 0;
			if (hipEventSynchronize(t.stop) == hipSuccess && hipEventElapsedTime(&ms, t.start, t.stop) == hipSuccess) {
				family_ms[t.family] += ms;
				family_launches[t.family] += 1;
			}
			(void)hipEventDestroy(t.start);
			(void)hipEventDestroy(t.stop);
		}
		pending.clear();
	}
};

namespace {

int apply_tiles(prgpu_scene* s, const prgpu_tile* tiles, uint32_t n_tiles)
{
	for (uint32_t i = 0; i < n_tiles; ++i)
		if (tiles[i].x1 > s->cfg.width || tiles[i].y1 > s->cfg.height || tiles[i].x0 > tiles[i].x1 || tiles[i].y0 > tiles[i].y1)
			return fail(PRGPU_EINVAL, "tile outside the film");
	std::vector<uint32_t> pixels;
	if (tiles != s->tiles.data())
		s->tiles.assign(tiles, tiles + n_tiles);
	prgpu_host::owned_pixels_morton(s->cfg.width, s->cfg.height, tiles, n_tiles, pixels);
	s->n_slots = (uint32_t)pixels.size();
	{
		const uint32_t g = s->mode == prgpu_scene::PERSISTENT && uint64_t(s->n_slots) <= uint64_t(s->ws_pp.max_blocks) * s->knobs.pp.slots ? 4u : 0u;
		const uint32_t n_groups = g ? s->n_slots / g : 0u;
		if (n_groups > 2) {
			uint32_t stride = (uint32_t)(n_groups * 0.6180339887) | 1u;
			auto gcd = [](uint32_t a, uint32_t b) { while (b) { const uint32_t t = a % b; a = b; b = t; } return a; };
			while (gcd(stride, n_groups) != 1)
				stride += 2;
			std::vector<uint32_t> out(pixels);
			for (uint32_t i = 0; i < n_groups; ++i) {
				const uint32_t src = (uint32_t)((uint64_t(i) * stride) % n_groups);
				std::copy(pixels.begin() + size_t(src) * g, pixels.begin() + size_t(src + 1) * g, out.begin() + size_t(i) * g);
			}
			pixels.swap(out);
		}
	}
	if (!pixels.empty())
		HIP_TRY(hipMemcpyAsync(s->ps.pixel, pixels.data(), pixels.size() * 4, hipMemcpyHostToDevice, s->stream));
	HIP_TRY(hipStreamSynchronize(s->stream));
	const uint32_t G	 = (uint32_t)s->groups.size();
	const uint32_t chunk = ((s->n_slots + G - 1) / G + 255u) / 256u * 256u;
	for (uint32_t g = 0; g < G; ++g) {
		prgpu_scene::Group& gr = s->groups[g];
		gr.slot_begin = std::min(s->n_slots, g * chunk);
		gr.n_slots	  = std::min(s->n_slots, (g + 1) * chunk) - gr.slot_begin;
		gr.active_a	  = s->active_a + gr.slot_begin;
		gr.active_b	  = s->active_b + gr.slot_begin;
		gr.dead_a	  = s->dead_a + gr.slot_begin;
		gr.dead_b	  = s->dead_b + gr.slot_begin;
		gr.ps		  = s->ps;
		gr.ps.sh_o += gr.slot_begin;
// ... 175 lines not shown
	if (!t.shape_lights.empty())
		UP(sc.shape_lights, t.shape_lights);
	sc.quadrics	  = nullptr;
	sc.n_quadrics = (uint32_t)t.quadrics.size();
	if (!t.quadrics.empty())
		UP(sc.quadrics, t.quadrics);
	sc.features		 = d->n_lights ? prd::FEAT_INFINITE_LIGHTS : 0u;
	if (!t.quadrics.empty())
		sc.features |= prd::FEAT_QUADRICS;
	if (!t.shape_lights.empty())
		sc.features |= prd::FEAT_SHAPE_LIGHTS;
	for (uint32_t i = 0; i < d->n_spectra; ++i)
		if (d->spectra[i].kind == PRGPU_SPEC_CHECKER)
			sc.features |= prd::FEAT_TEXTURES;
		else if (d->spectra[i].kind == PRGPU_SPEC_IMAGE)
			sc.features |= prd::FEAT_TEXTURES | prd::FEAT_IMAGES;
	if (has_expr)
		sc.features |= prd::FEAT_EXPR;
	for (uint32_t e = 0; e < d->n_entities; ++e)
		if (d->entities[e].has_uvs && d->uvs && d->entities[e].kind == PRGPU_ENTITY_MESH)
			sc.features |= prd::FEAT_TEXTURES;
	for (uint32_t i = 0; i < d->n_materials; ++i) {
		const uint32_t kind = d->materials[i].kind;
		if (kind == PRGPU_MAT_DIELECTRIC || kind == PRGPU_MAT_CONDUCTOR || kind == PRGPU_MAT_MIRROR)
			sc.features |= prd::FEAT_DELTA_MATERIALS;
		else if (kind == PRGPU_MAT_OREN_NAYAR || kind == PRGPU_MAT_NULL || kind == PRGPU_MAT_BLEND || kind == PRGPU_MAT_ADD)
			sc.features |= prd::FEAT_MIX_MATERIALS;
		else if (kind != PRGPU_MAT_LAMBERT)
			sc.features |= prd::FEAT_DELTA_MATERIALS | prd::FEAT_ROUGH_MATERIALS;
	}
	for (uint32_t e = 0; e < d->n_entities; ++e)
		if (d->entities[e].kind == PRGPU_ENTITY_PLANE)
			sc.features |= prd::FEAT_PLANES;
		else if (d->entities[e].kind == PRGPU_ENTITY_SPHERE)
			sc.features |= prd::FEAT_SPHERES;
		else if (d->entities[e].kind == PRGPU_ENTITY_DISK)
			sc.features |= prd::FEAT_DISKS;
	sc.features |= read_knobs().force_features & prd::FEAT_ALL & ~(prd::FEAT_LPE | prd::FEAT_QUADRICS | prd::FEAT_DISKS | prd::FEAT_IMAGES | prd::FEAT_MIX_MATERIALS | prd::FEAT_EXPR);
	sc.scene_radius	 = t.scene_radius;
	sc.wl_cdf_size	 = (uint32_t)t.wl_cdf.size();
	sc.wl_u_offset	 = t.wl_u_offset;
	sc.wl_u_scale	 = t.wl_u_scale;
	sc.agh_c		 = t.agh_c;
	sc.agh_n		 = t.agh_n;
	sc.rr_size		 = (uint32_t)t.rr_prob.size();
	sc.cam			 = t.cam;
	sc.cfg			 = d->settings;
	sc.spp			 = t.spp;
	sc.mj_x			 = t.mj_x;
	sc.mj_y			 = t.mj_y;
	sc.mj_seed		 = t.mj_seed;
	sc.halton_bx	 = t.halton_bx;
	sc.halton_by	 = t.halton_by;
	sc.halton_burnin = t.halton_burnin;
	sc.single_tap	 = t.single_tap;
	sc.centre_weight = t.centre_weight;
	sc.eps_t		 = t.eps_t;
	if (!(t.coord_scale <= prd::SCENE_COORD_MAX))
		return fail(PRGPU_EINVAL, "scene coordinates must be finite and at most 2^28 in magnitude (the BVH's quantisation grid)");
	sc.n_tris		 = d->n_triangles;

	prd::BvhBuildInput bin{ d->n_triangles, d->n_entities, sc.positions, sc.indices, sc.tri_entity, sc.entities, sc.tri_class };
	if (s->knobs.bvh_width == KNOB_INVALID)
		return fail(PRGPU_EINVAL, "PRGPU_BVH_WIDTH must be auto, 4 or 6");
	if (s->knobs.bvh_top == KNOB_INVALID)
		return fail(PRGPU_EINVAL, "PRGPU_BVH_TOP must be auto, file, area or morton");
	if (s->knobs.bvh_parity == KNOB_INVALID)
		return fail(PRGPU_EINVAL, "PRGPU_BVH_PARITY must be auto, even or odd");
	if (s->knobs.bvh_leaf == KNOB_INVALID)
		return fail(PRGPU_EINVAL, "PRGPU_BVH_LEAF must be auto, 3 or 1");
	bin.leaf = s->knobs.bvh_leaf;
	bin.width = s->knobs.bvh_width;
	bin.top	  = s->knobs.bvh_top;
	bin.parity = s->knobs.bvh_parity;
	bin.stack_capacity = prd::trace_stack_capacity();
	prd::BvhBuildOutput bout;
	{
		TraceRange bvh_range("prgpu_scene_create: LBVH build");
		if (!prd::build_lbvh(bin, bout, s->stream, err))
			return fail(PRGPU_EDEVICE, "LBVH build failed: " + err);
	}
	s->allocations.push_back(bout.recs);
	if (bout.leaf_units)
		s->allocations.push_back(bout.leaf_units);
	sc.recs	   = bout.recs;
	sc.n_inner = bout.n_inner;
	sc.bvh_wide = bout.wide ? 1u : 0u;
	s->bvh_cost4 = bout.cost4;
	s->bvh_cost6 = bout.cost6;
	s->bvh_leaf	 = bout.leaf;
	if (s->knobs.debug_counters)
		fprintf(stderr, "[prgpu] BVH leaf policy %d (PRGPU_BVH_LEAF=%s): price %.3f with 128-byte leaves, %.3f with single leaves (0 = not built); the built tree: %.2f inner, %.2f 128-byte-leaf, %.2f single-leaf records expected per ray through the scene's box\n",
				bout.leaf, s->knobs.bvh_leaf == 0 ? "auto" : (s->knobs.bvh_leaf == 1 ? "1" : "3"), bout.price3, bout.price1, bout.visits[0], bout.visits[1], bout.visits[2]);
	s->bvh_stack_bound = bout.stack_bound;
	s->bvh_top = (uint32_t)bout.top;
	sc.n_leaf  = bout.n_leaf;
	s->bvh_units = bout.n_units;
	{
		uint32_t* map = nullptr;
		const int rc2 = s->alloc(map, std::max<size_t>(1, d->n_triangles), true);
		if (rc2 != PRGPU_OK)
			return rc2;
		prd::launch_tri_slot(sc, bout.leaf_units, map, s->stream);
		sc.tri_slot = map;
	}

	const uint32_t np = d->settings.width * d->settings.height;
	s->n_pixels		  = np;
	prd::PathState& ps = s->ps;
#define AL(ptr, count, zero)                      \
	do {                                          \
		rc = s->alloc(ptr, count, zero);          \
		if (rc != PRGPU_OK)                       \
			return rc;                            \
	} while (0)
	const size_t ns = size_t(np) + prd::slot_array_padding();
	AL(ps.rng, np, false);
	HIP_TRY(hipMemcpyAsync(ps.rng, t.rng.data(), size_t(np) * 8, hipMemcpyHostToDevice, s->stream));
	AL(ps.pixel, np, false);
	AL(ps.st, ns, false);
	AL(ps.sh_o, ns, false);
	AL(ps.sh_d, ns, false);
	AL(ps.sh_xyz, ns, false);
	AL(ps.sh_slot, ns, false);
	s->pp_planes = t.single_tap ? 1u : (uint32_t)s->knobs.pp_planes;
	AL(ps.iter_xyz, size_t(np) * 3 * s->pp_planes, true);
	ps.plane_stride = 0;
	ps.iter_base	= 0;
	AL(s->own_xyz, size_t(np) * 3, true);
	AL(s->own_samples, np, true);
	AL(s->own_feedback, np, true);
	AL(ps.prim_entity, np, false);
	AL(ps.prim_prim, np, false);
	HIP_TRY(hipMemsetAsync(ps.prim_entity, 0xFF, size_t(np) * 4, s->stream));
	HIP_TRY(hipMemsetAsync(ps.prim_prim, 0xFF, size_t(np) * 4, s->stream));
	ps.out_xyz	= s->own_xyz;
	ps.samples	= s->own_samples;
	ps.feedback = s->own_feedback;
	AL(s->active_a, np, false);
	AL(s->active_b, np, false);
	AL(s->dead_a, np, false);
	AL(s->dead_b, np, false);
	AL(ps.iter, ns, true);
	AL(ps.cost, np, true);
	s->mode = prgpu_scene::PERSISTENT;
	if (s->knobs.mode == KNOB_INVALID)
		return fail(PRGPU_EINVAL, "PRGPU_MODE must be lockstep, streaming or persistent");
	if (s->knobs.pp_kernel == KNOB_INVALID)
		return fail(PRGPU_EINVAL, "PRGPU_PP_KERNEL must be auto, throughput or latency");
	if (s->knobs.mode == 0)
		s->mode = prgpu_scene::LOCKSTEP;
	else if (s->knobs.mode == 1)
		s->mode = t.single_tap ? prgpu_scene::STREAMING : prgpu_scene::LOCKSTEP;
	AL(s->pp_pixel, ns, false);
	AL(s->pp_next, 1, true);
	AL(s->pp_error, 1, true);
	AL(s->gstats, prd::N_DEVICE_COUNTERS, true);
	AL(s->gstats_before, prd::N_DEVICE_COUNTERS, true);
	AL(s->gstats_after, prd::N_DEVICE_COUNTERS, true);
	{
		hipDeviceProp_t prop;
		HIP_TRY(hipGetDeviceProperties(&prop, device));
		const uint32_t blocks_per_cu = 2;
		const int refill			 = 44;
		const uint32_t max_blocks = (uint32_t)std::max(1, prop.multiProcessorCount) * blocks_per_cu;
		auto make_ws = [&](prd::TraceWorkspace& w, uint32_t n_blocks) -> int {
			w.max_blocks   = n_blocks;
			w.refill_below = refill;
			AL(w.queue_head, 1, true);
			AL(w.spill, prd::trace_workspace_spill_entries(n_blocks), false);
			return PRGPU_OK;
		};
		rc = make_ws(s->ws, (uint32_t)std::max(1, prop.multiProcessorCount) * 3u);
		if (rc != PRGPU_OK)
			return rc;
		{
			uint32_t pp_blocks_per_cu = 768u / prd::persistent_block_threads();
			if (!s->knobs.pp_slots_set)
				s->knobs.pp.slots = prd::PersistentTuning().slots * (prd::persistent_block_threads() / 256u);
			if (s->knobs.pp_blocks_per_cu)
				pp_blocks_per_cu = (uint32_t)s->knobs.pp_blocks_per_cu;
			s->ws_pp.max_blocks = (uint32_t)std::max(1, prop.multiProcessorCount) * pp_blocks_per_cu;
			if (s->knobs.pp_max_blocks)
				s->ws_pp.max_blocks = std::min(s->ws_pp.max_blocks, (uint32_t)s->knobs.pp_max_blocks);
			s->ws_pp.refill_below = s->knobs.pp_refill;
			AL(s->ws_pp.spill, prd::trace_workspace_spill_entries(s->ws_pp.max_blocks), false);
			s->ws_pp.bl_entries = 2 * size_t(np) + size_t(s->ws_pp.max_blocks) * 1026u;
			AL(s->ws_pp.bl_list, s->ws_pp.bl_entries, false);
			AL(s->ws_pp.bl_word, s->ws_pp.bl_entries, false);
			AL(s->ws_pp.slot_unit, ns, false);
		}
		if (rc != PRGPU_OK)
			return rc;
		uint32_t n_groups = (uint32_t)s->knobs.groups;
		if (np < 64u * 1024u)
			n_groups = 1;
		s->groups.resize(n_groups);
		HIP_TRY(hipEventCreateWithFlags(&s->ev_resolve, hipEventDisableTiming));
		for (uint32_t g = 0; g < n_groups; ++g) {
			prgpu_scene::Group& gr = s->groups[g];
			if (g == 0)
				gr.s_main = s->stream;
			else
				HIP_TRY(hipStreamCreateWithFlags(&gr.s_main, hipStreamNonBlocking));
			HIP_TRY(hipStreamCreateWithFlags(&gr.s_shadow, hipStreamNonBlocking));
			HIP_TRY(hipEventCreateWithFlags(&gr.ev_shade, hipEventDisableTiming));
			HIP_TRY(hipEventCreateWithFlags(&gr.ev_shadow, hipEventDisableTiming));
			AL(gr.counters, 4, true);
			HIP_TRY(hipHostMalloc(reinterpret_cast<void**>(&gr.h_counters), 4 * sizeof(uint32_t), hipHostMallocDefault));
			rc = make_ws(gr.ws_closest, max_blocks);
			if (rc != PRGPU_OK)
				return rc;
			rc = make_ws(gr.ws_shadow, max_blocks);
			if (rc != PRGPU_OK)
				return rc;
		}
	}
	HIP_TRY(hipStreamSynchronize(s->stream));
	return apply_tiles(s, nullptr, 0);
}

int enqueue_vertex(prgpu_scene* s, prgpu_scene::Group& g)
{
	hipStream_t st = g.s_main;
	const bool sort_rays = s->knobs.sort_rays;
	if (sort_rays && g.active != nullptr && g.n_active > 0) {
		if (!g.sort_temp) {
			int rc = s->alloc(g.sort_keys_a, g.n_slots);
			rc	   = rc == PRGPU_OK ? s->alloc(g.sort_keys_b, g.n_slots) : rc;
			rc	   = rc == PRGPU_OK ? s->alloc(g.sort_active, g.n_slots) : rc;
			if (rc != PRGPU_OK)
				return rc;
			g.sort_temp_bytes = prd::sort_active_temp_bytes(g.n_slots);
			unsigned char* tmp = nullptr;
			rc = s->alloc(tmp, g.sort_temp_bytes);
			if (rc != PRGPU_OK)
				return rc;
			g.sort_temp = tmp;
		}
		s->time_begin(FAM_SORT, st);
		prd::launch_sort_active(s->sc, g.ps, g.active, g.n_active, g.sort_keys_a, g.sort_keys_b, g.sort_active, g.sort_temp, g.sort_temp_bytes, st);
		s->time_end(st);
		g.active = g.sort_active;
	}
	s->time_begin(FAM_TRACE_CLOSEST, st);
	prd::launch_trace_closest(s->sc, g.ps, g.active, g.slot_begin, g.n_active, s->instrument, g.ws_closest, g.counters, s->gstats, st);
	s->time_end(st);
	s->rays_closest += g.n_active;
	if (g.shadow_pending) {
		HIP_TRY(hipStreamWaitEvent(st, g.ev_shadow, 0));
		g.shadow_pending = false;
	}
	s->time_begin(FAM_SHADE, st);
	prd::launch_shade(s->sc, g.ps, g.active, g.slot_begin, g.n_active, g.next, g.counters, nullptr, g.ws_closest.queue_head, g.ws_shadow.queue_head,
					  s->gstats, st);
	s->time_end(st);
	HIP_TRY(hipMemcpyAsync(g.h_counters, g.counters, 3 * sizeof(uint32_t), hipMemcpyDeviceToHost, st));
	HIP_TRY(hipEventRecord(g.ev_shade, st));
	return PRGPU_OK;
}

int render_iteration(prgpu_scene* s, uint32_t iter)
{
	uint32_t running = 0;
	for (auto& g : s->groups) {
		g.done = true;
		if (!g.n_slots)
			continue;
		if (s->resolve_recorded && g.s_main != s->stream)
			HIP_TRY(hipStreamWaitEvent(g.s_main, s->ev_resolve, 0));
		s->time_begin(FAM_RAYGEN, g.s_main);
		prd::launch_raygen(s->sc, g.ps, g.slot_begin, g.n_slots, iter, s->gstats, g.s_main);
		s->time_end(g.s_main);
		g.active		 = nullptr;
		g.next			 = g.active_a;
		g.n_active		 = g.n_slots;
		g.depth			 = 0;
		g.done			 = false;
		g.shadow_pending = false;
		const int rc = enqueue_vertex(s, g);
		if (rc != PRGPU_OK)
			return rc;
		++running;
	}
	while (running) {
		bool progress = false;
		for (auto& g : s->groups) {
			if (g.done)
				continue;
			const hipError_t q = hipEventQuery(g.ev_shade);
			if (q == hipErrorNotReady)
				continue;
			if (q != hipSuccess)
				return fail(PRGPU_EDEVICE, std::string("hipEventQuery failed: ") + hipGetErrorString(q));
			progress				= true;
			const uint32_t n_next	= g.h_counters[0];
			const uint32_t n_shadow = g.h_counters[1];
			if (n_shadow) {
				HIP_TRY(hipStreamWaitEvent(g.s_shadow, g.ev_shade, 0));
				s->time_begin(FAM_TRACE_ANY, g.s_shadow);
				prd::launch_trace_shadow(s->sc, g.ps, n_shadow, s->instrument, g.ws_shadow, s->gstats, g.s_shadow);
				s->time_end(g.s_shadow);
				HIP_TRY(hipEventRecord(g.ev_shadow, g.s_shadow));
				g.shadow_pending = true;
				s->rays_any += n_shadow;
			}
			g.active = g.next;
			g.next	 = (g.next == g.active_a) ? g.active_b : g.active_a;
			g.n_active = n_next;
			g.depth += 1;
			if (g.n_active > 0 && g.depth < s->cfg.max_ray_depth) {
				const int rc = enqueue_vertex(s, g);
				if (rc != PRGPU_OK)
					return rc;
			} else {
				g.done = true;
				--running;
			}
		}
		if (!progress) {
			for (auto& g : s->groups)
				if (!g.done) {
					HIP_TRY(hipEventSynchronize(g.ev_shade));
					break;
				}
		}
	}
	for (auto& g : s->groups) {
		if (!g.n_slots)
			continue;
		if (g.shadow_pending) {
			HIP_TRY(hipStreamWaitEvent(s->stream, g.ev_shadow, 0));
			g.shadow_pending = false;
		}
		if (g.s_main != s->stream)
			HIP_TRY(hipStreamWaitEvent(s->stream, g.ev_shade, 0));
	}
	s->time_begin(FAM_RESOLVE, s->stream);
	prd::launch_resolve(s->sc, s->ps, iter, s->stream);
	s->time_end(s->stream);
	if (s->ps.lpe) {
		prd::PathState pl  = s->ps;
		pl.online_mean	   = nullptr;
// ... 56 lines not shown
	HIP_TRY(hipGetLastError());
	return PRGPU_OK;
}

int render_vf_iteration(prgpu_scene* s, uint32_t iter)
{
	if (!s->n_slots)
		return PRGPU_OK;
	hipStream_t st		   = s->stream;
	prgpu_scene::Group& g0 = s->groups[0];
	s->time_begin(FAM_RAYGEN, st);
	prd::launch_raygen(s->sc, s->ps, 0, s->n_slots, iter, s->gstats, st);
	s->time_end(st);
	s->time_begin(FAM_TRACE_CLOSEST, st);
	prd::launch_trace_closest(s->sc, s->ps, nullptr, 0, s->n_slots, s->instrument, g0.ws_closest, g0.counters, s->gstats, st);
	s->time_end(st);
	s->time_begin(FAM_VF, st);
	prd::launch_vf_shade(s->sc, s->ps, s->vf, s->n_slots, g0.ws_closest.queue_head, s->gstats, st);
	s->time_end(st);
	s->time_begin(FAM_RESOLVE, st);
	prd::launch_resolve(s->sc, s->ps, iter, st);
	s->time_end(st);
	HIP_TRY(hipGetLastError());
	return PRGPU_OK;
}

int enqueue_round(prgpu_scene* s, prgpu_scene::Group& g, uint32_t iter_end)
{
	hipStream_t st = g.s_main;
	if (g.n_active) {
		s->time_begin(FAM_TRACE_CLOSEST, st);
		prd::launch_trace_closest(s->sc, g.ps, g.active, g.slot_begin, g.n_active, s->instrument, g.ws_closest, g.counters, s->gstats, st);
		s->time_end(st);
		s->rays_closest += g.n_active;
	} else {
		HIP_TRY(hipMemsetAsync(g.counters, 0, 3 * sizeof(uint32_t), st));
	}
	if (g.shadow_pending) {
		HIP_TRY(hipStreamWaitEvent(st, g.ev_shadow, 0));
		g.shadow_pending = false;
	}
	if (g.n_active) {
		s->time_begin(FAM_SHADE, st);
		prd::launch_shade(s->sc, g.ps, g.active, g.slot_begin, g.n_active, g.next, g.counters, g.dead_cur, g.ws_closest.queue_head,
						  g.ws_shadow.queue_head, s->gstats, st);
		s->time_end(st);
	}
	if (g.n_dead_prev) {
		s->time_begin(FAM_RAYGEN, st);
		prd::launch_regen(s->sc, g.ps, g.dead_prev, g.n_dead_prev, iter_end, g.next, g.counters, s->gstats, st);
		s->time_end(st);
	}
	HIP_TRY(hipMemcpyAsync(g.h_counters, g.counters, 3 * sizeof(uint32_t), hipMemcpyDeviceToHost, st));
	HIP_TRY(hipEventRecord(g.ev_shade, st));
	return PRGPU_OK;
}

int render_streaming(prgpu_scene* s, uint32_t iter_begin, uint32_t iter_end)
{
	uint32_t running = 0;
	for (auto& g : s->groups) {
		g.done = true;
		if (!g.n_slots)
			continue;
		s->time_begin(FAM_RAYGEN, g.s_main);
		prd::launch_raygen(s->sc, g.ps, g.slot_begin, g.n_slots, iter_begin, s->gstats, g.s_main);
		s->time_end(g.s_main);
		g.active		 = nullptr;
		g.next			 = g.active_a;
		g.n_active		 = g.n_slots;
		g.dead_cur		 = g.dead_a;
		g.dead_prev		 = g.dead_b;
		g.n_dead_prev	 = 0;
		g.done			 = false;
		g.shadow_pending = false;
		const int rc = enqueue_round(s, g, iter_end);
		if (rc != PRGPU_OK)
			return rc;
		++running;
	}
	while (running) {
		bool progress = false;
		for (auto& g : s->groups) {
			if (g.done)
				continue;
			const hipError_t q = hipEventQuery(g.ev_shade);
			if (q == hipErrorNotReady)
				continue;
			if (q != hipSuccess)
				return fail(PRGPU_EDEVICE, std::string("hipEventQuery failed: ") + hipGetErrorString(q));
			progress				= true;
			const uint32_t n_next	= g.h_counters[0];
			const uint32_t n_shadow = g.h_counters[1];
			const uint32_t n_dead	= g.n_active ? g.h_counters[2] : 0;
			if (n_shadow && g.n_active) {
				HIP_TRY(hipStreamWaitEvent(g.s_shadow, g.ev_shade, 0));
				s->time_begin(FAM_TRACE_ANY, g.s_shadow);
				prd::launch_trace_shadow(s->sc, g.ps, n_shadow, s->instrument, g.ws_shadow, s->gstats, g.s_shadow);
				s->time_end(g.s_shadow);
				HIP_TRY(hipEventRecord(g.ev_shadow, g.s_shadow));
				g.shadow_pending = true;
				s->rays_any += n_shadow;
			}
			g.active	  = g.next;
			g.next		  = (g.next == g.active_a) ? g.active_b : g.active_a;
			g.n_active	  = n_next;
			std::swap(g.dead_cur, g.dead_prev);
			g.n_dead_prev = n_dead;
			if (g.n_active > 0 || g.n_dead_prev > 0) {
				const int rc = enqueue_round(s, g, iter_end);
				if (rc != PRGPU_OK)
					return rc;
			} else {
				g.done = true;
				--running;
			}
		}
		if (!progress) {
			for (auto& g : s->groups)
				if (!g.done) {
					HIP_TRY(hipEventSynchronize(g.ev_shade));
					break;
				}
		}
	}
	for (auto& g : s->groups) {
		if (!g.n_slots)
			continue;
		if (g.shadow_pending) {
			HIP_TRY(hipStreamWaitEvent(s->stream, g.ev_shadow, 0));
			g.shadow_pending = false;
		}
		if (g.s_main != s->stream)
			HIP_TRY(hipStreamWaitEvent(s->stream, g.ev_shade, 0));
	}
	HIP_TRY(hipGetLastError());
	return PRGPU_OK;
}

bool use_latency_kernel(const prgpu_scene* s)
{
	if (s->knobs.pp_kernel == 1 || prd::persistent_block_threads() != 256u || !prd::latency_variant_built(s->sc.features))
		return false;
	if (s->knobs.pp_kernel == 2)
		return true;
	return false;
}

int render_persistent(prgpu_scene* s, uint32_t iter_begin, uint32_t iter_end)
{
	if (!s->n_slots)
		return PRGPU_OK;
	prd::PathState ps = s->ps;
	ps.pixel		  = s->pp_pixel;
	const uint64_t per_iter = std::max<uint64_t>(1, s->n_slots);
	uint32_t chunk			= (uint32_t)std::min<uint64_t>(1u << 15, std::max<uint64_t>((uint64_t)s->knobs.pp_launch_min_iters, s->knobs.pp_launch_samples / per_iter));
	const bool all_in_flight = uint64_t(s->n_slots) <= uint64_t(s->ws_pp.max_blocks) * s->knobs.pp.slots;
	const bool latency = use_latency_kernel(s);
	const bool calibrating = s->knobs.pp.shader_wave < 0 && !all_in_flight && !latency;
	auto decide = [&]() -> int {
		if (!calibrating || s->pp_shader_waves >= 0 || s->pp_calibration_tries == 0)
			return PRGPU_OK;
		HIP_TRY(hipStreamSynchronize(s->stream));
		unsigned long long t0[3] = { 0, 0, 0 }, t1[3] = { 0, 0, 0 };
		HIP_TRY(hipMemcpy(t0, s->gstats_before + prd::shade_ticks_counter(), sizeof(t0), hipMemcpyDeviceToHost));
		HIP_TRY(hipMemcpy(t1, s->gstats_after + prd::shade_ticks_counter(), sizeof(t1), hipMemcpyDeviceToHost));
		const unsigned long long shading = t1[0] - t0[0], alive = t1[2] - t0[2];
		if (alive == 0ull && s->pp_calibration_tries < 3)
			return PRGPU_OK;
		const double share	= alive > 0ull ? double(shading) / double(alive) : 0.0;
		s->pp_shader_waves	= share >= 0.22 ? (share >= 0.45 ? 2 : 1) : 0;
		s->pp_shading_share = share;
		if (s->knobs.debug_counters)
			fprintf(stderr, "[prgpu] shading passes took %.1f %% of the calibration launch's wave time: %d dedicated shading wave(s) per block from now on\n", 100.0 * share, s->pp_shader_waves);
		return PRGPU_OK;
	};
	if (latency ? prd::latency_geometry(s->n_slots, s->ws_pp.max_blocks, s->knobs.pl.slots_per_wave).total_slots < s->n_slots : !all_in_flight)
		ps.cost = nullptr;
	const bool ring			= !s->sc.single_tap;
	if (ring) {
		chunk			= std::min(chunk, s->pp_planes);
		ps.plane_stride = 3u * s->n_pixels;
	}
	for (uint32_t b = iter_begin; b < iter_end;) {
		const int rc_decide = decide();
		if (rc_decide != PRGPU_OK)
			return rc_decide;
		const bool calibration = calibrating && s->pp_shader_waves < 0;
		const uint32_t e	   = (uint32_t)std::min<uint64_t>(iter_end, uint64_t(b) + (calibration ? std::min(chunk, 8u) : chunk));
		const int shader_wave  = s->knobs.pp.shader_wave >= 0 ? s->knobs.pp.shader_wave : (all_in_flight ? 1 : std::max(0, s->pp_shader_waves));
		ps.iter_base = b;
		const size_t gbytes = sizeof(unsigned long long) * prd::N_DEVICE_COUNTERS;
		if (calibration)
			HIP_TRY(hipMemcpyAsync(s->gstats_before, s->gstats, gbytes, hipMemcpyDeviceToDevice, s->stream));
		s->time_begin(FAM_PATH, s->stream);
		if (latency)
			prd::launch_path_latency(s->sc, ps, s->ps.pixel, s->n_slots, b, e, s->instrument, s->ws_pp, s->knobs.pl, s->pp_error, s->gstats, s->stream);
		else
			prd::launch_path_persistent(s->sc, ps, s->ps.pixel, s->n_slots, b, e, s->instrument || calibration, s->ws_pp, s->knobs.pp, shader_wave, s->pp_next, s->pp_error, s->gstats, s->stream);
		s->time_end(s->stream);
		HIP_TRY(hipGetLastError());
		if (calibration) {
			HIP_TRY(hipMemcpyAsync(s->gstats_after, s->gstats, gbytes, hipMemcpyDeviceToDevice, s->stream));
			if (!s->instrument)
				HIP_TRY(hipMemcpyAsync(s->gstats + PRGPU_STAT_COUNT, s->gstats_before + PRGPU_STAT_COUNT, gbytes - sizeof(unsigned long long) * PRGPU_STAT_COUNT, hipMemcpyDeviceToDevice, s->stream));
			++s->pp_calibration_tries;
		}
		++s->pp_launches;
		if (latency) {
			const prd::LatencyGeometry g = prd::latency_geometry(s->n_slots, s->ws_pp.max_blocks, s->knobs.pl.slots_per_wave);
			s->pp_last_blocks = g.n_blocks;
			s->pp_last_slots  = g.slots_per_wave * (prd::persistent_block_threads() / 64u);
			s->pp_last_kernel = PRGPU_KERNEL_LATENCY;
		} else {
			const prd::PersistentGeometry g = prd::persistent_geometry(s->n_slots, s->ws_pp.max_blocks, s->knobs.pp.slots);
			s->pp_last_blocks = g.n_blocks;
			s->pp_last_slots  = g.slots_per_block;
			s->pp_last_kernel = PRGPU_KERNEL_THROUGHPUT;
		}
		if (ring) {
			prd::PathState pr = s->ps;
			for (uint32_t i = b; i < e; ++i) {
				pr.iter_xyz = s->ps.iter_xyz + size_t(i - b) * ps.plane_stride;
				s->time_begin(FAM_RESOLVE, s->stream);
				prd::launch_resolve(s->sc, pr, i, s->stream);
				s->time_end(s->stream);
			}
			if (s->ps.lpe) {
				prd::PathState pl  = s->ps;
				pl.online_mean	   = nullptr;
				pl.online_variance = nullptr;
				pl.lpe			   = nullptr;
				for (uint32_t k = 0; k < s->lpe_host.n; ++k) {
					pl.out_xyz = s->lpe_host.out[k];
					for (uint32_t i = b; i < e; ++i) {
						pl.iter_xyz = s->lpe_host.iter[k] + size_t(i - b) * ps.plane_stride;
						prd::launch_resolve(s->sc, pl, i, s->stream);
					}
				}
			}
			HIP_TRY(hipGetLastError());
		}
		b = e;
	}
	return PRGPU_OK;
}

int tune_pixel_order(prgpu_scene* s)
{
	if (s->mode != prgpu_scene::PERSISTENT || s->next_iteration < (s->order_tuned_at == 0u ? 1u : std::max(64u, 8u * s->order_tuned_at)) || !s->n_slots || use_latency_kernel(s))
		return PRGPU_OK;
	s->order_tuned_at = s->next_iteration;
	if (!s->knobs.pp_tune_order)
		return PRGPU_OK;
	const prd::PersistentGeometry g = prd::persistent_geometry(s->n_slots, s->ws_pp.max_blocks, s->knobs.pp.slots);
	if (uint64_t(g.n_blocks) * g.slots_per_block < s->n_slots || g.n_blocks != s->ws_pp.max_blocks || g.n_blocks % 3u != 0u)
		return PRGPU_OK;
	const float r1 = 1.12f, r2 = 1.25f;
	const uint32_t n = s->n_slots, spb = g.slots_per_block, B = g.n_blocks, LB = B / 3u;
	std::vector<uint32_t> owned(n), cost(s->n_pixels);
	HIP_TRY(hipMemcpy(owned.data(), s->ps.pixel, size_t(n) * 4, hipMemcpyDeviceToHost));
	HIP_TRY(hipMemcpy(cost.data(), s->ps.cost, size_t(s->n_pixels) * 4, hipMemcpyDeviceToHost));
	std::vector<uint32_t> c(n);
	{
		const int W = (int)s->cfg.width, H = (int)s->cfg.height;
		for (uint32_t i = 0; i < n; ++i) {
			const int px = (int)(owned[i] % (uint32_t)W), py = (int)(owned[i] / (uint32_t)W);
			uint64_t sum = 0;
			uint32_t cnt = 0;
			for (int y = std::max(0, py - 2); y <= std::min(H - 1, py + 2); ++y)
				for (int x = std::max(0, px - 2); x <= std::min(W - 1, px + 2); ++x) {
					const uint32_t v = cost[size_t(y) * W + x];
					if (v) {
						sum += v;
						++cnt;
					}
				}
			c[i] = cnt ? (uint32_t)(sum * 16u / cnt) : 0u;
		}
	}
	std::vector<uint32_t> sorted(c);
	const size_t k = size_t(double(n) * 0.999);
	std::nth_element(sorted.begin(), sorted.begin() + k, sorted.end());
	const float c_ref = (float)sorted[k];
	const float t1 = c_ref / r1, t2 = c_ref / r2;
	std::vector<uint32_t> fill(B, 0u), cap(B);
	for (uint32_t b = 0; b < B; ++b)
		cap[b] = (uint32_t)std::min<uint64_t>(spb, uint64_t(n) > uint64_t(b) * spb ? uint64_t(n) - uint64_t(b) * spb : 0u);
	std::vector<uint32_t> out(n);
	uint32_t cursor[3] = { 0, 0, 0 };
	auto deal = [&](uint32_t pixel, uint32_t n_blocks, uint32_t& cur) -> bool {
		for (uint32_t tries = 0; tries < n_blocks; ++tries) {
			const uint32_t b = cur;
			cur				 = cur + 1 == n_blocks ? 0 : cur + 1;
			if (fill[b] < cap[b]) {
				out[size_t(b) * spb + fill[b]++] = pixel;
				return true;
			}
		}
		return false;
	};
	for (int pass = 0; pass < 3; ++pass)
		for (uint32_t i = 0; i < n; ++i) {
			const int cls = (float)c[i] > t1 ? 0 : ((float)c[i] > t2 ? 1 : 2);
			if (cls != pass)
				continue;
			bool ok = false;
// ... 1028 lines not shown
```

Baseline: 226.0 Msamples/s.

## Keep per-path pixel, RNG, radiance sum and feedback in slot-owned state

Moves the pixel index and RNG state into SlotState's padding, and adds a per-slot 128-byte SlotTail holding the running radiance sum, feedback bits, iteration, block unit and LPE state. While a path is alive, contributions go into this slot-local record instead of scattered per-pixel global arrays (iter_xyz, rng, feedback). The record is folded into the pixel buffers once, when the sample ends. This cuts scattered global read-modify-writes during shading in the persistent kernel. It adds a new tail allocation sized from max_blocks times the slot padding, and overloads the PathState iter pointer through a union, which the wavefront path could misuse.

```diff
diff --git a/pearray_amd/csrc/device/pr_device.h b/pearray_amd/csrc/device/pr_device.h
--- a/pearray_amd/csrc/device/pr_device.h
+++ b/pearray_amd/csrc/device/pr_device.h
@@ -181,7 +181,9 @@
 struct __attribute__((aligned(128))) SlotState {
 	float4 ray_o, ray_d;
 	float4 hit;
-	uint32_t flags, pad[3];
+	uint32_t flags;
+	uint32_t pixel;
+	uint64_t rng;
 	float4 sh_o, sh_d;
 	float4 wl, wl_pdf;
 	float4 cie_x, cie_y, cie_z;
@@ -189,12 +191,24 @@
 	float4 last_pos;
 	float4 sh_xyz;
 };
-static_assert(sizeof(SlotState) == 256, "SlotState must be two 128-byte lines");
+static_assert(sizeof(SlotState) == 256 && offsetof(SlotState, rng) == 56 && offsetof(SlotState, cie_x) == 128, "SlotState must be two 128-byte lines");
+struct __attribute__((aligned(128))) SlotTail {
+	float sum[3];
+	uint32_t feedback;
+	uint32_t iter;
+	uint32_t unit;
+	uint32_t lpe_state;
+	uint32_t pad[25];
+};
+static_assert(sizeof(SlotTail) == 128, "SlotTail must be one 128-byte line");
 struct PathState {
 	uint64_t* rng;
 	uint32_t* pixel;
 	struct SlotState* st;
-	uint32_t* iter;
+	union {
+		uint32_t* iter;
+		struct SlotTail* tail;
+	};
 	float4* sh_o;
 	float4* sh_d;
 	float4* sh_xyz;
diff --git a/pearray_amd/csrc/device/render.h b/pearray_amd/csrc/device/render.h
--- a/pearray_amd/csrc/device/render.h
+++ b/pearray_amd/csrc/device/render.h
@@ -11,7 +11,6 @@
 	int refill_below	 = 44;
 	uint32_t* bl_list	 = nullptr;
 	uint32_t* bl_word	 = nullptr;
-	uint32_t* slot_unit	 = nullptr;
 	size_t bl_entries	 = 0;
 };
 size_t trace_workspace_spill_entries(uint32_t max_blocks);
diff --git a/pearray_amd/csrc/device/render.hip b/pearray_amd/csrc/device/render.hip
--- a/pearray_amd/csrc/device/render.hip
+++ b/pearray_amd/csrc/device/render.hip
@@ -817,6 +817,40 @@
 	}
 }
 
+constexpr bool SLOT_OWNS_PATH = PR_UNIT != PR_WAVEFRONT;
+__device__ __forceinline__ uint32_t slot_pixel(const PathState& ps, uint32_t slot)
+{
+	if constexpr (SLOT_OWNS_PATH)
+		return ps.st[slot].pixel;
+	else
+		return ps.pixel[slot];
+}
+__device__ __forceinline__ void path_fragment(const PathState& ps, uint32_t slot, uint32_t pixel, size_t entry, uint32_t fb, const float xyz[3], uint32_t lpe_mask = 0u)
+{
+	if constexpr (SLOT_OWNS_PATH) {
+		SlotTail& t = ps.tail[slot];
+		if (fb) {
+			t.feedback |= fb;
+		} else {
+			t.sum[0] += xyz[0];
+			t.sum[1] += xyz[1];
+			t.sum[2] += xyz[2];
+			if (lpe_mask != 0u) {
+				const size_t lentry = (ps.plane_stride ? size_t(t.iter - ps.iter_base) * ps.plane_stride : size_t(0)) + size_t(3) * pixel;
+				for (uint32_t k = 0; k < PRGPU_LPE_MAX; ++k)
+					if (lpe_mask & (1u << k)) {
+						float* plane = ps.lpe->iter[k];
+						plane[lentry + 0] += xyz[0];
+						plane[lentry + 1] += xyz[1];
+						plane[lentry + 2] += xyz[2];
+					}
+			}
+		}
+	} else {
+		apply_fragment(ps, pixel, entry, fb, xyz, lpe_mask);
+	}
+}
+
 __device__ __forceinline__ void fold_iteration(const PathState& ps, uint32_t pixel, uint32_t iter, const float value[3], bool with_lpe = false)
 {
 	const float it = (float)(iter + 1), itm1 = (float)iter;
@@ -899,7 +933,7 @@
 __device__ __forceinline__ bool camera_path(const DevScene& sc, const PathState& ps, uint32_t slot, uint32_t iter, BlockStats& bs, bool with_lpe = false, WlTable wlt = WlTable())
 {
 	const prgpu_settings& cfg = sc.cfg;
-	const uint32_t pixel	  = ps.pixel[slot];
+	const uint32_t pixel	  = slot_pixel(ps, slot);
 	const uint32_t gx = pixel % cfg.width, gy = pixel / cfg.width;
 	uint64_t rnd = ps.rng[pixel];
 	float ax, ay;
@@ -1027,7 +1061,10 @@
 		d = normalized(d);
 	}
 	const bool mono	   = cfg.spectral_mono || !cfg.spectral_hero;
-	ps.rng[pixel]	   = rnd;
+	if constexpr (SLOT_OWNS_PATH)
+		ps.st[slot].rng = rnd;
+	else
+		ps.rng[pixel] = rnd;
 	if (has_ray) {
 		ps.st[slot].ray_o = make_float4(o.x, o.y, o.z, cam.near_t);
 		ps.st[slot].ray_d = make_float4(d.x, d.y, d.z, cam.far_t);
@@ -1055,7 +1092,10 @@
 	ps.st[slot].flags	   = 0u | (mono ? (FLAG_MONO | FLAG_GROUP_MONO) : 0u) | FLAG_LAST_DELTA | (has_ray ? 0u : FLAG_NO_RAY);
 	if (with_lpe && ps.lpe) {
 		const DevLpe& L	   = *ps.lpe;
-		L.state[slot]	   = lpe_step(ps.lpe, 0u, LPE_SYM_CAMERA);
+		if constexpr (SLOT_OWNS_PATH)
+			ps.tail[slot].lpe_state = lpe_step(ps.lpe, 0u, LPE_SYM_CAMERA);
+		else
+			L.state[slot] = lpe_step(ps.lpe, 0u, LPE_SYM_CAMERA);
 		const size_t lentry = (ps.plane_stride ? size_t(iter - ps.iter_base) * ps.plane_stride : size_t(0)) + size_t(3) * pixel;
 		for (uint32_t k = 0; k < L.n; ++k) {
 			float* plane	  = L.iter[k];
@@ -1064,7 +1104,12 @@
 			plane[lentry + 2] = 0.0f;
 		}
 	}
-	{
+	if constexpr (SLOT_OWNS_PATH) {
+		SlotTail& t = ps.tail[slot];
+		t.sum[0] = t.sum[1] = t.sum[2] = 0.0f;
+		t.feedback							= 0u;
+		t.iter								= iter;
+	} else {
 		const size_t entry = (ps.plane_stride ? size_t(iter - ps.iter_base) * ps.plane_stride : size_t(0)) + size_t(3) * pixel;
 		ps.iter_xyz[entry + 0] = 0.0f;
 		ps.iter_xyz[entry + 1] = 0.0f;
@@ -1705,8 +1750,8 @@
 {
 	constexpr bool EXPR		  = (FEATS & FEAT_EXPR) != 0u;
 	const prgpu_settings& cfg = sc.cfg;
-	const uint32_t pixel = ps.pixel[slot];
-	const size_t entry	 = iter_entry(ps, slot, pixel);
+	const uint32_t pixel = slot_pixel(ps, slot);
+	const size_t entry	 = SLOT_OWNS_PATH ? size_t(0) : iter_entry(ps, slot, pixel);
 	const float4 ro = ps.st[slot].ray_o, rd = ps.st[slot].ray_d;
 	const V3 ray_o = v3(ro.x, ro.y, ro.z), ray_d = v3(rd.x, rd.y, rd.z);
 	const float4 hit4  = hit_src ? *hit_src : ps.st[slot].hit;
@@ -1733,7 +1778,7 @@
 	const bool power_mis = cfg.mis == PRGPU_MIS_POWER;
 	const Blob hf		 = mono ? hero_only() : blob(1.0f);
 	const bool with_lpe	 = (FEATS & FEAT_LPE) && ps.lpe != nullptr;
-	uint32_t lpe		 = with_lpe ? ps.lpe->state[slot] : 0u;
+	uint32_t lpe		 = with_lpe ? (SLOT_OWNS_PATH ? ps.tail[slot].lpe_state : ps.lpe->state[slot]) : 0u;
 
 	if (depth == 0 && tri == INVALID) {
 		ps.prim_entity[pixel] = INVALID;
@@ -1756,11 +1801,11 @@
 				float dir_pdf;
 				inf_light_eval<EXPR>(sc, il, ray_d, wl, true, radiance, dir_pdf);
 				fb = fragment_value(sc, blob(1), blob(1), grp_imp, radiance, mono, cie, blend, xyz);
-				apply_fragment(ps, pixel, entry, fb, xyz, m_bg);
+				path_fragment(ps, slot, pixel, entry, fb, xyz, m_bg);
 			}
 			if (!illuminated) {
 				fb = fragment_value(sc, blob(1), blob(1), grp_imp, blob(0), mono, cie, blend, xyz);
-				apply_fragment(ps, pixel, entry, fb, xyz, m_bg);
+				path_fragment(ps, slot, pixel, entry, fb, xyz, m_bg);
 			}
 		} else if ((FEATS & FEAT_INFINITE_LIGHTS) && sc.n_inf_lights && cfg.direct) {
 			float denom_mis = 0;
@@ -1787,10 +1832,10 @@
 				const Blob mis	  = (hf * p0) / ((power_mis ? wvl_pdf * wvl_pdf : wvl_pdf) * denom);
 				fb				  = fragment_value(sc, mis, throughput, grp_imp, radiance, mono, cie, blend, xyz);
 			}
-			apply_fragment(ps, pixel, entry, fb, xyz, m_bg);
+			path_fragment(ps, slot, pixel, entry, fb, xyz, m_bg);
 		} else {
 			fb = fragment_value(sc, hf / (wvl_pdf * bsum(hf)), throughput, grp_imp, blob(0), mono, cie, blend, xyz);
-			apply_fragment(ps, pixel, entry, fb, xyz, m_bg);
+			path_fragment(ps, slot, pixel, entry, fb, xyz, m_bg);
 		}
 	} else {
 		const V3 P = ray_o + ray_d * hit4.x;
@@ -1838,7 +1883,7 @@
 					const Blob mis		 = (hf * p0) / ((power_mis ? wvl_pdf * wvl_pdf : wvl_pdf) * denom);
 					fb					 = fragment_value(sc, mis, throughput, grp_imp, radiance, mono, cie, blend, xyz);
 				}
-				apply_fragment(ps, pixel, entry, fb, xyz, with_lpe ? lpe_accepting(ps.lpe, lpe_step(ps.lpe, lpe, LPE_SYM_EMISSIVE)) : 0u);
+				path_fragment(ps, slot, pixel, entry, fb, xyz, with_lpe ? lpe_accepting(ps.lpe, lpe_step(ps.lpe, lpe, LPE_SYM_EMISSIVE)) : 0u);
 			}
 			if (!cfg.emissive_scatter)
 				go_on = false;
@@ -1857,7 +1902,7 @@
 				mat.transmission = resolve_texture(sc, mat.transmission, gp.uv);
 			}
 			const V3 Vt				 = to_tangent_space(N, gp.Nx, gp.Ny, -ray_d);
-			uint64_t rnd			 = ps.rng[pixel];
+			uint64_t rnd			 = SLOT_OWNS_PATH ? ps.st[slot].rng : ps.rng[pixel];
 			const bool deltaMat		 = (FEATS & FEAT_DELTA_MATERIALS) && (mat.kind == PRGPU_MAT_DIELECTRIC || mat.kind == PRGPU_MAT_CONDUCTOR || mat.kind == PRGPU_MAT_MIRROR);
 			const bool roughMat		 = (FEATS & FEAT_ROUGH_MATERIALS) && (mat.kind == PRGPU_MAT_ROUGH_CONDUCTOR || mat.kind == PRGPU_MAT_ROUGH_DIELECTRIC || mat.kind == PRGPU_MAT_PRINCIPLED);
 			const bool delta1 = comb && mix_delta_only(sc.materials[mat.two_sided].m.kind), delta2 = comb && mix_delta_only(sc.materials[mat.thin].m.kind);
@@ -1947,7 +1992,7 @@
 							const uint32_t m_nee = with_lpe ? lpe_accepting(ps.lpe, lpe_step(ps.lpe, lpe_step(ps.lpe, lpe, scatter_symbol(MIX ? sym_kind : mat.kind, MIX ? sym_roughness : mat.roughness_x, Vt, Lt)), LPE_SYM_BACKGROUND)) : 0u;
 							sh_xyz		= make_float4(xyz_vis[0], xyz_vis[1], xyz_vis[2], __uint_as_float(fb_vis | (fb_occ << 8) | (m_nee << 16)));
 						} else {
-							apply_fragment(ps, pixel, entry, fb_occ, xyz_occ);
+							path_fragment(ps, slot, pixel, entry, fb_occ, xyz_occ);
 						}
 						break;
 					}
@@ -2054,7 +2099,7 @@
 						const uint32_t m_nee = with_lpe ? lpe_accepting(ps.lpe, lpe_step(ps.lpe, lpe_step(ps.lpe, lpe, scatter_symbol(MIX ? sym_kind : mat.kind, MIX ? sym_roughness : mat.roughness_x, Vt, Lt)), LPE_SYM_EMISSIVE)) : 0u;
 						sh_xyz		= make_float4(xyz_vis[0], xyz_vis[1], xyz_vis[2], __uint_as_float(fb_vis | (fb_occ << 8) | (m_nee << 16)));
 					} else {
-						apply_fragment(ps, pixel, entry, fb_occ, xyz_occ);
+						path_fragment(ps, slot, pixel, entry, fb_occ, xyz_occ);
 					}
 				} while (false);
 			}
@@ -2182,7 +2227,7 @@
 							ps.st[slot].last_pos = make_float4(P.x, P.y, P.z, 0.0f);
 						ps.st[slot].flags		= (flags & ~0xFFu) | nd;
 						if (with_lpe)
-							ps.lpe->state[slot] = lpe;
+							(SLOT_OWNS_PATH ? ps.tail[slot].lpe_state : ps.lpe->state[slot]) = lpe;
 						atomicAdd(&bs.v[PRGPU_STAT_CAMERA_RAYS], 1u);
 						atomicAdd(&bs.v[PRGPU_STAT_BOUNCE_RAYS], 1u);
 						if (flags & FLAG_MONO)
@@ -2190,7 +2235,10 @@
 					}
 				}
 			}
-			ps.rng[pixel] = rnd;
+			if constexpr (SLOT_OWNS_PATH)
+				ps.st[slot].rng = rnd;
+			else
+				ps.rng[pixel] = rnd;
 		}
 	}
 }
@@ -2390,12 +2438,11 @@
 	if (pw & PP_SHADOW) {
 		const float4 x		 = ps.st[slot].sh_xyz;
 		const uint32_t fbs	 = __float_as_uint(x.w);
-		const uint32_t pixel = ps.pixel[slot];
 		if (pw & PP_VISIBLE) {
 			const float xyz[3] = { x.x, x.y, x.z };
-			apply_fragment(ps, pixel, iter_entry(ps, slot, pixel), fbs & 0xFFu, xyz, (FEATS & FEAT_LPE) ? (fbs >> 16) & 0xFu : 0u);
+			path_fragment(ps, slot, (FEATS & FEAT_LPE) ? ps.st[slot].pixel : 0u, 0, fbs & 0xFFu, xyz, (FEATS & FEAT_LPE) ? (fbs >> 16) & 0xFu : 0u);
 		} else if ((fbs >> 8) & 0xFFu) {
-			ps.feedback[pixel] |= (fbs >> 8) & 0xFFu;
+			ps.tail[slot].feedback |= (fbs >> 8) & 0xFFu;
 		}
 	}
 }
@@ -2405,9 +2452,18 @@
 {
 	if (ps.cost)
 		ps.cost[pixel] += (ps.st[slot].flags & 0xFFu) + 1u;
+	ps.rng[pixel]	  = ps.st[slot].rng;
+	const SlotTail& t = ps.tail[slot];
+	if (t.feedback)
+		ps.feedback[pixel] |= t.feedback;
+	const float v[3] = { t.sum[0], t.sum[1], t.sum[2] };
 	if (!ps.plane_stride) {
-		const float v[3] = { ps.iter_xyz[3 * pixel], ps.iter_xyz[3 * pixel + 1], ps.iter_xyz[3 * pixel + 2] };
 		fold_iteration(ps, pixel, iter, v, (FEATS & FEAT_LPE) != 0u);
+	} else {
+		float* e = ps.iter_xyz + size_t(iter - ps.iter_base) * ps.plane_stride + size_t(3) * pixel;
+		e[0]	 = v[0];
+		e[1]	 = v[1];
+		e[2]	 = v[2];
 	}
 }
 
@@ -2430,7 +2486,6 @@
 	uint32_t bl_cap;
 	uint32_t* bl_list;
 	uint32_t* bl_word;
-	uint32_t* slot_unit;
 	unsigned long long* gstats;
 };
 constexpr uint32_t PP_SHADE_HELP = 128u;
@@ -2455,7 +2510,7 @@
 			sh.q_shade[q][i] = PP_EMPTY;
 		sh.pending[i] = 0;
 		if (i < block_slots)
-			ps.pixel[slot0 + i] = INVALID;
+			ps.st[slot0 + i].pixel = INVALID;
 	}
 	if (threadIdx.x == 0) {
 		sh.ray_head = sh.ray_tail = 0;
@@ -2582,17 +2637,17 @@
 				bool need_pixel	 = false;
 				uint32_t iter	 = 0;
 				if (ended) {
-					const uint32_t pixel = ps.pixel[slot];
+					const uint32_t pixel = ps.st[slot].pixel;
 					need_pixel			 = true;
 					if (pixel != INVALID) {
-						iter = ps.iter[slot];
+						iter = ps.tail[slot].iter;
 						fold_ended_sample<FEATS>(ps, slot, pixel, iter);
 						if (iter + 1 < a.iter_end) {
 							if (!a.resident) {
 								need_pixel = false;
 								iter	   = iter + 1;
 							} else {
-								const uint32_t old = __hip_atomic_fetch_add(&bl_word[a.slot_unit[slot]], 1u, __ATOMIC_ACQ_REL, __HIP_MEMORY_SCOPE_WORKGROUP);
+								const uint32_t old = __hip_atomic_fetch_add(&bl_word[ps.tail[slot].unit], 1u, __ATOMIC_ACQ_REL, __HIP_MEMORY_SCOPE_WORKGROUP);
 								if ((old >> 16) >= (old & 0xFFFFu) + 1u) {
 									need_pixel = false;
 									iter	   = iter + 1;
@@ -2628,8 +2683,8 @@
 								uint32_t entry	 = BL_HOLE;
 								if (i < a.n_owned) {
 									entry				= a.owned[i];
-									ps.pixel[slot]		= entry;
-									a.slot_unit[slot]	= pos + rank;
+									ps.st[slot].pixel	= entry;
+									ps.tail[slot].unit	= pos + rank;
 									iter				= a.iter_begin;
 									need_pixel			= false;
 								}
@@ -2671,8 +2726,8 @@
 									const uint32_t old = __hip_atomic_fetch_add(&bl_word[k], 1u << 16, __ATOMIC_ACQ_REL, __HIP_MEMORY_SCOPE_WORKGROUP);
 									const uint32_t r   = (old >> 16) + 1u;
 									if ((old & 0xFFFFu) >= r) {
-										ps.pixel[slot]	  = p;
-										a.slot_unit[slot] = k;
+										ps.st[slot].pixel  = p;
+										ps.tail[slot].unit = k;
 										iter			  = a.iter_begin + r;
 										need_pixel		  = false;
 									}
@@ -2683,13 +2738,13 @@
 				} else {
 					uint32_t idx;
 					if (a.direct_map)
-						idx = need_pixel && ps.pixel[slot] == INVALID ? slot : a.n_owned;
+						idx = need_pixel && ps.st[slot].pixel == INVALID ? slot : a.n_owned;
 					else
 						idx = wave_append(need_pixel, a.next_pixel);
 					if (need_pixel) {
 						if (idx < a.n_owned) {
-							ps.pixel[slot] = a.owned[idx];
-							iter		   = a.iter_begin;
+							ps.st[slot].pixel = a.owned[idx];
+							iter			  = a.iter_begin;
 						} else {
 							retired = true;
 						}
@@ -2697,7 +2752,6 @@
 				}
 				const unsigned long long t0c = COUNT ? wall_clock64() : 0ull;
 				if (ended && !retired) {
-					ps.iter[slot] = iter;
 					camera_path(sc, ps, slot, iter, sh.bs, (FEATS & FEAT_LPE) != 0u, wlt);
 					alive = true;
 				}
@@ -3531,7 +3585,6 @@
 	a.bl_cap		  = (uint32_t)std::min<uint64_t>(n_owned, 2ull * ((n_owned + g.n_blocks - 1) / g.n_blocks) + 1024ull);
 	a.bl_list		  = ws.bl_list;
 	a.bl_word		  = ws.bl_word;
-	a.slot_unit		  = ws.slot_unit;
 	a.resident		  = resident_ok && !all_in_flight && iter_end - iter_begin >= 2u && iter_end - iter_begin < 65536u && ws.bl_list != nullptr
 						&& uint64_t(a.bl_cap) * g.n_blocks <= ws.bl_entries && uint64_t(a.bl_cap) * (iter_end - iter_begin) < (1ull << 31)
 					  ? 1u
@@ -3576,7 +3629,6 @@
 	a.iter_begin	 = iter_begin;
 	a.iter_end		 = iter_end;
 	a.spill			 = ws.spill;
-	a.slot_index	 = ws.slot_unit;
 	a.refill_below	 = std::min(64, std::max(1, tune.refill_below));
 	a.shade_min		 = (uint32_t)std::min(64, std::max(1, tune.shade_min));
 	a.gstats		 = gstats;
diff --git a/pearray_amd/csrc/prgpu_api.hip b/pearray_amd/csrc/prgpu_api.hip
--- a/pearray_amd/csrc/prgpu_api.hip
+++ b/pearray_amd/csrc/prgpu_api.hip
@@ -183,7 +183,8 @@
 	Mode mode = LOCKSTEP;
 	Knobs knobs;
 	uint32_t pp_planes = 1;
-	uint32_t *pp_pixel = nullptr, *pp_next = nullptr, *pp_error = nullptr;
+	uint32_t *pp_next = nullptr, *pp_error = nullptr;
+	prd::SlotTail* pp_tail = nullptr;
 	unsigned long long* gstats = nullptr;
 	prd::TraceWorkspace ws;
 	prd::TraceWorkspace ws_pp;
@@ -665,7 +666,6 @@
 		s->mode = prgpu_scene::LOCKSTEP;
 	else if (s->knobs.mode == 1)
 		s->mode = t.single_tap ? prgpu_scene::STREAMING : prgpu_scene::LOCKSTEP;
-	AL(s->pp_pixel, ns, false);
 	AL(s->pp_next, 1, true);
 	AL(s->pp_error, 1, true);
 	AL(s->gstats, prd::N_DEVICE_COUNTERS, true);
@@ -701,7 +701,7 @@
 			s->ws_pp.bl_entries = 2 * size_t(np) + size_t(s->ws_pp.max_blocks) * 1026u;
 			AL(s->ws_pp.bl_list, s->ws_pp.bl_entries, false);
 			AL(s->ws_pp.bl_word, s->ws_pp.bl_entries, false);
-			AL(s->ws_pp.slot_unit, ns, false);
+			AL(s->pp_tail, std::min<size_t>(ns, size_t(s->ws_pp.max_blocks) * prd::slot_array_padding()), false);
 		}
 		if (rc != PRGPU_OK)
 			return rc;
@@ -1064,7 +1064,8 @@
 	if (!s->n_slots)
 		return PRGPU_OK;
 	prd::PathState ps = s->ps;
-	ps.pixel		  = s->pp_pixel;
+	ps.pixel		  = nullptr;
+	ps.tail			  = s->pp_tail;
 	const uint64_t per_iter = std::max<uint64_t>(1, s->n_slots);
 	uint32_t chunk			= (uint32_t)std::min<uint64_t>(1u << 15, std::max<uint64_t>((uint64_t)s->knobs.pp_launch_min_iters, s->knobs.pp_launch_samples / per_iter));
 	const bool all_in_flight = uint64_t(s->n_slots) <= uint64_t(s->ws_pp.max_blocks) * s->knobs.pp.slots;
```

Result: slower. 223.4 Msamples/s (-1.1%).
